# dmuley/sph-code

Measured on AMD Instinct MI355X. Metric: particle-steps/sec + achieved HBM GB/s, 10^6-particle 3D sphere, 1/2/4/8 GPUs, higher is better.
Workload: dtype f64

## Files before the change

### sph-code_amd/csrc/sphx_api.hip

```cpp
#include "sphx_internal.h"
#include <stdarg.h>
#include <stdlib.h>
#include <new>

int sphx_set_err(sphx_ctx* ctx, int code, const char* fmt, ...) {
    if (ctx) {
        va_list ap;
        va_start(ap, fmt);
        vsnprintf(ctx->err, sizeof(ctx->err), fmt, ap);
        va_end(ap);
    }
    return code;
}

void sphx_release(sphx_ctx* ctx, DevBuf& b) {
    for (size_t q = 0; q < ctx->allocs.size(); ++q)
        if (ctx->allocs[q] == b.p) { ctx->allocs[q] = ctx->allocs.back(); ctx->allocs.pop_back(); break; }
    if (b.p) (void)hipFree(b.p);
    b.p = nullptr;
    b.cap = 0;
}

int sphx_ensure(sphx_ctx* ctx, DevBuf& b, size_t bytes, hipStream_t in_use_on) {
    if (bytes == 0) bytes = 8;
// ... 275 lines not shown
    SPHX_TRY(upload(ctx, ctx->in_f, mu_array, nb));
    SPHX_TRY(upload(ctx, ctx->in_g, gamma_array, nb));
    SPHX_TRY(upload(ctx, ctx->in_h, particle_type, nb));
    if (neighbor) {
        SPHX_TRY(sphx_transpose_nbr(ctx, n, k, ctx->idx64.as<int64_t>()));
        ctx->nbr_api_valid = true; ctx->nbr_api_n = n; ctx->nbr_api_k = k;
    }
    PrepIn pin;
    pin.pos_aos(ctx->in_a.as<double>()); pin.vel_aos(ctx->in_b.as<double>());
    pin.m = ctx->in_c.as<double>(); pin.h = ctx->in_d.as<double>(); pin.T = ctx->in_e.as<double>();
    pin.mu = ctx->in_f.as<double>(); pin.gam = ctx->in_g.as<double>(); pin.ptype = ctx->in_h.as<double>();
    SPHX_TRY(sphx_prep(ctx, n, pin, visc_mode == 1, ctx->stream));
    SPHX_TRY(sphx_pass_density(ctx, n, k));
    if (visc_mode == 1) {
        SPHX_TRY(sphx_pass_visc_pw(ctx, n, k, ctx->in_c.as<double>()));
    } else {
        SPHX_TRY(sphx_pass_pi(ctx, n, k, ctx->in_d.as<double>(), ctx->in_h.as<double>()));
        SPHX_TRY(sphx_pass_visc(ctx, n, k, ctx->in_c.as<double>()));
    }
    if (f_un_nb) {
        SPHX_TRY(upload(ctx, ctx->in_i, f_un, (size_t)n * s * sizeof(double)));
        SPHX_TRY(sphx_ensure(ctx, ctx->F, (size_t)n * s * sizeof(double)));
        SPHX_TRY(sphx_pass_species(ctx, n, k, s, ctx->in_i.as<double>(), ctx->F.as<double>()));
        SPHX_TRY(download(ctx, f_un_nb, ctx->F.p, (size_t)n * s * sizeof(double)));
    }
    SPHX_TRY(download(ctx, hydro_accel, ctx->ha.p, 3 * nb));
    SPHX_TRY(download(ctx, visc_accel, ctx->va.p, 3 * nb));
    SPHX_TRY(download(ctx, visc_heat, ctx->vh.p, nb));
    SPHX_TRY(download(ctx, rho, ctx->rho.p, nb));
    SPHX_TRY(download(ctx, nden, ctx->nden.p, nb));
    SPHX_TRY(download(ctx, rho_dust, ctx->rhod.p, nb));
    HIPCHK(hipStreamSynchronize(ctx->stream));
    return SPHX_OK;
}

extern "C" int sphx_state_upload(sphx_ctx* ctx, int64_t n, int s, const double* pos, const double* vel,
                                 const double* mass, const double* ptype, const double* f_un,
                                 const double* T, const double* mu, const double* gamma,
                                 const double* E_internal, const double* accel_old) {
    if (!ctx) return SPHX_E_ARG;
    NEED(pos); NEED(vel); NEED(mass); NEED(ptype); NEED(T); NEED(mu); NEED(gamma); NEED(E_internal);
    if (n < 1 || n > 0x7FFFFFF0ll) return sphx_set_err(ctx, SPHX_E_ARG, "n=%lld out of range", (long long)n);
    if (f_un && (s < 1 || s > SPHX_MAX_SPECIES)) return sphx_set_err(ctx, SPHX_E_ARG, "s=%d out of range", s);
    HIPCHK(hipSetDevice(ctx->device));
    const size_t nb = (size_t)n * sizeof(double);
    StateArrays& st = ctx->st;
    DevBuf* scal[] = {&st.x, &st.y, &st.z, &st.vx, &st.vy, &st.vz, &st.ax, &st.ay, &st.az,
                      &st.m, &st.T, &st.mu, &st.gam, &st.E, &st.hprev, &st.ptype};
    for (DevBuf* b : scal) SPHX_TRY(sphx_ensure(ctx, *b, nb));
    SPHX_TRY(sphx_ensure(ctx, st.id, (size_t)n * sizeof(int)));
    SPHX_TRY(upload(ctx, ctx->in_a, pos, 3 * nb));
    SPHX_TRY(sphx_aos_to_soa3(ctx, n, ctx->in_a.as<double>(), st.x.as<double>(), st.y.as<double>(), st.z.as<double>()));
    SPHX_TRY(upload(ctx, ctx->in_b, vel, 3 * nb));
    SPHX_TRY(sphx_aos_to_soa3(ctx, n, ctx->in_b.as<double>(), st.vx.as<double>(), st.vy.as<double>(), st.vz.as<double>()));
    if (accel_old) {
        SPHX_TRY(upload(ctx, ctx->in_c, accel_old, 3 * nb));
        SPHX_TRY(sphx_aos_to_soa3(ctx, n, ctx->in_c.as<double>(), st.ax.as<double>(), st.ay.as<double>(), st.az.as<double>()));
    } else {
        HIPCHK(hipMemsetAsync(st.ax.p, 0, nb, ctx->stream));
        HIPCHK(hipMemsetAsync(st.ay.p, 0, nb, ctx->stream));
        HIPCHK(hipMemsetAsync(st.az.p, 0, nb, ctx->stream));
    }
    HIPCHK(hipMemcpyAsync(st.m.p, mass, nb, hipMemcpyHostToDevice, ctx->stream));
    HIPCHK(hipMemcpyAsync(st.T.p, T, nb, hipMemcpyHostToDevice, ctx->stream));
    HIPCHK(hipMemcpyAsync(st.mu.p, mu, nb, hipMemcpyHostToDevice, ctx->stream));
    HIPCHK(hipMemcpyAsync(st.gam.p, gamma, nb, hipMemcpyHostToDevice, ctx->stream));
    HIPCHK(hipMemcpyAsync(st.E.p, E_internal, nb, hipMemcpyHostToDevice, ctx->stream));
    HIPCHK(hipMemcpyAsync(st.ptype.p, ptype, nb, hipMemcpyHostToDevice, ctx->stream));
    HIPCHK(hipMemsetAsync(st.hprev.p, 0, nb, ctx->stream));
    SPHX_TRY(sphx_iota(ctx, n, st.id.as<int>()));
    ctx->s = 0;
    if (f_un) {
        const int sp = (s + 15) & ~15;
        SPHX_TRY(upload(ctx, ctx->in_d, f_un, (size_t)n * s * sizeof(double)));
        SPHX_TRY(sphx_ensure(ctx, ctx->fun_id, (size_t)n * sp * sizeof(double)));
        HIPCHK(hipMemsetAsync(ctx->fun_id.p, 0, (size_t)n * sp * sizeof(double), ctx->stream));
        HIPCHK(hipMemcpy2DAsync(ctx->fun_id.p, (size_t)sp * sizeof(double), ctx->in_d.p, (size_t)s * sizeof(double),
                                (size_t)s * sizeof(double), (size_t)n, hipMemcpyDeviceToDevice, ctx->stream));
        ctx->s = s;
        ctx->sp = sp;
    }
    HIPCHK(hipMemsetAsync(ctx->scal.p, 0, SC_NSLOTS * 8, ctx->stream));
    HIPCHK(hipMemsetAsync(ctx->badc.p, 0, (size_t)BADC_BUCKETS * BADC_STRIDE * sizeof(u64), ctx->stream));
    ctx->ct_primed = false;
    ctx->nbr_api_valid = false;
    HIPCHK(hipStreamSynchronize(ctx->stream));
    ctx->n = n;
    ctx->npad = sphx_pad64(n);
    ctx->has_state = true;
    ctx->drag = false;
    ctx->agb_on = false;
    ctx->gravity = 0;
    ctx->loop_forms = 0;
    ctx->list_valid = false;
    ctx->clip_valid = false;
    ctx->h_clip = 0.0;
    ctx->lag_bvalid[0] = ctx->lag_bvalid[1] = ctx->lag_hvalid[0] = ctx->lag_hvalid[1] = false;
    ctx->step_count = 0;
    ctx->tprev_valid = false;
    ctx->dt_last = 0.0;
    return SPHX_OK;
}

extern "C" int sphx_state_set_drag(sphx_ctx* ctx, const double* mean_grain_mass, const double* mean_cross) {
    if (!ctx) return SPHX_E_ARG;
    if (!ctx->has_state || ctx->step_count != 0)
        return sphx_set_err(ctx, SPHX_E_STATE, "sphx_state_set_drag must follow sphx_state_upload directly");
    HIPCHK(hipSetDevice(ctx->device));
    if (!mean_grain_mass || !mean_cross) { ctx->drag = false; return SPHX_OK; }
    const size_t nb = (size_t)ctx->n * sizeof(double);
    SPHX_TRY(sphx_ensure(ctx, ctx->st.mgm, nb));
    SPHX_TRY(sphx_ensure(ctx, ctx->st.mcs, nb));
    HIPCHK(hipMemcpyAsync(ctx->st.mgm.p, mean_grain_mass, nb, hipMemcpyHostToDevice, ctx->stream));
    HIPCHK(hipMemcpyAsync(ctx->st.mcs.p, mean_cross, nb, hipMemcpyHostToDevice, ctx->stream));
    HIPCHK(hipStreamSynchronize(ctx->stream));
    ctx->drag = true;
    return SPHX_OK;
}

extern "C" int sphx_state_set_loop_forms(sphx_ctx* ctx, int on, double d) {
    if (!ctx) return SPHX_E_ARG;
    if (!ctx->has_state) return sphx_set_err(ctx, SPHX_E_STATE, "sphx_state_set_loop_forms before sphx_state_upload");
    if (on && !(d > 0.0)) return sphx_set_err(ctx, SPHX_E_ARG, "the loop forms need the driver's global d > 0 (drv:68)");
    if (on && ctx->use_verlet) return sphx_set_err(ctx, SPHX_E_STATE, "loop-form steps are not combined with incremental search");
    if (on && ctx->visc_mode != 0)
        return sphx_set_err(ctx, SPHX_E_ARG, "loop-form steps have their own (pairwise) viscosity: visc_mode must be 0");
    ctx->loop_forms = on ? 1 : 0;
    ctx->loop_d = d;
    return SPHX_OK;
}

extern "C" int sphx_set_gravity_order(sphx_ctx* ctx, int order) {
    if (!ctx) return SPHX_E_ARG;
    if (order != 1 && order != 2) return sphx_set_err(ctx, SPHX_E_ARG, "gravity order %d not 1 (monopole) or 2 (quadrupole)", order);
    ctx->grav_order = order;
    return SPHX_OK;
}

extern "C" int sphx_set_clip_grad(sphx_ctx* ctx, int on) {
    if (!ctx) return SPHX_E_ARG;
    ctx->clip_grad = on ? 1 : 0;
    return SPHX_OK;
}

extern "C" int sphx_set_visc_mode(sphx_ctx* ctx, int mode) {
    if (!ctx) return SPHX_E_ARG;
    if (mode != 0 && mode != 1)
        return sphx_set_err(ctx, SPHX_E_ARG, "visc_mode %d unknown (0 = ref_axis0, 1 = pairwise)", mode);
    if (mode != 0 && ctx->loop_forms)
        return sphx_set_err(ctx, SPHX_E_ARG, "loop-form steps have their own (pairwise) viscosity: visc_mode must be 0");
    ctx->visc_mode = mode;
    return SPHX_OK;
}

extern "C" int sphx_state_set_gravity(sphx_ctx* ctx, int mode, double G) {
    if (!ctx) return SPHX_E_ARG;
    if (!ctx->has_state) return sphx_set_err(ctx, SPHX_E_STATE, "sphx_state_set_gravity before sphx_state_upload");
    if (mode < 0 || mode > 2) return sphx_set_err(ctx, SPHX_E_ARG, "gravity mode %d not in {0, 1, 2}", mode);
    if (mode == 2 && ctx->use_verlet)
        return sphx_set_err(ctx, SPHX_E_STATE, "tree gravity needs the cell grid of every step: not with incremental search");
    ctx->gravity = mode;
    ctx->grav_G = G;
    return SPHX_OK;
}

static PrepIn prep_in_of_state(const StateArrays& s) {
    PrepIn in;
    in.x = s.x.as<double>(); in.y = s.y.as<double>(); in.z = s.z.as<double>(); in.ps = 1;
    in.vx = s.vx.as<double>(); in.vy = s.vy.as<double>(); in.vz = s.vz.as<double>(); in.vs = 1;
    in.m = s.m.as<double>(); in.h = s.hprev.as<double>(); in.T = s.T.as<double>();
    in.mu = s.mu.as<double>(); in.gam = s.gam.as<double>(); in.ptype = s.ptype.as<double>();
    return in;
}

static int step_cell_hint(sphx_ctx* ctx, int64_t n, double* cell_hint) {
    *cell_hint = 0.0;
    if (ctx->step_count == 0) return SPHX_OK;
    const double* hs;
    if (ctx->lag_hvalid[ctx->lag_hslot]) {
        HIPCHK(hipEventSynchronize(ctx->lag_halias[ctx->lag_hslot] ? ctx->lag_halias[ctx->lag_hslot]
                                                                     : ctx->lag_hev[ctx->lag_hslot]));
        hs = (const double*)((char*)ctx->pinned + LAG_OFF + 512 * ctx->lag_hslot + 256);
        const u64* sv = (const u64*)hs;
        for (int q = 0; q < 10; ++q) ctx->knn_lag[q] = sv[(SC_NFAILQ - SC_HSUM) + q];
        ctx->knn_lag_valid = true;
    } else {
        HIPCHK(hipMemcpyAsync((char*)ctx->pinned + 256, ctx->scal.as<double>() + SC_HSUM, 4 * sizeof(double),
                              hipMemcpyDeviceToHost, ctx->stream));
        HIPCHK(hipStreamSynchronize(ctx->stream));
        hs = (const double*)((char*)ctx->pinned + 256);
    }
    const double hmean = hs[3] > 0.0 ? hs[0] / hs[3] : 0.0;
    if (hmean > 0.0 && isfinite(hmean)) {
        *cell_hint = ctx->cell_factor * sphx_cell_feedback(ctx, n) * hmean;
        ctx->h_clip = ctx->h_clip_factor * hmean;
    }
    return SPHX_OK;
}

static int step_search(sphx_ctx* ctx, int k, double dist, hipEvent_t* ev) {
    const int64_t n = ctx->n;
    if (ctx->use_verlet) SPHX_TRY(sphx_clamp(ctx, n, ctx->st));
    SPHX_TRY(sphx_ensure(ctx, ctx->nbr, (size_t)k * ctx->npad * sizeof(int)));
    if (ctx->use_verlet && ctx->list_valid && ctx->list_n == n && ctx->list_k == k) {
        StateArrays& r = ctx->st;
        HIPCHK(hipEventRecord(ev[1], ctx->stream));
        int64_t nfail = 0;
        SPHX_TRY(sphx_knn_refresh(ctx, n, k, r.x.as<double>(), r.y.as<double>(), r.z.as<double>(),
                                  ctx->nbr.as<int>(), r.hprev.as<double>(), &nfail));
        if (nfail == 0) {
            ctx->stats.refresh_steps++;
            return SPHX_OK;
        }
        ctx->list_valid = false;
    }
    double cell_hint = 0.0;
    SPHX_TRY(step_cell_hint(ctx, n, &cell_hint));
    {
        StateArrays& r = ctx->st;
        const bool blob = ctx->use_blob && !ctx->use_verlet;
        GridBuildOpts g;
        g.lagged = true;
        g.alias_ev = ev[1];
        g.sort_cells_later = blob;
        if (!ctx->use_verlet) { g.clamp_vel[0] = r.vx.as<double>(); g.clamp_vel[1] = r.vy.as<double>(); g.clamp_vel[2] = r.vz.as<double>(); }
        SPHX_TRY(sphx_build_grid(ctx, n, k, r.x.as<double>(), r.y.as<double>(), r.z.as<double>(), cell_hint, g));
        if (blob) SPHX_TRY(sphx_build_blob_order(ctx, n, true));
    }
    const bool split = ctx->side_stream && !ctx->use_verlet;
    SPHX_TRY(sphx_permute_state(ctx, n, split, ev[1]));
    StateArrays& r = ctx->st;
    KnnIn in;
    in.xs = r.x.as<double>(); in.ys = r.y.as<double>(); in.zs = r.z.as<double>();
    in.id = r.id.as<int>(); in.inv = ctx->inv.as<int>();
    in.rsearch = r.hprev.as<double>();
    in.hinted = ctx->step_count > 0 && !ctx->use_verlet;
    in.lag_external = true;
    in.rscale = ctx->rscale;
    in.rbound = dist;
    KnnOut o;
    o.nbr = ctx->nbr.as<int>();
    o.h_sorted = r.hprev.as<double>();
    o.idx64 = nullptr; o.dist = nullptr; o.nontriv = nullptr; o.h_by_id = nullptr;
    if (ctx->use_verlet) {
        SPHX_TRY(sphx_ensure(ctx, ctx->list64, (size_t)n * 64 * sizeof(int)));
        SPHX_TRY(sphx_ensure(ctx, ctx->dref, (size_t)n * sizeof(double)));
        o.list64 = ctx->list64.as<int>();
        o.dref = ctx->dref.as<double>();
        in.rscale = ctx->rscale_build;
    }
    SPHX_TRY(sphx_knn(ctx, n, k, in, o));
    if (split) HIPCHK(hipStreamWaitEvent(ctx->stream, ctx->ev_perm, 0));
    if (ctx->use_verlet) {
        SPHX_TRY(sphx_save_list_positions(ctx, n, r.x.as<double>(), r.y.as<double>(), r.z.as<double>()));
        ctx->list_valid = true;
        ctx->list_n = n;
        ctx->list_k = k;
    }
    ctx->stats.rebuild_steps++;
    return SPHX_OK;
}

static int step_h_sums_out(sphx_ctx* ctx, int64_t n, const double* h, hipStream_t stream) {
    SPHX_TRY(sphx_hsum(ctx, n, h, stream));
    const int hsl = ctx->lag_hslot ^ 1;
    HIPCHK(hipMemcpyAsync((char*)ctx->pinned + LAG_OFF + 512 * hsl + 256, ctx->scal.as<double>() + SC_HSUM,
                          (SC_KGDBG + 2 - SC_HSUM + 1) * sizeof(double), hipMemcpyDeviceToHost, stream));
    HIPCHK(hipEventRecord(ctx->lag_hev[hsl], stream));
    ctx->lag_halias[hsl] = nullptr;
    ctx->lag_hvalid[hsl] = true;
    ctx->lag_hslot = hsl;
    return SPHX_OK;
}

static int step_sums(sphx_ctx* ctx, int k, hipEvent_t* ev, hipEvent_t search_end, bool detail) {
    const int64_t n = ctx->n;
    StateArrays& s = ctx->st;
    const bool pairwise = ctx->visc_mode == 1 && !ctx->loop_forms;
    const bool fork = ctx->qorder && ctx->use_lds && !ctx->loop_forms && ctx->side_stream;
    if (fork) HIPCHK(hipStreamWaitEvent(ctx->side_stream, search_end, 0));
    else SPHX_TRY(step_h_sums_out(ctx, n, s.hprev.as<double>(), ctx->stream));
    if (ctx->qorder && ctx->use_lds) SPHX_TRY(sphx_blob_translate(ctx, n, k));
    const bool species = ctx->s > 0 && ctx->fun_id.p;
    if (ctx->loop_forms) {
        if (ctx->drag || species)
            SPHX_TRY(sphx_prep(ctx, n, prep_in_of_state(s), pairwise, ctx->stream));
        if (detail) HIPCHK(hipEventRecord(ev[3], ctx->stream));
        SPHX_TRY(sphx_loop_step_sums(ctx, n, k, ctx->loop_d));
        if (detail) HIPCHK(hipEventRecord(ev[9], ctx->stream));
        if (species) SPHX_TRY(sphx_step_species(ctx, n, k));
        if (detail) HIPCHK(hipEventRecord(ev[4], ctx->stream));
        if (detail) HIPCHK(hipEventRecord(ev[5], ctx->stream));
    } else {
        SPHX_TRY(sphx_prep(ctx, n, prep_in_of_state(s), pairwise, fork ? ctx->side_stream : ctx->stream));
        if (fork) {
            HIPCHK(hipEventRecord(ctx->ev_join, ctx->side_stream));
            HIPCHK(hipStreamWaitEvent(ctx->stream, ctx->ev_join, 0));
            SPHX_TRY(step_h_sums_out(ctx, n, s.hprev.as<double>(), ctx->side_stream));
        }
        if (detail) HIPCHK(hipEventRecord(ev[3], ctx->stream));
        const bool sp_fused = species && ctx->species_fused && ctx->species_lds && ctx->use_lds && ctx->qorder && ctx->blob_lists &&
                              !ctx->map_perm && ctx->sp == 16 && ctx->s <= 16 && k <= SPHX_MAX_K;
        if (sp_fused) {
            const int S = ctx->s;
            SPHX_TRY(sphx_ensure(ctx, ctx->rho, (size_t)n * sizeof(double)));
            SPHX_TRY(sphx_ensure(ctx, ctx->rhod, (size_t)n * sizeof(double)));
            SPHX_TRY(sphx_ensure(ctx, ctx->nden, (size_t)n * sizeof(double)));
            SPHX_TRY(sphx_ensure(ctx, ctx->G, (size_t)n * 3 * sizeof(double)));
            SPHX_TRY(sphx_ensure(ctx, ctx->ha, (size_t)n * 3 * sizeof(double)));
            SPHX_TRY(sphx_ensure(ctx, ctx->F, (size_t)n * S * sizeof(double)));
            if (ctx->agb_on) {
                SPHX_TRY(sphx_ensure(ctx, ctx->Zmet, (size_t)n * sizeof(double)));
                SPHX_TRY(sphx_ensure(ctx, ctx->agb_dust, (size_t)n * S * sizeof(double)));
            }
            SPHX_TRY(sphx_blob_density_species(ctx, n, k, true, S, ctx->fun_id.as<double>(), s.id.as<int>(),
                                               s.m.as<double>(), ctx->F.as<double>(), ctx->Zmet.as<double>(),
                                               ctx->agb_dust.as<double>(), (ctx->agb_on && ctx->Zmet.p && ctx->agb_dust.p) ? 1 : 0));
        } else {
            SPHX_TRY(sphx_pass_density(ctx, n, k, true));
        }
        if (detail) HIPCHK(hipEventRecord(ev[9], ctx->stream));
        if (species && !sp_fused) SPHX_TRY(sphx_step_species(ctx, n, k));
        if (detail) HIPCHK(hipEventRecord(ev[4], ctx->stream));
        if (ctx->visc_mode == 1) {
            SPHX_TRY(sphx_pass_visc_pw(ctx, n, k, s.m.as<double>()));
        } else {
            SPHX_TRY(sphx_pass_pi(ctx, n, k, s.hprev.as<double>(), s.ptype.as<double>()));
            if (detail) HIPCHK(hipEventRecord(ev[5], ctx->stream));
            SPHX_TRY(sphx_pass_visc(ctx, n, k, s.m.as<double>()));
        }
    }
    if (ctx->drag)
        SPHX_TRY(sphx_pass_drag(ctx, n, k, s.m.as<double>(), s.ptype.as<double>(), s.mgm.as<double>(), s.mcs.as<double>()));
    return SPHX_OK;
}

static int one_step(sphx_ctx* ctx, int k, double dist, int first, double fixed_dt, bool call_first, bool call_last) {
    const int64_t n = ctx->n;
    const int ring = (int)(ctx->step_count % 3);
    hipEvent_t* ev = ctx->evring[ring];
    const bool detail = ctx->timing_detail;
    ctx->ev_detail[ring] = detail;
    const bool rec0 = detail || call_first, rec7 = detail || call_last;
    ctx->ev_has07[ring] = (rec0 ? 1 : 0) | (rec7 ? 2 : 0) | (ctx->visc_mode == 1 && !ctx->loop_forms ? 4 : 0);
    ctx->map_perm = nullptr;
    ctx->qorder = nullptr;
    ctx->blob_lists = false;
    ctx->blob_split_valid = false;
    ctx->pass_part = 0;
    ctx->nbr_api_valid = false;
    if (rec0) HIPCHK(hipEventRecord(ev[0], ctx->stream));
    SPHX_TRY(step_search(ctx, k, dist, ev));
    HIPCHK(hipEventRecord(ev[2], ctx->stream));
    SPHX_TRY(step_sums(ctx, k, ev, ev[2], detail));
    if (detail) HIPCHK(hipEventRecord(ev[6], ctx->stream));
    StateArrays& s = ctx->st;
    if (ctx->gravity) {
        SPHX_TRY(sphx_ensure(ctx, ctx->grav, (size_t)n * 3 * sizeof(double)));
        double* eps = ctx->scal.as<double>() + SC_GRAV_EPS;
        SPHX_TRY(sphx_median(ctx, n, s.hprev.as<double>(), eps));
        if (ctx->gravity == 1)
            SPHX_TRY(sphx_gravity_launch(ctx, n, s.x.as<double>(), s.y.as<double>(), s.z.as<double>(), 1,
                                         s.m.as<double>(), eps, 0.0, ctx->grav_G, nullptr, ctx->grav.as<double>()));
        else
            SPHX_TRY(sphx_gravity_tree_launch(ctx, n, s.x.as<double>(), s.y.as<double>(), s.z.as<double>(),
                                              s.m.as<double>(), ctx->grav_ws, eps, 0.0, ctx->grav_G, nullptr,
                                              ctx->grav.as<double>()));
    }
    if (detail) HIPCHK(hipEventRecord(ev[8], ctx->stream));
    SPHX_TRY(sphx_integrate(ctx, n, 1, first, fixed_dt));
    if (rec7) HIPCHK(hipEventRecord(ev[7], ctx->stream));
    ctx->step_count++;
    return SPHX_OK;
}

static int collect_stats(sphx_ctx* ctx, int ring) {
    if (!(ctx->ev_pending & (1u << ring))) return SPHX_OK;
    ctx->ev_pending &= ~(1u << ring);
    hipEvent_t* ev = ctx->evring[ring];
    const int has = ctx->ev_has07[ring];
    HIPCHK(hipEventSynchronize((has & 2) ? ev[7] : ev[2]));
    sphx_stats& st = ctx->stats;
    float ms[7] = {0.f, 0.f, 0.f, 0.f, 0.f, 0.f, 0.f};
    HIPCHK(hipEventElapsedTime(&ms[1], ev[1], ev[2]));
    st.ms_search += ms[1];
    st.steps += 1;
    st.search_steps += 1;
    st.n = ctx->n;
    if (!ctx->ev_detail[ring]) return SPHX_OK;
    float tot;
    HIPCHK(hipEventElapsedTime(&tot, ev[0], ev[7]));
    HIPCHK(hipEventElapsedTime(&ms[0], ev[0], ev[1]));
    st.ms_grid += ms[0]; st.ms_total += tot;
    for (int i = 2; i < 6; ++i) {
        if ((has & 4) && i >= 4) break;
        HIPCHK(hipEventElapsedTime(&ms[i], ev[i], ev[i + 1]));
    }
    if (has & 4) HIPCHK(hipEventElapsedTime(&ms[5], ev[4], ev[6]));
    st.ms_prep += ms[2];
    float mg = 0.f, mi = 0.f;
    HIPCHK(hipEventElapsedTime(&mg, ev[6], ev[8]));
    HIPCHK(hipEventElapsedTime(&mi, ev[8], ev[7]));
    ms[6] = mi;
    st.ms_gravity += mg;
    {
        float md = 0.f, msp = 0.f;
        HIPCHK(hipEventElapsedTime(&md, ev[3], ev[9]));
        HIPCHK(hipEventElapsedTime(&msp, ev[9], ev[4]));
        ms[3] = md;
        st.ms_species += msp;
    }
    st.ms_density += ms[3]; st.ms_pi += ms[4]; st.ms_visc += ms[5]; st.ms_integrate += ms[6];
    st.detail_steps += 1;
    return SPHX_OK;
}

extern "C" int sphx_step(sphx_ctx* ctx, int nsteps, int k, double dist, int first, double fixed_dt) {
    if (!ctx) return SPHX_E_ARG;
    if (!ctx->has_state) return sphx_set_err(ctx, SPHX_E_STATE, "sphx_step before sphx_state_upload");
    if (k < 1 || k > SPHX_MAX_K) return sphx_set_err(ctx, SPHX_E_ARG, "N_NEIGH=%d not in 1..%d", k, SPHX_MAX_K);
    if (nsteps < 1) return sphx_set_err(ctx, SPHX_E_ARG, "nsteps=%d < 1", nsteps);
    HIPCHK(hipSetDevice(ctx->device));
    if (!(dist > 0.0) || !isfinite(dist)) dist = 0.0;
    ctx->k = k;
    const bool per_call = !ctx->timing_detail;
    if (per_call) HIPCHK(hipEventRecord(ctx->ev[8], ctx->stream));
    for (int it = 0; it < nsteps; ++it) {
        const int ring = (int)(ctx->step_count % 3);
        SPHX_TRY(collect_stats(ctx, ring));
        SPHX_TRY(one_step(ctx, k, dist, first && it == 0, fixed_dt, false, false));
        ctx->ev_pending |= 1u << ring;
        SPHX_TRY(collect_stats(ctx, (ring + 1) % 3));
    }
    if (per_call) HIPCHK(hipEventRecord(ctx->ev[9], ctx->stream));
    HIPCHK(hipMemcpyAsync(ctx->pinned, ctx->scal.p, SC_NSLOTS * 8, hipMemcpyDeviceToHost, ctx->stream));
    HIPCHK(hipStreamSynchronize(ctx->stream));
    for (int r = 0; r < 3; ++r) SPHX_TRY(collect_stats(ctx, (int)((ctx->step_count + r) % 3)));
    if (per_call) {
        float tot = 0.f;
        HIPCHK(hipEventElapsedTime(&tot, ctx->ev[8], ctx->ev[9]));
        ctx->stats.ms_total += tot;
    }
    const u64* sc = (const u64*)ctx->pinned;
    ctx->dt_last = ((const double*)ctx->pinned)[SC_DT];
    ctx->stats.candidates = (int64_t)sc[SC_CAND];
    ctx->stats.retries = (int64_t)sc[SC_RETRY];
    ctx->stats.fallback_queries = (int64_t)(u32)sc[SC_NFAILQ];
    ctx->stats.short_rows = (int64_t)sc[SC_SHORT];
    SPHX_TRY(sphx_badc_read(ctx));
    return SPHX_OK;
}

extern "C" int sphx_state_download(sphx_ctx* ctx, double* pos, double* vel, double* accel,
                                   double* E_internal, double* T, double* sizes, double* rho,
                                   double* nden, double* visc_heat, double* dt_last) {
    if (!ctx) return SPHX_E_ARG;
    if (!ctx->has_state) return sphx_set_err(ctx, SPHX_E_STATE, "no state uploaded");
    HIPCHK(hipSetDevice(ctx->device));
    const int64_t n = ctx->n;
    const size_t nb = (size_t)n * sizeof(double);
    StateArrays& s = ctx->st;
    const int* id = s.id.as<int>();
    SPHX_TRY(sphx_ensure(ctx, ctx->out_a, 3 * nb));
    double* stage = ctx->out_a.as<double>();
    struct V3 { double* host; DevBuf *a, *b, *c; };
    V3 v3[] = {{pos, &s.x, &s.y, &s.z}, {vel, &s.vx, &s.vy, &s.vz}, {accel, &s.ax, &s.ay, &s.az}};
    for (V3& v : v3) {
        if (!v.host) continue;
        SPHX_TRY(sphx_soa3_to_aos_by_id(ctx, n, id, v.a->as<double>(), v.b->as<double>(), v.c->as<double>(), stage));
        SPHX_TRY(download(ctx, v.host, stage, 3 * nb));
        HIPCHK(hipStreamSynchronize(ctx->stream));
    }
    struct V1 { double* host; const double* dev; };
    const bool stepped = ctx->step_count > 0;
    V1 v1[] = {{E_internal, s.E.as<double>()}, {T, s.T.as<double>()}, {sizes, s.hprev.as<double>()},
               {rho, stepped ? ctx->rho.as<double>() : nullptr},
               {nden, stepped ? ctx->nden.as<double>() : nullptr},
               {visc_heat, stepped ? ctx->vh.as<double>() : nullptr}};
    for (V1& v : v1) {
        if (!v.host) continue;
        if (!v.dev) { memset(v.host, 0, nb); continue; }
        SPHX_TRY(sphx_scatter_rows_by_id(ctx, n, 1, id, v.dev, stage));
        SPHX_TRY(download(ctx, v.host, stage, nb));
        HIPCHK(hipStreamSynchronize(ctx->stream));
    }
    if (dt_last) *dt_last = ctx->dt_last;
    return SPHX_OK;
}

int sphx_agb_table_set(sphx_ctx* ctx, int S, int nspl, const int32_t* ntx, const int32_t* nty, const double* tx, const double* ty,
                       const double* coeffs, const int32_t* mapto, double divisor, const double* mu_specie, double solar_mass) {
    ctx->agb_on = false;
    if (nspl == 0) return SPHX_OK;
    if (S < 7 || S > AGB_MAX_SPEC) return sphx_set_err(ctx, SPHX_E_ARG, "AGB table: %d species (7..%d)", S, AGB_MAX_SPEC);
    if (!ntx || !nty || !tx || !ty || !coeffs || !mapto || !mu_specie)
        return sphx_set_err(ctx, SPHX_E_ARG, "AGB table: NULL argument");
    if (nspl < 1 || nspl > AGB_MAX_SPL) return sphx_set_err(ctx, SPHX_E_ARG, "AGB table: %d splines", nspl);
    if (!(divisor != 0.0)) return sphx_set_err(ctx, SPHX_E_ARG, "AGB table: divisor is 0");
    HIPCHK(hipSetDevice(ctx->device));
    AgbTable& t = ctx->agb;
    t.nspl = nspl; t.nspec = S;
    size_t ntx_tot = 0, nty_tot = 0, nc_tot = 0;
    for (int o = 0; o < nspl; ++o) {
        if (ntx[o] < 4 || nty[o] < 4) return sphx_set_err(ctx, SPHX_E_ARG, "AGB table: spline %d has fewer than 4 knots", o);
        if (mapto[o] < 0 || mapto[o] >= S) return sphx_set_err(ctx, SPHX_E_ARG, "AGB table: mapto[%d]=%d out of range", o, mapto[o]);
        ntx_tot += ntx[o]; nty_tot += nty[o]; nc_tot += (size_t)(ntx[o] - 2) * (nty[o] - 2);
    }
    size_t ox = 0, oy = ntx_tot, oc = ntx_tot + nty_tot;
    for (int o = 0; o < nspl; ++o) {
        t.tx_off[o] = (int)ox; t.ty_off[o] = (int)oy; t.c_off[o] = (int)oc;
        t.ntx[o] = ntx[o]; t.nty[o] = nty[o]; t.mapto[o] = mapto[o];
        ox += ntx[o]; oy += nty[o]; oc += (size_t)(ntx[o] - 2) * (nty[o] - 2);
    }
// ... 122 lines not shown
```

### sph-code_amd/csrc/sphx_dev.hip

```cpp
#include "sphx_internal.h"
#pragma clang fp contract(off)
#include <float.h>
#include "sphx_leapfrog.h"

extern "C" int sphx_set_stream(sphx_ctx* ctx, void* stream) {
    if (!ctx) return SPHX_E_ARG;
    HIPCHK(hipSetDevice(ctx->device));
    HIPCHK(hipStreamSynchronize(ctx->stream));
    ctx->stream = (hipStream_t)stream;
    return SPHX_OK;
}

extern "C" int sphx_reset_stream(sphx_ctx* ctx) {
    if (!ctx) return SPHX_E_ARG;
    HIPCHK(hipSetDevice(ctx->device));
    HIPCHK(hipStreamSynchronize(ctx->stream));
    ctx->stream = ctx->own_stream;
    return SPHX_OK;
}

__global__ __launch_bounds__(256) void gather3_aos_kernel(int n, const int* perm, const double* aos,
                                                          double* xs, double* ys, double* zs, int* inv) {
    int t = blockIdx.x * blockDim.x + threadIdx.x;
    if (t >= n) return;
// ... 81 lines not shown

extern "C" int sphx_dev_get_order(sphx_ctx* ctx, int64_t n_total, int32_t* out) {
    if (!ctx) return SPHX_E_ARG;
    NEED(out);
    if (!ctx->map_perm || ctx->n != n_total)
        return sphx_set_err(ctx, SPHX_E_STATE, "sphx_dev_get_order: no search over %lld particles", (long long)n_total);
    HIPCHK(hipSetDevice(ctx->device));
    HIPCHK(hipMemcpyAsync(out, ctx->map_perm, (size_t)n_total * sizeof(int), hipMemcpyDeviceToDevice, ctx->stream));
    return SPHX_OK;
}

extern "C" int sphx_dev_select_blobs(sphx_ctx* ctx, int part) {
    if (!ctx) return SPHX_E_ARG;
    if (part < 0 || part > 2) return sphx_set_err(ctx, SPHX_E_ARG, "sphx_dev_select_blobs: part %d not in 0..2", part);
    ctx->pass_part = 0;
    if (part == 0) return 0;
    if (!(ctx->map_perm && ctx->qorder && ctx->blob_lists && ctx->blob_split_valid)) return 0;
    ctx->pass_part = part;
    return 1;
}

extern "C" int sphx_dev_blob_split_counts(sphx_ctx* ctx, int32_t counts[3]) {
    if (!ctx) return SPHX_E_ARG;
    NEED(counts);
    if (!ctx->blob_split_valid) return sphx_set_err(ctx, SPHX_E_STATE, "sphx_dev_blob_split_counts: no split (LDS passes off, or no search yet)");
    HIPCHK(hipSetDevice(ctx->device));
    HIPCHK(hipMemcpyAsync(counts, ctx->blob_split.as<int>() + (size_t)ctx->blob_split_nblk, 3 * sizeof(int),
                          hipMemcpyDeviceToHost, ctx->stream));
    HIPCHK(hipStreamSynchronize(ctx->stream));
    return SPHX_OK;
}

extern "C" int sphx_dev_set_mean_h(sphx_ctx* ctx, double mean_h) {
    if (!ctx) return SPHX_E_ARG;
    ctx->dev_hmean = mean_h;
    return SPHX_OK;
}

extern "C" int sphx_dev_prep(sphx_ctx* ctx, const double* pos, const double* vel, const double* mass,
                             const double* h, const double* T, const double* mu, const double* gamma,
                             const double* ptype) {
    if (!ctx) return SPHX_E_ARG;
    NEED(pos); NEED(vel); NEED(mass); NEED(h); NEED(T); NEED(mu); NEED(gamma); NEED(ptype);
    if (!ctx->map_perm) return sphx_set_err(ctx, SPHX_E_STATE, "sphx_dev_prep before sphx_dev_search");
    HIPCHK(hipSetDevice(ctx->device));
    PrepIn in;
    in.pos_aos(pos); in.vel_aos(vel);
    in.m = mass; in.h = h; in.T = T; in.mu = mu; in.gam = gamma; in.ptype = ptype;
    return sphx_prep(ctx, ctx->n, in, ctx->visc_mode == 1, ctx->stream);
}

struct Borrow {
    DevBuf& b;
    DevBuf saved;
    Borrow(DevBuf& buf, void* p, size_t bytes) : b(buf), saved(buf) {
        if (p) { b.p = p; b.cap = bytes; }
    }
    ~Borrow() { b = saved; }
    Borrow(const Borrow&) = delete;
    Borrow& operator=(const Borrow&) = delete;
};

extern "C" int sphx_dev_density(sphx_ctx* ctx, double* rho, double* rho_dust, double* nden,
                                double* hydro_accel) {
    if (!ctx) return SPHX_E_ARG;
    if (!ctx->map_perm) return sphx_set_err(ctx, SPHX_E_STATE, "sphx_dev_density before sphx_dev_search");
    HIPCHK(hipSetDevice(ctx->device));
    const size_t nb = (size_t)ctx->n * sizeof(double);
    Borrow b1(ctx->rho, rho, nb), b2(ctx->rhod, rho_dust, nb), b3(ctx->nden, nden, nb), b4(ctx->ha, hydro_accel, 3 * nb);
    SPHX_TRY(sphx_pass_density(ctx, ctx->n, ctx->k));
    return SPHX_OK;
}

extern "C" int sphx_dev_pi(sphx_ctx* ctx, const double* rho_complete, double* Pi, double* Bw, double* ct_out) {
    if (!ctx) return SPHX_E_ARG;
    NEED(rho_complete);
    if (!ctx->map_perm) return sphx_set_err(ctx, SPHX_E_STATE, "sphx_dev_pi before sphx_dev_search");
    HIPCHK(hipSetDevice(ctx->device));
    const int64_t n = ctx->n;
    if (ctx->pass_part != 1)
        hipLaunchKernelGGL(inject_field_kernel, dim3((unsigned)((n + 255) / 256)), dim3(256), 0, ctx->stream, (int)n,
                           ctx->map_perm, rho_complete, ctx->rho_s.as<double>(), 1);
    HIPCHK(hipGetLastError());
    if (ctx->pass_part == 2) ctx->ct_primed = true;
    {
        Borrow b1(ctx->Pi, Pi, (size_t)n * sizeof(double)), b2(ctx->Bw, Bw, (size_t)n * sizeof(double));
        SPHX_TRY(sphx_pass_pi(ctx, n, ctx->k, nullptr, nullptr));
    }
    if (ct_out)
        HIPCHK(hipMemcpyAsync(ct_out, ctx->scal.as<u64>() + SC_CT_BITS, 8, hipMemcpyDeviceToDevice, ctx->stream));
    return SPHX_OK;
}

extern "C" int sphx_dev_visc(sphx_ctx* ctx, const double* Bw_complete, const double* mass,
                             double* visc_accel, double* visc_heat) {
    if (!ctx) return SPHX_E_ARG;
    NEED(Bw_complete); NEED(mass);
    if (!ctx->map_perm) return sphx_set_err(ctx, SPHX_E_STATE, "sphx_dev_visc before sphx_dev_search");
    HIPCHK(hipSetDevice(ctx->device));
    const int64_t n = ctx->n;
    if (ctx->pass_part != 1)
        hipLaunchKernelGGL(inject_field_kernel, dim3((unsigned)((n + 255) / 256)), dim3(256), 0, ctx->stream, (int)n,
                           ctx->map_perm, Bw_complete, ctx->bc_s.as<double>(), 2);
    HIPCHK(hipGetLastError());
    Borrow b1(ctx->va, visc_accel, 3 * (size_t)n * sizeof(double)), b2(ctx->vh, visc_heat, (size_t)n * sizeof(double));
    SPHX_TRY(sphx_pass_visc(ctx, n, ctx->k, mass));
    return SPHX_OK;
}

extern "C" int sphx_dev_visc_pairwise(sphx_ctx* ctx, const double* rho_complete, const double* mass,
                                      double* visc_accel, double* visc_heat, double* ct_out) {
    if (!ctx) return SPHX_E_ARG;
    NEED(rho_complete); NEED(mass);
    if (!ctx->map_perm) return sphx_set_err(ctx, SPHX_E_STATE, "sphx_dev_visc_pairwise before sphx_dev_search");
    if (ctx->visc_mode != 1) return sphx_set_err(ctx, SPHX_E_STATE, "sphx_dev_visc_pairwise needs sphx_set_visc_mode(ctx, 1)");
    if (!ctx->recs_pw)
        return sphx_set_err(ctx, SPHX_E_STATE, "sphx_dev_visc_pairwise: the records were not built in pairwise mode "
                                               "(sphx_set_visc_mode(ctx, 1) before sphx_dev_prep)");
    HIPCHK(hipSetDevice(ctx->device));
    const int64_t n = ctx->n;
    if (ctx->pass_part != 1)
        hipLaunchKernelGGL(inject_field_kernel, dim3((unsigned)((n + 255) / 256)), dim3(256), 0, ctx->stream, (int)n,
                           ctx->map_perm, rho_complete, ctx->rho_s.as<double>(), 1);
    HIPCHK(hipGetLastError());
    if (ctx->pass_part == 2) ctx->ct_primed = true;
    {
        Borrow b1(ctx->va, visc_accel, 3 * (size_t)n * sizeof(double)), b2(ctx->vh, visc_heat, (size_t)n * sizeof(double));
        SPHX_TRY(sphx_pass_visc_pw(ctx, n, ctx->k, mass));
    }
    if (ct_out)
        HIPCHK(hipMemcpyAsync(ct_out, ctx->scal.as<u64>() + SC_CT_BITS, 8, hipMemcpyDeviceToDevice, ctx->stream));
    return SPHX_OK;
}

#define nan_to_num_v sphx_nan_to_num
struct DevIntegArgs {
    int n;
    double *pos, *vel, *acc, *E, *T;
    const double *m, *mu, *gam, *ptype, *ha, *va, *vh;
    const double *G, *rho;
    const double *drag_on, *drag_re, *drho, *drhod;
    double dt, m_h, kB, lim;
    const double* red2;
    double* dt_out;
    int first;
    double fixed_dt, dt_0, max_age;
    u64* counters;
};
__global__ __launch_bounds__(256) void dev_integrate_kernel(DevIntegArgs a) {
    int i = blockIdx.x * blockDim.x + threadIdx.x;
    if (i >= a.n) return;
    double dt = a.dt;
    if (a.red2) {
        if (a.red2[0] > 0.5) {
            if (i == 0) *a.dt_out = 0.0;
            return;
        }
        const double ct_min = -a.red2[1];
        const double ctv = sphx_ct_value(ct_min > DBL_MAX, ct_min, a.dt_0);
        dt = (a.fixed_dt > 0.0) ? a.fixed_dt : sphx_dt_rule(ctv, a.first, a.dt_0, a.max_age);
        if (i == 0) *a.dt_out = dt;
    }
    const double g = (a.ptype[i] == 0.0) ? 1.0 : 0.0;
    double v[3], pa[3], vis[3];
    bool bad_acc = false;
#pragma unroll
    for (int c = 0; c < 3; ++c) {
        v[c] = a.vel[3 * (size_t)i + c];
        if (a.G) {
            const double praw = a.G[3 * (size_t)i + c] / a.rho[i] * g;
            pa[c] = nan_to_num_v(praw);
            vis[c] = a.va[3 * (size_t)i + c];
            bad_acc = bad_acc || !sphx_finite(praw) || !sphx_finite(vis[c]);
        } else {
            const double praw = -a.ha[3 * (size_t)i + c] * g, vraw = -a.va[3 * (size_t)i + c] * g;
            pa[c] = nan_to_num_v(praw);
            vis[c] = nan_to_num_v(vraw);
            bad_acc = bad_acc || !sphx_finite(praw) || !sphx_finite(vraw);
        }
        if (a.drag_on) {
            const double draw = a.drag_on[3 * (size_t)i + c] * a.drhod[i] / a.drho[i] * g, rraw = a.drag_re[3 * (size_t)i + c];
            const double dg = nan_to_num_v(draw);
            vis[c] = dg + nan_to_num_v(rraw) + vis[c];
            bad_acc = bad_acc || !sphx_finite(draw) || !sphx_finite(rraw);
        }
    }
    double x[3], old[3], tot[3];
#pragma unroll
    for (int c = 0; c < 3; ++c) { x[c] = a.pos[3 * (size_t)i + c]; old[c] = a.acc[3 * (size_t)i + c]; }
    sphx_leapfrog_update(dt, x, v, vis, pa, nullptr, old, tot);
#pragma unroll
    for (int c = 0; c < 3; ++c) {
        a.pos[3 * (size_t)i + c] = x[c];
        a.vel[3 * (size_t)i + c] = v[c];
        a.acc[3 * (size_t)i + c] = tot[c];
    }
    double E = a.E[i], T;
    const double heat = a.vh[i];
    const bool bad_en = !sphx_finite(E) || !sphx_finite(heat * dt);
    sphx_energy_update(dt, heat, a.mu[i], a.gam[i], a.m[i], a.m_h, a.kB, E, T);
    a.E[i] = E;
    a.T[i] = T;
    if (a.counters) {
        bool bad_st = false;
#pragma unroll
        for (int c = 0; c < 3; ++c) bad_st = bad_st || !sphx_finite(x[c]) || !sphx_finite(v[c]);
        sphx_count_bad(a.counters, BAD_ACCEL, bad_acc);
        sphx_count_bad(a.counters, BAD_ENERGY, bad_en);
        sphx_count_bad(a.counters, BAD_STATE, bad_st);
    }
}
static DevIntegArgs dev_integ_args(sphx_ctx* ctx, int64_t n_owned, double* pos, double* vel, double* accel_old, double* E_internal,
                                   double* T, const double* mass, const double* mu, const double* gamma, const double* ptype,
                                   const double* ha, const double* va, const double* vh, double dt) {
// ... 595 lines not shown
```

### sph-code_amd/csrc/sphx_grid.hip

```cpp
#include "sphx_internal.h"
#include <rocprim/rocprim.hpp>
#include <float.h>

#define RED_BLOCK 256
#define RED_MAXBLOCKS 1024
#define FUSED_MAXBLOCKS 4096

__device__ __forceinline__ double wave_min(double v) {
#pragma unroll
    for (int o = 32; o > 0; o >>= 1) v = fmin(v, __shfl_xor(v, o, 64));
    return v;
}
__device__ __forceinline__ double wave_max(double v) {
#pragma unroll
    for (int o = 32; o > 0; o >>= 1) v = fmax(v, __shfl_xor(v, o, 64));
    return v;
}

__device__ __forceinline__ double wave_sum(double v) {
#pragma unroll
    for (int o = 32; o > 0; o >>= 1) v += __shfl_xor(v, o, 64);
    return v;
}

#define BB_W 13
#define BB_PIVOT 16
#define BB_OUT 19
struct ClipBox { double lo[3], hi[3]; int on; double pivot[3]; int pivot_dev; };
static void clip_set_pivot(ClipBox& clip, const double* fallback) {
    clip.pivot_dev = 0;
    for (int c = 0; c < 3; ++c) clip.pivot[c] = clip.on ? 0.5 * (clip.lo[c] + clip.hi[c]) : (fallback ? fallback[c] : 0.0);
    if (!clip.on && !fallback) clip.pivot_dev = 1;
    for (int c = 0; c < 3; ++c) if (!isfinite(clip.pivot[c])) clip.pivot[c] = 0.0;
}
__device__ __forceinline__ void clip_pivot(const ClipBox& clip, int n, const double* x, const double* y, const double* z,
                                           double p[3]) {
    p[0] = clip.pivot[0]; p[1] = clip.pivot[1]; p[2] = clip.pivot[2];
    if (clip.pivot_dev && n > 0) {
        const double f[3] = {x[0], y[0], z[0]};
        for (int c = 0; c < 3; ++c) p[c] = isfinite(f[c]) ? f[c] : 0.0;
    }
}
__global__ __launch_bounds__(RED_BLOCK) void bbox_partial(int n, const double* x, const double* y,
                                                          const double* z, ClipBox clip, double* partial) {
    __shared__ double sm[RED_BLOCK / 64][BB_W];
    double mn[3] = {INFINITY, INFINITY, INFINITY}, mx[3] = {-INFINITY, -INFINITY, -INFINITY};
    double su[3] = {0.0, 0.0, 0.0}, sq[3] = {0.0, 0.0, 0.0}, cnt = 0.0;
    double piv[3];
    clip_pivot(clip, n, x, y, z, piv);
    for (int i = blockIdx.x * blockDim.x + threadIdx.x; i < n; i += gridDim.x * blockDim.x) {
        double v[3] = {x[i], y[i], z[i]};
        if (isfinite(v[0]) && isfinite(v[1]) && isfinite(v[2])) {
            bool in = true;
#pragma unroll
            for (int c = 0; c < 3; ++c) {
                mn[c] = fmin(mn[c], v[c]); mx[c] = fmax(mx[c], v[c]);
                if (clip.on && (v[c] < clip.lo[c] || v[c] > clip.hi[c])) in = false;
            }
            if (in) {
                cnt += 1.0;
#pragma unroll
                for (int c = 0; c < 3; ++c) { const double r = v[c] - piv[c]; su[c] += r; sq[c] += r * r; }
            }
        }
    }
    int lane = threadIdx.x & 63, wave = threadIdx.x >> 6;
#pragma unroll
    for (int c = 0; c < 3; ++c) {
        mn[c] = wave_min(mn[c]); mx[c] = wave_max(mx[c]); su[c] = wave_sum(su[c]); sq[c] = wave_sum(sq[c]);
    }
    cnt = wave_sum(cnt);
    if (lane == 0) {
        for (int c = 0; c < 3; ++c) {
            sm[wave][c] = mn[c]; sm[wave][3 + c] = mx[c]; sm[wave][6 + c] = su[c]; sm[wave][9 + c] = sq[c];
        }
        sm[wave][12] = cnt;
    }
    __syncthreads();
    if (threadIdx.x < BB_W) {
        const int c = threadIdx.x;
        double v = sm[0][c];
        for (int w = 1; w < RED_BLOCK / 64; ++w)
            v = c < 3 ? fmin(v, sm[w][c]) : (c < 6 ? fmax(v, sm[w][c]) : v + sm[w][c]);
        partial[blockIdx.x * BB_W + c] = v;
    }
// ... 19 lines not shown
    if ((threadIdx.x & 63) == 0) sw[threadIdx.x >> 6] = v;
    __syncthreads();
    if (threadIdx.x == 0) {
        const double a0 = sw[0], a1 = sw[1], a2 = sw[2], a3 = sw[3];
        out[c] = c < 3 ? fmin(fmin(a0, a1), fmin(a2, a3)) : (c < 6 ? fmax(fmax(a0, a1), fmax(a2, a3)) : (a0 + a1) + (a2 + a3));
    }
}

static int bbox_launch(sphx_ctx* ctx, int64_t n, const double* x, const double* y, const double* z, bool use_clip,
                       void* host_dst) {
    ClipBox clip;
    clip.on = (use_clip && ctx->clip_valid) ? 1 : 0;
    for (int c = 0; c < 3; ++c) { clip.lo[c] = ctx->clip_lo[c]; clip.hi[c] = ctx->clip_hi[c]; }
    clip_set_pivot(clip, nullptr);
    int blocks = (int)((n + RED_BLOCK - 1) / RED_BLOCK);
    if (blocks > RED_MAXBLOCKS) blocks = RED_MAXBLOCKS;
    SPHX_TRY(sphx_ensure(ctx, ctx->bbox_tmp, (size_t)(RED_MAXBLOCKS + 2 + FUSED_MAXBLOCKS) * BB_W * sizeof(double)));
    double* part = ctx->bbox_tmp.as<double>();
    double* fin = part + (size_t)RED_MAXBLOCKS * BB_W;
    hipLaunchKernelGGL(bbox_partial, dim3(blocks), dim3(RED_BLOCK), 0, ctx->stream, (int)n, x, y, z, clip, part);
    hipLaunchKernelGGL(bbox_final, dim3(BB_W + 3), dim3(256), 0, ctx->stream, blocks, part, fin, (int)n, x, y, z, clip);
    HIPCHK(hipGetLastError());
    HIPCHK(hipMemcpyAsync(host_dst, fin, BB_OUT * sizeof(double), hipMemcpyDeviceToHost, ctx->stream));
    return SPHX_OK;
}
static void bbox_finish(const void* host_src, double out_minmax[13], double rel[9] = nullptr) {
    memcpy(out_minmax, host_src, BB_W * sizeof(double));
    double piv[3];
    memcpy(piv, (const double*)host_src + BB_PIVOT, sizeof(piv));
    const double cnt = out_minmax[12] > 0.0 ? out_minmax[12] : 1.0;
    for (int c = 0; c < 3; ++c) {
        const double mean = out_minmax[6 + c] / cnt;
        double var = out_minmax[9 + c] / cnt - mean * mean;
        if (rel) { rel[c] = out_minmax[c] - piv[c]; rel[3 + c] = out_minmax[3 + c] - piv[c]; rel[6 + c] = mean; }
        out_minmax[6 + c] = piv[c] + mean;
        out_minmax[9 + c] = var > 0.0 ? sqrt(var) : 0.0;
    }
}
static int bbox_sync(sphx_ctx* ctx, int64_t n, const double* x, const double* y, const double* z,
                     double out_minmax[13], bool use_clip, double rel[9]) {
    SPHX_TRY(bbox_launch(ctx, n, x, y, z, use_clip, ctx->pinned));
    HIPCHK(hipStreamSynchronize(ctx->stream));
    bbox_finish(ctx->pinned, out_minmax, rel);
    return SPHX_OK;
}
int sphx_bbox(sphx_ctx* ctx, int64_t n, const double* x, const double* y, const double* z,
              double out_minmax[13], bool use_clip) {
    return bbox_sync(ctx, n, x, y, z, out_minmax, use_clip, nullptr);
}

__device__ __forceinline__ int cell_coord_g(double v, double vmin, double inv_cell, int nmax1) {
    double t = (v - vmin) * inv_cell;
    t = fmin(fmax(t, 0.0), (double)nmax1);
    return (int)t;
}

__global__ __launch_bounds__(256) void cell_count(int n, const double* x, const double* y,
                                                  const double* z, GridParams g, int* cell_of,
                                                  int* hist) {
    int i = blockIdx.x * blockDim.x + threadIdx.x;
    if (i >= n) return;
    int cx = cell_coord_g(x[i], g.xmin, g.inv_cell, g.nx - 1);
    int cy = cell_coord_g(y[i], g.ymin, g.inv_cell, g.ny - 1);
    int cz = cell_coord_g(z[i], g.zmin, g.inv_cell, g.nz - 1);
    int c = (cz * g.ny + cy) * g.nx + cx;
    cell_of[i] = c;
    atomicAdd(&hist[c], 1);
}

struct FusedCountArgs {
    int n;
    double *x, *y, *z, *vx, *vy, *vz;
    double lim;
    ClipBox clip;
    GridParams g;
    int* cell_of;
    int* hist;
    double* partial;
    unsigned* ticket;
    double* fin;
    u64* ct_reset;
    int* zero_int;
    int* rank;
};
__global__ __launch_bounds__(RED_BLOCK) void grid_count_fused(FusedCountArgs a) {
    __shared__ double sm[RED_BLOCK / 64][BB_W];
    double mn[3] = {INFINITY, INFINITY, INFINITY}, mx[3] = {-INFINITY, -INFINITY, -INFINITY};
    double su[3] = {0.0, 0.0, 0.0}, sq[3] = {0.0, 0.0, 0.0}, cnt = 0.0;
    const GridParams g = a.g;
    const double piv[3] = {a.clip.pivot[0], a.clip.pivot[1], a.clip.pivot[2]};
    if (a.ct_reset && blockIdx.x == 0 && threadIdx.x == 0) *a.ct_reset = SPHX_CT_NONE;
    if (a.zero_int && blockIdx.x == 0 && threadIdx.x == 0) { a.zero_int[0] = 0; a.zero_int[1] = 0; }
    for (int i = blockIdx.x * blockDim.x + threadIdx.x; i < a.n; i += gridDim.x * blockDim.x) {
        double v[3] = {a.x[i], a.y[i], a.z[i]};
        if (a.vx) {
            const double o0 = v[0], o1 = v[1], o2 = v[2];
#pragma unroll
            for (int c = 0; c < 3; ++c) {
                double q = v[c];
                q = (q > a.lim) ? a.lim : q;
                q = (q < -a.lim) ? -a.lim : q;
                v[c] = sphx_nan_to_num(q);
            }
            if (__double_as_longlong(v[0]) != __double_as_longlong(o0)) a.x[i] = v[0];
            if (__double_as_longlong(v[1]) != __double_as_longlong(o1)) a.y[i] = v[1];
            if (__double_as_longlong(v[2]) != __double_as_longlong(o2)) a.z[i] = v[2];
            const double w0 = a.vx[i], w1 = a.vy[i], w2 = a.vz[i];
            const double u0 = sphx_nan_to_num(w0), u1 = sphx_nan_to_num(w1), u2 = sphx_nan_to_num(w2);
            if (__double_as_longlong(u0) != __double_as_longlong(w0)) a.vx[i] = u0;
            if (__double_as_longlong(u1) != __double_as_longlong(w1)) a.vy[i] = u1;
            if (__double_as_longlong(u2) != __double_as_longlong(w2)) a.vz[i] = u2;
        }
        if (isfinite(v[0]) && isfinite(v[1]) && isfinite(v[2])) {
            bool in = true;
#pragma unroll
            for (int c = 0; c < 3; ++c) {
                mn[c] = fmin(mn[c], v[c]); mx[c] = fmax(mx[c], v[c]);
                if (a.clip.on && (v[c] < a.clip.lo[c] || v[c] > a.clip.hi[c])) in = false;
            }
            if (in) {
                cnt += 1.0;
#pragma unroll
                for (int c = 0; c < 3; ++c) { const double r = v[c] - piv[c]; su[c] += r; sq[c] += r * r; }
            }
        }
        const int cx = cell_coord_g(v[0], g.xmin, g.inv_cell, g.nx - 1);
        const int cy = cell_coord_g(v[1], g.ymin, g.inv_cell, g.ny - 1);
        const int cz = cell_coord_g(v[2], g.zmin, g.inv_cell, g.nz - 1);
        const int c = (cz * g.ny + cy) * g.nx + cx;
        a.cell_of[i] = c;
        if (a.rank) a.rank[i] = atomicAdd(&a.hist[c], 1);
        else atomicAdd(&a.hist[c], 1);
    }
    const int lane = threadIdx.x & 63, wave = threadIdx.x >> 6;
#pragma unroll
    for (int c = 0; c < 3; ++c) {
        mn[c] = wave_min(mn[c]); mx[c] = wave_max(mx[c]); su[c] = wave_sum(su[c]); sq[c] = wave_sum(sq[c]);
    }
    cnt = wave_sum(cnt);
    if (lane == 0) {
        for (int c = 0; c < 3; ++c) {
            sm[wave][c] = mn[c]; sm[wave][3 + c] = mx[c]; sm[wave][6 + c] = su[c]; sm[wave][9 + c] = sq[c];
        }
        sm[wave][12] = cnt;
    }
    __syncthreads();
    if (threadIdx.x < BB_W) {
        const int c = threadIdx.x;
        double v = sm[0][c];
        for (int w = 1; w < RED_BLOCK / 64; ++w)
            v = c < 3 ? fmin(v, sm[w][c]) : (c < 6 ? fmax(v, sm[w][c]) : v + sm[w][c]);
        a.partial[blockIdx.x * BB_W + c] = v;
    }
}


#define SCAN_ITEMS 8
#define SCAN_BLOCK 256
#define SCAN_TILE (SCAN_ITEMS * SCAN_BLOCK)

__device__ __forceinline__ int block_exclusive_scan(int v, int* total_out) {
    __shared__ int wsum[SCAN_BLOCK / 64];
    int lane = threadIdx.x & 63, wave = threadIdx.x >> 6;
    int incl = v;
#pragma unroll
    for (int o = 1; o < 64; o <<= 1) {
        int up = __shfl_up(incl, o, 64);
        if (lane >= o) incl += up;
    }
    if (lane == 63) wsum[wave] = incl;
    __syncthreads();
    int woff = 0, tot = 0;
#pragma unroll
    for (int w = 0; w < SCAN_BLOCK / 64; ++w) {
        int s = wsum[w];
        if (w < wave) woff += s;
        tot += s;
    }
    __syncthreads();
    *total_out = tot;
    return woff + incl - v;
}

#define LBS_ITEMS 32
#define LBS_TILE (LBS_ITEMS * 256)
#define LBS_MAXTILES 512
template <int ZERO>
__global__ __launch_bounds__(256) void lookback_scan_kernel(int n_items, int* __restrict__ in, int* __restrict__ out,
                                                            u64* state, int* ctr, unsigned epoch, int ntiles) {
    __shared__ int s_prefix;
// ... 177 lines not shown
    }
    if (bb_part && (int)blockIdx.x < BB_W && (int)gridDim.x >= BB_W) {
        const int c = blockIdx.x;
        double v = c < 3 ? INFINITY : (c < 6 ? -INFINITY : 0.0);
        for (int b = threadIdx.x; b < bb_nblocks; b += 256) {
            const double p = bb_part[b * BB_W + c];
            v = c < 3 ? fmin(v, p) : (c < 6 ? fmax(v, p) : v + p);
        }
        v = c < 3 ? wave_min(v) : (c < 6 ? wave_max(v) : wave_sum(v));
        if ((threadIdx.x & 63) == 0) sw[threadIdx.x >> 6] = v;
        __syncthreads();
        if (threadIdx.x == 0) {
            const double a0 = sw[0], a1 = sw[1], a2 = sw[2], a3 = sw[3];
            const double r_ = c < 3 ? fmin(fmin(a0, a1), fmin(a2, a3)) : (c < 6 ? fmax(fmax(a0, a1), fmax(a2, a3)) : (a0 + a1) + (a2 + a3));
            bb_out[c] = r_;
            if (bb_host) bb_host[c] = r_;
        }
    }
}

#define CELL_SORT_SERIAL 16
#define CELL_SORT_WAVE 512
#define DENSE_CELL 48
#define CROWDED_LIST_MIN 2048
template <int U>
__device__ __forceinline__ void sort_crowded_cell(int* perm, int bs, int m, int lane) {
    int v[U], rank[U];
#pragma unroll
    for (int u = 0; u < U; ++u) {
        const int q = lane + 64 * u;
        v[u] = q < m ? perm[bs + q] : 0x7FFFFFFF;
        rank[u] = 0;
    }
#pragma unroll
    for (int c2 = 0; c2 < U; ++c2) {
        const int lc = m - 64 * c2 < 64 ? m - 64 * c2 : 64;
        for (int tt = 0; tt < lc; ++tt) {
            const int kt = __builtin_amdgcn_readlane(v[c2], tt);
#pragma unroll
            for (int u = 0; u < U; ++u) rank[u] += kt < v[u] ? 1 : 0;
        }
    }
#pragma unroll
    for (int u = 0; u < U; ++u)
        if (lane + 64 * u < m) perm[bs + rank[u]] = v[u];
}
__device__ __forceinline__ void sort_crowded_cell_any(int* perm, int bs, int m, int lane) {
    if (m <= 64) sort_crowded_cell<1>(perm, bs, m, lane);
    else if (m <= 128) sort_crowded_cell<2>(perm, bs, m, lane);
    else if (m <= 256) sort_crowded_cell<4>(perm, bs, m, lane);
    else sort_crowded_cell<8>(perm, bs, m, lane);
}
__device__ __forceinline__ void sort_cell_members(int* perm, int s, int cnt, bool on) {
    if (on && cnt > 1 && cnt <= CELL_SORT_SERIAL) {
        for (int i = s + 1; i < s + cnt; ++i) {
            const int v = perm[i];
            int j = i - 1;
            while (j >= s && perm[j] > v) { perm[j + 1] = perm[j]; --j; }
            perm[j + 1] = v;
        }
    }
    u64 big = __builtin_amdgcn_ballot_w64(on && cnt > CELL_SORT_SERIAL && cnt <= CELL_SORT_WAVE);
    const int lane = threadIdx.x & 63;
    while (big) {
        const int t = __builtin_ctzll(big);
        big &= big - 1;
        const int bs = __builtin_amdgcn_readlane(s, t), m = __builtin_amdgcn_readlane(cnt, t);
        sort_crowded_cell_any(perm, bs, m, lane);
    }
}
__global__ __launch_bounds__(256) void cell_sort_members(int ncells, const int* cell_start, int* perm) {
    int c = blockIdx.x * blockDim.x + threadIdx.x;
    int s = 0, cnt = 0;
    if (c < ncells) { s = cell_start[c]; cnt = cell_start[c + 1] - s; }
    sort_cell_members(perm, s, cnt, true);
}

#define SPHX_MAX_CELLS (SCAN_TILE * 4096)

int sphx_build_grid(sphx_ctx* ctx, int64_t n, int k, const double* x, const double* y, const double* z, double cell_hint,
                    const GridBuildOpts& opts) {
    double bb[13], rel[9];
    bool clamp_pending = opts.clamp_vel[0] != nullptr;
    auto clamp_now = [&]() -> int {
        if (!clamp_pending) return SPHX_OK;
        clamp_pending = false;
        return sphx_clamp(ctx, n, ctx->st);
    };
    ClipBox clip0;
    clip0.on = ctx->clip_valid ? 1 : 0;
    for (int c = 0; c < 3; ++c) { clip0.lo[c] = ctx->clip_lo[c]; clip0.hi[c] = ctx->clip_hi[c]; }
    bool fused = false;
    int lag_cur = 0;
    if (opts.lagged) {
        const int prev = ctx->lag_bslot, cur = prev ^ 1;
        char* slot = (char*)ctx->pinned + LAG_OFF;
        const int64_t pn = ctx->lag_bn[prev];
        const int use = (ctx->lag_bvalid[prev] && pn > 0 && (n > pn ? n - pn : pn - n) * 4 <= n) ? prev : cur;
        lag_cur = cur;
        fused = use == prev;
        if (!fused) {
            SPHX_TRY(clamp_now());
            SPHX_TRY(bbox_launch(ctx, n, x, y, z, true, slot + 512 * cur));
            HIPCHK(hipEventRecord(ctx->lag_bev[cur], ctx->stream));
            ctx->lag_balias[cur] = nullptr;
        }
        HIPCHK(hipEventSynchronize(ctx->lag_balias[use] ? ctx->lag_balias[use] : ctx->lag_bev[use]));
        bbox_finish(slot + 512 * use, bb, rel);
        ctx->lag_bvalid[cur] = true;
        ctx->lag_bn[cur] = n;
        ctx->lag_bslot = cur;
    } else {
        SPHX_TRY(clamp_now());
        SPHX_TRY(bbox_sync(ctx, n, x, y, z, bb, true, rel));
    }
    if (ctx->clip_valid && bb[12] < 0.5 * (double)n) {
        SPHX_TRY(clamp_now());
        SPHX_TRY(bbox_sync(ctx, n, x, y, z, bb, false, rel));
    }
    double tmin[3], tmax[3], L[3];
    for (int c = 0; c < 3; ++c) {
        if (!(bb[3 + c] >= bb[c])) { bb[c] = 0.0; bb[3 + c] = 0.0; rel[c] = rel[3 + c] = 0.0; }
        tmin[c] = bb[c]; tmax[c] = bb[3 + c];
        const double piv = bb[6 + c] - rel[6 + c];
        double lo_r = rel[c], hi_r = rel[3 + c];
        const double lo = rel[6 + c] - ctx->box_sigmas * bb[9 + c], hi = rel[6 + c] + ctx->box_sigmas * bb[9 + c];
        if (bb[9 + c] > 0.0 && hi > lo) {
            if (lo_r < lo) { lo_r = lo; bb[c] = piv + lo; }
            if (hi_r > hi) { hi_r = hi; bb[3 + c] = piv + hi; }
        }
        L[c] = hi_r - lo_r;
        if (!(L[c] >= 0.0) || !isfinite(L[c])) L[c] = bb[3 + c] - bb[c];
    }
    double Lmax = 0.0;
    for (int c = 0; c < 3; ++c) if (L[c] > Lmax) Lmax = L[c];
    for (int c = 0; c < 3; ++c) {
        const double mid = 0.5 * (bb[c] + bb[3 + c]), half = (L[c] > 0.0 ? L[c] : Lmax);
        ctx->clip_lo[c] = mid - half;
        ctx->clip_hi[c] = mid + half;
    }
    ctx->clip_valid = (Lmax > 0.0);
    if (!(Lmax > 0.0)) Lmax = 1.0;
    double cell = cell_hint;
    if (!(cell > 0.0) || !isfinite(cell)) {
        double V = 1.0;
        for (int c = 0; c < 3; ++c) V *= (L[c] > 1e-6 * Lmax ? L[c] : 1e-6 * Lmax);
        cell = ctx->cell_factor * cbrt(V * (double)k / ((double)n * 4.1887902047863905));
    }
    if (cell < Lmax * 1e-4) cell = Lmax * 1e-4;
    int64_t cap = 32 * n + 1024;
    if (cap > SPHX_MAX_CELLS) cap = SPHX_MAX_CELLS;
    if (ctx->max_cells > 0 && cap > ctx->max_cells) cap = ctx->max_cells;
    int nx, ny, nz;
    for (;;) {
        nx = (int)fmin(floor(L[0] / cell) + 1.0, 2047.0);
        ny = (int)fmin(floor(L[1] / cell) + 1.0, 2047.0);
        nz = (int)fmin(floor(L[2] / cell) + 1.0, 2047.0);
        int64_t tot = (int64_t)nx * ny * nz;
        if (tot <= cap) break;
        cell *= 1.02 * cbrt((double)tot / (double)cap);
    }
    GridParams& g = ctx->grid;
    for (int c = 0; c < 3; ++c) { ctx->tbox_h[c] = tmin[c]; ctx->tbox_h[3 + c] = tmax[c]; }
    ctx->olev.L = 0;
    ctx->tbox = ctx->bbox_tmp.as<double>() + (size_t)RED_MAXBLOCKS * BB_W;
    g.xmin = bb[0]; g.ymin = bb[1]; g.zmin = bb[2];
    g.cell = cell; g.inv_cell = 1.0 / cell;
    g.nx = nx; g.ny = ny; g.nz = nz;
    g.ncells = nx * ny * nz;
    g.fnx1 = (float)(nx - 1); g.fny1 = (float)(ny - 1); g.fnz1 = (float)(nz - 1);
    ctx->stats.cells = g.ncells;
    ctx->stats.cell_size = cell;

    const int nc = g.ncells;
    SPHX_TRY(sphx_ensure(ctx, ctx->cell_of, (size_t)n * sizeof(int)));
    SPHX_TRY(sphx_ensure(ctx, ctx->perm, (size_t)n * sizeof(int)));
    SPHX_TRY(sphx_ensure(ctx, ctx->cell_start, ((size_t)nc + 2) * sizeof(int)));
    const size_t fill_cap0 = ctx->cell_fill.cap;
    SPHX_TRY(sphx_ensure(ctx, ctx->cell_fill, ((size_t)nc + 2) * sizeof(int)));
    if (ctx->cell_fill.cap != fill_cap0) ctx->cell_fill_zeroed = nullptr;
    int nblk = (nc + SCAN_TILE - 1) / SCAN_TILE;
    SPHX_TRY(sphx_ensure(ctx, ctx->scan_tmp, ((size_t)nblk + 2) * sizeof(int)));
    int* fill = ctx->cell_fill.as<int>();
    int* start = ctx->cell_start.as<int>();
    int* bsum = ctx->scan_tmp.as<int>();
    if (ctx->cell_fill_zeroed != ctx->cell_fill.p) {
        HIPCHK(hipMemsetAsync(fill, 0, ctx->cell_fill.cap, ctx->stream));
        ctx->cell_fill_zeroed = ctx->cell_fill.p;
    }
    int pb = (int)((n + 255) / 256);
    (void)bsum;
    int bb_fold_blocks = 0;
    const int* rank_dev = nullptr;
    const double* bb_fold_part = nullptr;
    double* bb_fold_out = nullptr;
    if (fused) {
        const bool fresh = ctx->bbox_tmp.p == nullptr;
        SPHX_TRY(sphx_ensure(ctx, ctx->bbox_tmp, (size_t)(RED_MAXBLOCKS + 2 + FUSED_MAXBLOCKS) * BB_W * sizeof(double)));
        double* fin = ctx->bbox_tmp.as<double>() + (size_t)RED_MAXBLOCKS * BB_W;
        unsigned* ticket = reinterpret_cast<unsigned*>(fin + BB_W);
        double* part = fin + 2 * BB_W;
        if (fresh || !ctx->bbox_ticket_zeroed) {
            HIPCHK(hipMemsetAsync(ticket, 0, sizeof(double), ctx->stream));
            ctx->bbox_ticket_zeroed = true;
        }
        FusedCountArgs fa;
        fa.n = (int)n;
        fa.x = const_cast<double*>(x); fa.y = const_cast<double*>(y); fa.z = const_cast<double*>(z);
        fa.vx = fa.vy = fa.vz = nullptr;
        if (clamp_pending) { fa.vx = opts.clamp_vel[0]; fa.vy = opts.clamp_vel[1]; fa.vz = opts.clamp_vel[2]; }
        clamp_pending = false;
        fa.lim = ctx->cst.pos_clamp;
        fa.clip = clip0;
        clip_set_pivot(fa.clip, ctx->tbox_h);
        memcpy((char*)ctx->pinned + LAG_OFF + 512 * lag_cur + BB_PIVOT * sizeof(double), fa.clip.pivot, 3 * sizeof(double));
        fa.g = g;
        fa.cell_of = ctx->cell_of.as<int>();
        fa.hist = fill;
        fa.partial = part; fa.ticket = ticket; fa.fin = fin;
        fa.ct_reset = ctx->scal.as<u64>() + SC_CT_BITS;
        fa.zero_int = nullptr;
        SPHX_TRY(sphx_ensure(ctx, ctx->cell_rank, (size_t)n * sizeof(int)));
        fa.rank = ctx->cell_rank.as<int>();
        rank_dev = fa.rank;
        if (ctx->fail_list.p && ctx->fail_list.cap >= ((size_t)sphx_pad64(n) + 64) * sizeof(int)) {
            fa.zero_int = ctx->fail_list.as<int>() + sphx_pad64(n);
            ctx->fcount_zeroed = ctx->fail_list.p;
            ctx->fcount_zeroed_n = n;
        }
        ctx->ct_primed = true;
        int fb = pb < FUSED_MAXBLOCKS ? pb : FUSED_MAXBLOCKS;
        hipLaunchKernelGGL(grid_count_fused, dim3(fb), dim3(RED_BLOCK), 0, ctx->stream, fa);
        HIPCHK(hipGetLastError());
        if (pb >= BB_W) {
            bb_fold_blocks = fb; bb_fold_part = part; bb_fold_out = fin;
        } else {
            hipLaunchKernelGGL(bbox_final, dim3(BB_W), dim3(256), 0, ctx->stream, fb, part, fin, 0,
                               (const double*)nullptr, (const double*)nullptr, (const double*)nullptr, fa.clip);
            bb_fold_out = fin;
        }
    } else {
        hipLaunchKernelGGL(cell_count, dim3(pb), dim3(256), 0, ctx->stream, (int)n, x, y, z, g,
                           ctx->cell_of.as<int>(), fill);
    }
    bool hist_zeroed = false;
    SPHX_TRY(excl_scan_plus_total(ctx, fill, start, nc, rank_dev != nullptr, &hist_zeroed));
    const bool to_host = bb_fold_part != nullptr && bb_fold_out && pb >= BB_W;
    double* bb_host = to_host ? reinterpret_cast<double*>((char*)ctx->pinned + LAG_OFF + 512 * lag_cur) : nullptr;
    hipLaunchKernelGGL(cell_scatter, dim3(pb), dim3(256), 0, ctx->stream, (int)n,
                       ctx->cell_of.as<int>(), start, fill, ctx->perm.as<int>(), bb_fold_blocks, bb_fold_part, bb_fold_out, bb_host, rank_dev);
    if (rank_dev && !hist_zeroed) HIPCHK(hipMemsetAsync(fill, 0, ((size_t)nc + 1) * sizeof(int), ctx->stream));
    if (bb_fold_out) {
        char* slot = (char*)ctx->pinned + LAG_OFF;
        if (!to_host)
            HIPCHK(hipMemcpyAsync(slot + 512 * lag_cur, bb_fold_out, BB_W * sizeof(double), hipMemcpyDeviceToHost, ctx->stream));
        if (opts.alias_ev) {
            ctx->lag_balias[lag_cur] = opts.alias_ev;
        } else {
            HIPCHK(hipEventRecord(ctx->lag_bev[lag_cur], ctx->stream));
            ctx->lag_balias[lag_cur] = nullptr;
        }
    }
    ctx->cells_unsorted = opts.sort_cells_later;
    if (!opts.sort_cells_later) {
        hipLaunchKernelGGL(cell_sort_members, dim3((unsigned)((nc + 255) / 256)), dim3(256), 0, ctx->stream, nc, start,
                           ctx->perm.as<int>());
    }
    HIPCHK(hipGetLastError());
    return SPHX_OK;
}

__device__ __forceinline__ int olev_key_of(const OutLevels& o, double x, double y, double z) {
    const double ax = fabs(x - o.cx), ay = fabs(y - o.cy), az = fabs(z - o.cz);
    const double m = fmax(fmax(ax, ay), az) / o.hmax;
    int e = 0;
    (void)frexp(m, &e);
    int lev = (m == m && m <= 1.7e308) ? e : o.L;
    lev = lev < 1 ? 1 : (lev > o.L ? o.L : lev);
    const double W = ldexp(o.hmax, lev);
    const double ic = (double)OLEV_N / (2.0 * W);
    const double nm1 = (double)(OLEV_N - 1);
    const int cx = (int)fmin(fmax((x - (o.cx - W)) * ic, 0.0), nm1);
    const int cy = (int)fmin(fmax((y - (o.cy - W)) * ic, 0.0), nm1);
    const int cz = (int)fmin(fmax((z - (o.cz - W)) * ic, 0.0), nm1);
    return ((lev - 1) * OLEV_N + cz) * OLEV_N * OLEV_N + cy * OLEV_N + cx;
}
__global__ __launch_bounds__(256) void olev_count(int n, const double* x, const double* y, const double* z, GridParams g,
                                                  OutLevels o, int* key, int* hist) {
    const int i = blockIdx.x * blockDim.x + threadIdx.x;
    if (i >= n) return;
    const double xi = x[i], yi = y[i], zi = z[i];
    int kx = -1;
    if (sphx_outside_box(g, xi, yi, zi)) {
        kx = olev_key_of(o, xi, yi, zi);
        atomicAdd(&hist[kx], 1);
    }
    key[i] = kx;
}
__global__ __launch_bounds__(256) void olev_scatter(int n, const int* key, const int* start, int* hist, int* list) {
    const int i = blockIdx.x * blockDim.x + threadIdx.x;
    if (i >= n) return;
    const int kx = key[i];
    if (kx < 0) return;
    list[start[kx] + atomicSub(&hist[kx], 1) - 1] = i;
}

int sphx_build_outlier_levels(sphx_ctx* ctx, int64_t n, const double* xs, const double* ys, const double* zs) {
    const GridParams& g = ctx->grid;
    OutLevels& o = ctx->olev;
    o.L = 0;
    const double ex = 0.5 * g.nx * g.cell, ey = 0.5 * g.ny * g.cell, ez = 0.5 * g.nz * g.cell;
    o.cx = g.xmin + ex; o.cy = g.ymin + ey; o.cz = g.zmin + ez;
    o.hmax = fmax(fmax(ex, ey), ez);
    if (!(o.hmax > 0.0) || !isfinite(o.hmax)) return SPHX_OK;
    double ext = 0.0;
// ... 146 lines not shown
```

### sph-code_amd/csrc/sphx_integrate.hip

```cpp
#include "sphx_internal.h"
#pragma clang fp contract(off)
#include <float.h>

#include "sphx_leapfrog.h"
#define nan_to_num sphx_nan_to_num

__global__ __launch_bounds__(256) void clamp_kernel(int n, double lim, double* x, double* y, double* z,
                                                    double* vx, double* vy, double* vz) {
    int i = blockIdx.x * blockDim.x + threadIdx.x;
    if (i >= n) return;
    double* p[3] = {x, y, z};
    double* v[3] = {vx, vy, vz};
#pragma unroll
    for (int c = 0; c < 3; ++c) {
        p[c][i] = sphx_clamp_pos(p[c][i], lim);
        v[c][i] = nan_to_num(v[c][i]);
    }
}

int sphx_clamp(sphx_ctx* ctx, int64_t n, StateArrays& s) {
    hipLaunchKernelGGL(clamp_kernel, dim3((unsigned)((n + 255) / 256)), dim3(256), 0, ctx->stream, (int)n,
                       ctx->cst.pos_clamp, s.x.as<double>(), s.y.as<double>(), s.z.as<double>(),
                       s.vx.as<double>(), s.vy.as<double>(), s.vz.as<double>());
    HIPCHK(hipGetLastError());
    return SPHX_OK;
}

struct GatherArgs {
    int n, narr, s;
    const int* perm;
    const double* src[18];
    double* dst[18];
    const int* id_src; int* id_dst; int* inv;
    const double* fun_src; double* fun_dst;
    GridParams bs_g; BlobBits bs_b;
    const int *bs_cell_of, *bs_cell_start, *bs_mstart;
    int* bs_porder;
    int* bs_mcount;
};
__global__ __launch_bounds__(256) void gather_kernel(GatherArgs a) {
    int t = blockIdx.x * blockDim.x + threadIdx.x;
    if (t >= a.n) return;
    const int p = a.perm[t];
    if (a.bs_porder) {
        const int c = a.bs_cell_of[p];
        const int cx = c % a.bs_g.nx, cy = (c / a.bs_g.nx) % a.bs_g.ny, cz = c / (a.bs_g.nx * a.bs_g.ny);
        const unsigned rk = blob_rank(cx, cy, cz, a.bs_b);
        a.bs_porder[a.bs_mstart[rk] + (t - a.bs_cell_start[c])] = t;
        if (t == a.bs_cell_start[c]) a.bs_mcount[rk] = 0;
    }
    for (int q = 0; q < a.narr; ++q) a.dst[q][t] = a.src[q][p];
    if (a.id_src) {
        const int id = a.id_src[p];
        a.id_dst[t] = id;
        if (a.inv) a.inv[id] = t;
    }
    if (a.fun_src) {
        const double2* src = reinterpret_cast<const double2*>(a.fun_src + (size_t)p * a.s);
        double2* dst = reinterpret_cast<double2*>(a.fun_dst + (size_t)t * a.s);
        for (int q = 0; q < a.s / 2; ++q) dst[q] = src[q];
    }
}

int sphx_permute_state(sphx_ctx* ctx, int64_t n, bool split, hipEvent_t after_first) {
    StateArrays& a = ctx->st;
    StateArrays& b = ctx->alt;
    DevBuf* src[] = {&a.x, &a.y, &a.z, &a.hprev, &a.vx, &a.vy, &a.vz, &a.ax, &a.ay, &a.az,
                     &a.m, &a.T, &a.mu, &a.gam, &a.E, &a.ptype};
    DevBuf* dst[] = {&b.x, &b.y, &b.z, &b.hprev, &b.vx, &b.vy, &b.vz, &b.ax, &b.ay, &b.az,
                     &b.m, &b.T, &b.mu, &b.gam, &b.E, &b.ptype};
    GatherArgs g;
    g.bs_porder = nullptr;
    if (ctx->blob_scatter_pending) {
        g.bs_g = ctx->grid; g.bs_b = ctx->blob_scatter_bits;
        g.bs_cell_of = ctx->cell_of.as<int>(); g.bs_cell_start = ctx->cell_start.as<int>();
        g.bs_mstart = ctx->blob_scatter_mstart; g.bs_porder = ctx->porder.as<int>();
        g.bs_mcount = ctx->mcount.as<int>();
        ctx->blob_scatter_pending = false;
    }
    g.n = (int)n; g.narr = 16; g.s = ctx->sp;
    g.perm = ctx->perm.as<int>();
    for (int q = 0; q < 16; ++q) {
        SPHX_TRY(sphx_ensure(ctx, *dst[q], (size_t)n * sizeof(double)));
        g.src[q] = src[q]->as<double>();
        g.dst[q] = dst[q]->as<double>();
    }
    if (ctx->drag) {
// ... 34 lines not shown
    __shared__ bool last;
    double s = 0.0, c = 0.0;
    unsigned nbad = 0;
    for (int i = blockIdx.x * blockDim.x + threadIdx.x; i < n; i += gridDim.x * blockDim.x) {
        const double v = h[i];
        if (v > 0.0 && (clip <= 0.0 || v <= clip)) { s += v; c += 1.0; }
        nbad += (v > 0.0 && v <= DBL_MAX) ? 0u : 1u;
    }
    if (__ballot(nbad != 0u)) {
#pragma unroll
        for (int o = 32; o > 0; o >>= 1) nbad += __shfl_xor(nbad, o, 64);
        if ((threadIdx.x & 63) == 0)
            atomicAdd(&counters[(((blockIdx.x << 2) | (threadIdx.x >> 6)) & (BADC_BUCKETS - 1)) * BADC_STRIDE + BAD_H], (u64)nbad);
    }
#pragma unroll
    for (int o = 32; o > 0; o >>= 1) { s += __shfl_xor(s, o, 64); c += __shfl_xor(c, o, 64); }
    if ((threadIdx.x & 63) == 0) { sm[threadIdx.x >> 6] = s; sc[threadIdx.x >> 6] = c; }
    __syncthreads();
    if (threadIdx.x == 0) {
        partial[2 * blockIdx.x] = sm[0] + sm[1] + sm[2] + sm[3];
        partial[2 * blockIdx.x + 1] = sc[0] + sc[1] + sc[2] + sc[3];
        __threadfence();
        last = atomicInc(ticket, gridDim.x - 1) == gridDim.x - 1;
    }
    __syncthreads();
    if (last) {
        __threadfence();
        double ts = 0.0, tc = 0.0;
        for (unsigned b = threadIdx.x; b < gridDim.x; b += blockDim.x) {
            ts += __builtin_nontemporal_load(&partial[2 * b]);
            tc += __builtin_nontemporal_load(&partial[2 * b + 1]);
        }
#pragma unroll
        for (int o = 32; o > 0; o >>= 1) { ts += __shfl_xor(ts, o, 64); tc += __shfl_xor(tc, o, 64); }
        __syncthreads();
        if ((threadIdx.x & 63) == 0) { sm[threadIdx.x >> 6] = ts; sc[threadIdx.x >> 6] = tc; }
        __syncthreads();
        if (threadIdx.x == 0) {
            *out_sum = (sm[0] + sm[1]) + (sm[2] + sm[3]);
            *out_cnt = (sc[0] + sc[1]) + (sc[2] + sc[3]);
        }
    }
}
#define HSUM_BLOCKS 512
int sphx_hsum(sphx_ctx* ctx, int64_t n, const double* h, hipStream_t stream) {
    double* out = ctx->scal.as<double>() + SC_HSUM;
    double* cnt = ctx->scal.as<double>() + SC_HCNT;
    const bool fresh = ctx->hsum_tmp.p == nullptr;
    SPHX_TRY(sphx_ensure(ctx, ctx->hsum_tmp, (size_t)(2 * HSUM_BLOCKS + 2) * sizeof(double), stream));
    double* partial = ctx->hsum_tmp.as<double>();
    unsigned* ticket = reinterpret_cast<unsigned*>(partial + 2 * HSUM_BLOCKS);
    if (fresh) HIPCHK(hipMemsetAsync(ticket, 0, sizeof(double), stream));
    int blocks = (int)((n + 255) / 256);
    if (blocks > HSUM_BLOCKS) blocks = HSUM_BLOCKS;
    hipLaunchKernelGGL(hsum_kernel, dim3(blocks), dim3(256), 0, stream, (int)n, h, ctx->h_clip, partial, ticket,
                       out, cnt, ctx->badc.as<u64>());
    HIPCHK(hipGetLastError());
    return SPHX_OK;
}

__global__ void prime_ct_kernel(u64* ct_bits) { *ct_bits = SPHX_CT_NONE; }
int sphx_prime_ct(sphx_ctx* ctx, u64* ct_bits) {
    hipLaunchKernelGGL(prime_ct_kernel, dim3(1), dim3(1), 0, ctx->stream, ct_bits);
    HIPCHK(hipGetLastError());
    return SPHX_OK;
}

__global__ void dt_kernel(u64* ct_bits, double* dt_out, int first, double fixed_dt, double dt_0,
                          double max_age) {
    if (threadIdx.x != 0 || blockIdx.x != 0) return;
    double dt;
    const u64 b = *ct_bits;
    *ct_bits = SPHX_CT_NONE;
    if (fixed_dt > 0.0) {
        dt = fixed_dt;
    } else {
        const double ct = sphx_ct_value(b == SPHX_CT_NONE, __longlong_as_double((long long)b), dt_0);
        dt = sphx_dt_rule(ct, first, dt_0, max_age);
    }
    *dt_out = dt;
}

int sphx_compute_dt(sphx_ctx* ctx, int first, double fixed_dt) {
    hipLaunchKernelGGL(dt_kernel, dim3(1), dim3(64), 0, ctx->stream, ctx->scal.as<u64>() + SC_CT_BITS,
                       ctx->scal.as<double>() + SC_DT, first, fixed_dt, ctx->cst.dt_0, ctx->cst.max_age);
    HIPCHK(hipGetLastError());
    ctx->ct_primed = true;
    return SPHX_OK;
}

struct IntegArgs {
    int n;
    double *x, *y, *z, *vx, *vy, *vz, *ax, *ay, *az;
    double *E, *T;
    const double *m, *mu, *gam, *ptype;
    const double *ha, *va, *vh;
    const double *rho, *rhod, *drag_on, *drag_re;
    const double* grav;
    const double* G;
    const double* dt;
    double m_h, kB;
    int no_old;
    const u64* ct_bits;
    double* dt_out;
    int first;
    double fixed_dt, dt_0, max_age;
    u64* counters;
};
__global__ __launch_bounds__(256) void integrate_kernel(IntegArgs a) {
    int i = blockIdx.x * blockDim.x + threadIdx.x;
    if (i >= a.n) return;
    double dt;
    if (a.ct_bits) {
        if (a.fixed_dt > 0.0) {
            dt = a.fixed_dt;
        } else {
            const u64 b = *a.ct_bits;
            const double ct = sphx_ct_value(b == SPHX_CT_NONE, __longlong_as_double((long long)b), a.dt_0);
            dt = sphx_dt_rule(ct, a.first, a.dt_0, a.max_age);
        }
        if (i == 0) *a.dt_out = dt;
    } else {
        dt = *a.dt;
    }
    const double g = (a.ptype[i] == 0.0) ? 1.0 : 0.0;
    const double v[3] = {a.vx[i], a.vy[i], a.vz[i]};
    double pa[3], vis[3];
    bool bad_acc = false;
#pragma unroll
    for (int c = 0; c < 3; ++c) {
        if (a.G) {
            const double praw = a.G[3 * (size_t)i + c] / a.rho[i] * g;
            pa[c] = nan_to_num(praw);
            vis[c] = a.va[3 * (size_t)i + c];
            bad_acc = bad_acc || !sphx_finite(praw) || !sphx_finite(vis[c]);
        } else {
            const double praw = -a.ha[3 * (size_t)i + c] * g, vraw = -a.va[3 * (size_t)i + c] * g;
            pa[c] = nan_to_num(praw);
            vis[c] = nan_to_num(vraw);
            bad_acc = bad_acc || !sphx_finite(praw) || !sphx_finite(vraw);
        }
        if (a.drag_on) {
            const double draw = a.drag_on[3 * (size_t)i + c] * a.rhod[i] / a.rho[i] * g, rraw = a.drag_re[3 * (size_t)i + c];
            const double dg = nan_to_num(draw);
            vis[c] = dg + nan_to_num(rraw) + vis[c];
            bad_acc = bad_acc || !sphx_finite(draw) || !sphx_finite(rraw);
        }
    }
    double x[3] = {a.x[i], a.y[i], a.z[i]};
    double vv[3] = {v[0], v[1], v[2]};
    double gr[3], old[3], tot[3];
#pragma unroll
    for (int c = 0; c < 3; ++c) gr[c] = a.grav ? a.grav[3 * (size_t)i + c] : 0.0;
    old[0] = a.ax[i]; old[1] = a.ay[i]; old[2] = a.az[i];
    sphx_leapfrog_update(dt, x, vv, vis, pa, a.grav ? gr : nullptr, a.no_old ? nullptr : old, tot);
    a.x[i] = x[0]; a.y[i] = x[1]; a.z[i] = x[2];
    a.vx[i] = vv[0]; a.vy[i] = vv[1]; a.vz[i] = vv[2];
    a.ax[i] = tot[0]; a.ay[i] = tot[1]; a.az[i] = tot[2];
    double E = a.E[i], T;
    const double heat = a.vh[i];
    const bool bad_en = !sphx_finite(E) || !sphx_finite(heat * dt);
    sphx_energy_update(dt, heat, a.mu[i], a.gam[i], a.m[i], a.m_h, a.kB, E, T);
    a.E[i] = E;
    a.T[i] = T;
    if (a.counters) {
        bool bad_st = false;
#pragma unroll
        for (int c = 0; c < 3; ++c) bad_st = bad_st || !sphx_finite(x[c]) || !sphx_finite(vv[c]);
        sphx_count_bad(a.counters, BAD_ACCEL, bad_acc);
        sphx_count_bad(a.counters, BAD_ENERGY, bad_en);
        sphx_count_bad(a.counters, BAD_STATE, bad_st);
    }
}

int sphx_integrate(sphx_ctx* ctx, int64_t n, int fold_dt, int first, double fixed_dt) {
    StateArrays& s = ctx->st;
    IntegArgs a;
    a.ct_bits = fold_dt ? ctx->scal.as<u64>() + SC_CT_BITS : nullptr;
    a.dt_out = ctx->scal.as<double>() + SC_DT;
    a.first = first; a.fixed_dt = fixed_dt; a.dt_0 = ctx->cst.dt_0; a.max_age = ctx->cst.max_age;
    a.n = (int)n;
    a.x = s.x.as<double>(); a.y = s.y.as<double>(); a.z = s.z.as<double>();
    a.vx = s.vx.as<double>(); a.vy = s.vy.as<double>(); a.vz = s.vz.as<double>();
    a.ax = s.ax.as<double>(); a.ay = s.ay.as<double>(); a.az = s.az.as<double>();
    SPHX_TRY(sphx_ensure(ctx, ctx->alt.T, (size_t)n * sizeof(double)));
    a.E = s.E.as<double>(); a.T = ctx->alt.T.as<double>();
    a.m = s.m.as<double>(); a.mu = s.mu.as<double>(); a.gam = s.gam.as<double>();
    a.ptype = s.ptype.as<double>();
    a.ha = ctx->ha.as<double>(); a.va = ctx->va.as<double>(); a.vh = ctx->vh.as<double>();
    a.rho = ctx->rho.as<double>(); a.rhod = ctx->rhod.as<double>();
    a.drag_on = ctx->drag ? ctx->drag_on.as<double>() : nullptr;
    a.drag_re = ctx->drag ? ctx->drag_re.as<double>() : nullptr;
    a.grav = ctx->gravity ? ctx->grav.as<double>() : nullptr;
    a.G = ctx->loop_forms ? ctx->G.as<double>() : nullptr;
    a.dt = ctx->scal.as<double>() + SC_DT;
    a.m_h = ctx->cst.m_h; a.kB = ctx->cst.k_B;
    a.no_old = 0;
    a.counters = ctx->badc.as<u64>();
    hipLaunchKernelGGL(integrate_kernel, dim3((unsigned)((n + 255) / 256)), dim3(256), 0, ctx->stream, a);
    HIPCHK(hipGetLastError());
    { DevBuf t = s.T; s.T = ctx->alt.T; ctx->alt.T = t; }
    ctx->tprev_valid = true;
    return SPHX_OK;
}

__global__ __launch_bounds__(256) void pressure_by_id(int n, const int* id, const double* nden, const double* T, double kB,
                                                      double* out) {
    const int t = blockIdx.x * blockDim.x + threadIdx.x;
    if (t < n) out[id[t]] = nden[t] * kB * T[t];
}
extern "C" int sphx_state_download_pressure(sphx_ctx* ctx, double* pressure) {
    if (!ctx || !pressure) return SPHX_E_ARG;
    if (!ctx->has_state) return sphx_set_err(ctx, SPHX_E_STATE, "no state uploaded");
    HIPCHK(hipSetDevice(ctx->device));
    const int64_t n = ctx->n;
    if (ctx->step_count < 1 || !ctx->tprev_valid || !ctx->alt.T.p) { memset(pressure, 0, (size_t)n * sizeof(double)); return SPHX_OK; }
    SPHX_TRY(sphx_ensure(ctx, ctx->out_a, (size_t)n * sizeof(double)));
    hipLaunchKernelGGL(pressure_by_id, dim3((unsigned)((n + 255) / 256)), dim3(256), 0, ctx->stream, (int)n,
                       ctx->st.id.as<int>(), ctx->nden.as<double>(), ctx->alt.T.as<double>(), ctx->cst.k_B, ctx->out_a.as<double>());
    HIPCHK(hipGetLastError());
    HIPCHK(hipMemcpyAsync(pressure, ctx->out_a.p, (size_t)n * sizeof(double), hipMemcpyDeviceToHost, ctx->stream));
    HIPCHK(hipStreamSynchronize(ctx->stream));
    return SPHX_OK;
}

__global__ __launch_bounds__(256) void dt_rule_kernel(int n, const double* ct, const int* first, double dt_0,
                                                      double max_age, double* out) {
    int i = blockIdx.x * blockDim.x + threadIdx.x;
    if (i < n) out[i] = sphx_dt_rule(ct[i], first[i], dt_0, max_age);
}
static int up_(sphx_ctx* ctx, DevBuf& b, const void* host, size_t bytes) {
    SPHX_TRY(sphx_ensure(ctx, b, bytes));
    HIPCHK(hipMemcpyAsync(b.p, host, bytes, hipMemcpyHostToDevice, ctx->stream));
    return SPHX_OK;
}

extern "C" int sphx_dt_rule(sphx_ctx* ctx, int64_t n, const double* ct, const int32_t* first, double* dt) {
    if (!ctx) return SPHX_E_ARG;
    NEED(ct); NEED(first); NEED(dt);
    if (n < 1) return SPHX_OK;
    HIPCHK(hipSetDevice(ctx->device));
    SPHX_TRY(up_(ctx, ctx->in_a, ct, (size_t)n * 8));
    SPHX_TRY(up_(ctx, ctx->in_b, first, (size_t)n * 4));
    SPHX_TRY(sphx_ensure(ctx, ctx->out_a, (size_t)n * 8));
    hipLaunchKernelGGL(dt_rule_kernel, dim3((unsigned)((n + 255) / 256)), dim3(256), 0, ctx->stream, (int)n,
                       ctx->in_a.as<double>(), ctx->in_b.as<int>(), ctx->cst.dt_0, ctx->cst.max_age, ctx->out_a.as<double>());
    HIPCHK(hipGetLastError());
    HIPCHK(hipMemcpyAsync(dt, ctx->out_a.p, (size_t)n * 8, hipMemcpyDeviceToHost, ctx->stream));
    HIPCHK(hipStreamSynchronize(ctx->stream));
    return SPHX_OK;
}

__global__ __launch_bounds__(256) void clamp_aos_kernel(int n3, double lim, double* pos, double* vel) {
    int e = blockIdx.x * blockDim.x + threadIdx.x;
    if (e >= n3) return;
    pos[e] = sphx_clamp_pos(pos[e], lim);
    vel[e] = nan_to_num(vel[e]);
}
extern "C" int sphx_clamp_arrays(sphx_ctx* ctx, int64_t n, double* points, double* velocities) {
    if (!ctx) return SPHX_E_ARG;
    NEED(points); NEED(velocities);
    if (n < 1) return SPHX_OK;
    HIPCHK(hipSetDevice(ctx->device));
    const size_t nb3 = (size_t)n * 24;
    SPHX_TRY(up_(ctx, ctx->in_a, points, nb3));
    SPHX_TRY(up_(ctx, ctx->in_b, velocities, nb3));
    hipLaunchKernelGGL(clamp_aos_kernel, dim3((unsigned)((3 * n + 255) / 256)), dim3(256), 0, ctx->stream, (int)(3 * n),
                       ctx->cst.pos_clamp, ctx->in_a.as<double>(), ctx->in_b.as<double>());
    HIPCHK(hipGetLastError());
    HIPCHK(hipMemcpyAsync(points, ctx->in_a.p, nb3, hipMemcpyDeviceToHost, ctx->stream));
    HIPCHK(hipMemcpyAsync(velocities, ctx->in_b.p, nb3, hipMemcpyDeviceToHost, ctx->stream));
    HIPCHK(hipStreamSynchronize(ctx->stream));
    return SPHX_OK;
}

extern "C" int sphx_leapfrog(sphx_ctx* ctx, int64_t n, double* points, double* velocities, double* total_accel,
                             const double* old_accel, double* E_internal, double* T, const double* mass,
                             const double* mu, const double* gamma, const double* ptype, const double* grav_accel,
                             const double* delp, const double* densities, const double* dust_densities,
                             const double* drag_on_gas, const double* drag_reaction, const double* av_accel,
                             const double* av_heat, double dt) {
    if (!ctx) return SPHX_E_ARG;
    NEED(points); NEED(velocities); NEED(total_accel); NEED(E_internal); NEED(T); NEED(mass); NEED(mu);
    NEED(gamma); NEED(ptype); NEED(delp); NEED(densities); NEED(av_accel); NEED(av_heat);
    if ((drag_on_gas != nullptr) != (drag_reaction != nullptr) || (drag_on_gas && !dust_densities))
// ... 120 lines not shown
```

### sph-code_amd/csrc/sphx_internal.h

```cpp
#pragma once
#include <hip/hip_runtime.h>
#include <stdint.h>
#include <stdio.h>
#include <string.h>
#include <math.h>
#include <float.h>
#include <vector>
#include "../../include/sphx.h"
#include "sphx_agb.h"

#define SPHX_WAVE 64
#define SPHX_W6_C 1.5666814710608448

typedef unsigned long long u64;
typedef unsigned int u32;

struct DevBuf {
    void* p = nullptr;
    size_t cap = 0;
    template <class T> T* as() const { return (T*)p; }
};

struct __attribute__((aligned(64))) RecA {
    double x, y, z;
// ... 62 lines not shown
    unsigned out = 0;
    for (int q = 0; q < b; ++q) {
        out |= ((X[2] >> q) & 1u) << (3 * q);
        out |= ((X[1] >> q) & 1u) << (3 * q + 1);
        out |= ((X[0] >> q) & 1u) << (3 * q + 2);
    }
    return out;
}
__device__ __forceinline__ unsigned blob_rank(int cx, int cy, int cz, BlobBits b) {
    if (b.hilbert) return hilbert_rank((unsigned)cx, (unsigned)cy, (unsigned)cz, b.hilbert);
    unsigned out = 0;
    int pos = 0;
    for (int q = 0; q < 11; ++q) {
        if (q < b.bx) out |= (unsigned)((cx >> q) & 1) << pos++;
        if (q < b.by) out |= (unsigned)((cy >> q) & 1) << pos++;
        if (q < b.bz) out |= (unsigned)((cz >> q) & 1) << pos++;
    }
    return out;
}

struct StateArrays {
    DevBuf x, y, z, vx, vy, vz, ax, ay, az;
    DevBuf m, T, mu, gam, E, hprev;
    DevBuf ptype;
    DevBuf id;
    DevBuf fun;
    DevBuf mgm, mcs;
};

#define SPHX_LDS_KERNELS 16

struct sphx_ctx {
    int device = 0;
    hipStream_t stream = nullptr;
    hipStream_t own_stream = nullptr;
    hipStream_t side_stream = nullptr;
    sphx_constants cst;
    char tunables[1024] = {0};
    double rscale = 1.08, cell_factor = 0.55;
    double rscale_build = 1.3;
    bool use_verlet = false;
    bool use_blob = true;
    int blob_curve = 0;
    bool use_group = true;
    bool use_lds = true;
    bool drag_lds = true;
    bool blob_split_on = true;
    bool species_lds = true;
    bool species_fused = true;
    int blob_grid = 0;
    int blob_slots = 1 << 20;
    int olev_mode = 2;
    int distrust_mode = 0;
    bool cell_feedback = true;
    double cell_fb_hi = 0.30, cell_fb_lo = 0.10;
    int64_t max_cells = 0;
    double box_sigmas = 3.0;
    double h_clip_factor = 8.0;
    double reach_cap = 0.0;
    bool timing_detail = false;
    int clip_grad = 0;
    int visc_mode = 0;
    bool drag = false;
    int loop_forms = 0;
    double loop_d = 0.0;
    int gravity = 0;
    double grav_G = 0.0;
    int grav_order = 2;
    bool grav_per_thread = false;
    int grav_ws = 1;
    bool agb_on = false;
    AgbTable agb;
    double dev_hmean = 0.0;

    char err[512] = {0};
    sphx_stats stats;
    int64_t n = 0, npad = 0;
    int k = 0, s = 0;
    int sp = 0;
    bool has_state = false;
    int64_t step_count = 0;
    double dt_last = 0.0;
    bool tprev_valid = false;
    bool ct_primed = false;
    bool recs_pw = false;
    bool nbr_api_valid = false;
    int64_t nbr_api_n = 0;
    int nbr_api_k = 0;
    bool list_valid = false;
    int64_t list_n = 0;
    int list_k = 0;
    const int* map_perm = nullptr;
    int map_nactive = 0;
    const int* qorder = nullptr;
    bool blob_lists = false;
    bool blob_split_valid = false;
    int blob_split_nblk = 0;
    int pass_part = 0;
    bool loop2_interior_done = false;
    bool dev_ev_pending = false;
    const double *dev_drag_on = nullptr, *dev_drag_re = nullptr, *dev_drag_rho = nullptr, *dev_drag_rhod = nullptr;
    GridParams grid;
    const double* tbox = nullptr;
    double tbox_h[6] = {0, 0, 0, 0, 0, 0};
    double clip_lo[3] = {0, 0, 0}, clip_hi[3] = {0, 0, 0};
    bool clip_valid = false;
    double h_clip = 0.0;
    double cell_scale = 1.0;
    bool cells_unsorted = false;
    bool blob_scatter_pending = false;
    BlobBits blob_scatter_bits;
    const int* blob_scatter_mstart = nullptr;
    bool bbox_ticket_zeroed = false;
    const void* cell_fill_zeroed = nullptr;
    const void* mcount_zeroed = nullptr;
    int mcount_zeroed_M = 0;
    const void* fcount_zeroed = nullptr;
    int64_t fcount_zeroed_n = 0;
    const void* ds_cnt_zeroed = nullptr;
    const void* olev_fill_zeroed = nullptr;
    unsigned lbs_epoch[2] = {0u, 0u};
    const void* lds_raised[SPHX_LDS_KERNELS] = {nullptr};
    int n_lds_raised = 0;
    OutLevels olev;
    bool olev_ev_valid = false;
    u64 farq_seen = 0;
    int64_t farq_last = 0;
    int64_t list_len_last = 0;
    bool knn_lag_valid = false;
    u64 knn_lag[10] = {0, 0, 0, 0, 0, 0, 0, 0, 0, 0};
    u64 densep_seen = 0;
    int64_t densep_last = 0;
    u64 crowded_seen = 0;
    int64_t crowded_last = 0;
    bool distrust = false;
    u64 badhint_seen = 0;
    bool ev_detail[3] = {false, false, false};
    int ev_has07[3] = {0, 0, 0};
    unsigned ev_pending = 0;
    hipEvent_t lag_balias[2] = {nullptr, nullptr}, lag_halias[2] = {nullptr, nullptr};
    bool lag_bvalid[2] = {false, false}, lag_hvalid[2] = {false, false};
    int64_t lag_bn[2] = {0, 0};
    int lag_bslot = 0, lag_hslot = 0;

    std::vector<void*> allocs;
    DevBuf rec1, recv;
    DevBuf rho_s, bc_s, self_s;
    DevBuf drag_on, drag_re;
    DevBuf need_pyr;
    DevBuf fun_id;
    DevBuf crowded;
    DevBuf loop_side;
    DevBuf ds_cnt, ds_start, ds_ent;
    DevBuf lrec_a, lrec_v;
    DevBuf grav, grav_sort, grav_tmp;
    DevBuf grav_pyr, grav_cell;
    DevBuf grav_quad;
    DevBuf list64, dref, pos0, pos4;
    DevBuf nbr;
    DevBuf porder, mcount, mstart;
    DevBuf agb_knots, Zmet, agb_dust;
    DevBuf fail_list;
    DevBuf olev_start, olev_fill, olev_list, olev_key;
    DevBuf lbs_state[2];
    DevBuf cell_rank;
    DevBuf tie_list;
    DevBuf slot16, uniq;
// ... 5 lines not shown
    DevBuf idx64, dist_out, nontriv, h_api;
    DevBuf arb_rec, arb_wrec, arb_flag, arb_cmax, arb_q, arb_key, arb_tmp, arb_acc, arb_out, arb_red;
    DevBuf arb_pos, arb_cs, arb_perm;
    int64_t arb_ball_id = 0, arb_ball_n = 0, arb_ball_m = 0;
    GridParams arb_g;
    double arb_tb[6] = {0, 0, 0, 0, 0, 0};
    double arb_ms[4] = {0, 0, 0, 0};
    hipEvent_t arb_ev[5] = {nullptr, nullptr, nullptr, nullptr, nullptr};
    StateArrays st, alt;
    DevBuf badc;
    DevBuf scal_tmp;
    DevBuf hsum_tmp;
    hipEvent_t ev_join = nullptr;
    hipEvent_t ev_perm = nullptr;
    hipEvent_t olev_ev = nullptr;
    hipEvent_t ev[10] = {nullptr};
    hipEvent_t evring[3][10] = {{nullptr}};
    hipEvent_t lag_bev[2] = {nullptr, nullptr}, lag_hev[2] = {nullptr, nullptr};
    void* pinned = nullptr;
};

int sphx_set_err(sphx_ctx* ctx, int code, const char* fmt, ...);
int sphx_ensure(sphx_ctx* ctx, DevBuf& b, size_t bytes, hipStream_t in_use_on);
static inline int sphx_ensure(sphx_ctx* ctx, DevBuf& b, size_t bytes) { return sphx_ensure(ctx, b, bytes, ctx->stream); }
void sphx_release(sphx_ctx* ctx, DevBuf& b);

#define HIPCHK(expr)                                                                         \
    do {                                                                                     \
        hipError_t e_ = (expr);                                                              \
        if (e_ != hipSuccess)                                                                \
            return sphx_set_err(ctx, SPHX_E_HIP, "%s:%d %s -> %s", __FILE__, __LINE__,       \
                                #expr, hipGetErrorString(e_));                               \
    } while (0)
#define NEED(p)                                                                              \
    do {                                                                                     \
        if (!(p)) return sphx_set_err(ctx, SPHX_E_ARG, "%s: argument %s is NULL", __func__, #p); \
    } while (0)
#define SPHX_TRY(expr)                                                                       \
    do {                                                                                     \
        int r_ = (expr);                                                                     \
        if (r_ != SPHX_OK) return r_;                                                        \
    } while (0)

static inline int64_t sphx_pad64(int64_t n) { return (n + 63) & ~int64_t(63); }

__device__ __forceinline__ int xcd_block(int b, int nb) {
    const int q = nb >> 3, r = nb & 7, x = b & 7, s = b >> 3;
    return x * q + (x < r ? x : r) + s;
}

#ifndef SPHX_SUM_PARTS
#define SPHX_SUM_PARTS 4
#endif

#define LAG_OFF 1024

__device__ __forceinline__ double sphx_nan_to_num(double v) {
    if (v != v) return 0.0;
    if (v > DBL_MAX) return DBL_MAX;
    if (v < -DBL_MAX) return -DBL_MAX;
    return v;
}

#define SPHX_CT_NONE 0x7FF0000000000000ull
int sphx_prime_ct(sphx_ctx* ctx, u64* ct_bits);

enum {
    SC_CT_BITS = 0,
    SC_DT = 1,
    SC_CAND = 2,
    SC_RETRY = 3,
    SC_HSUM = 4,
    SC_DISP2 = 5,
    SC_NFAIL = 6,
    SC_HCNT = 7,
    SC_GRAV_EPS = 8,
    SC_NFAILQ = 9,
    SC_SHORT = 10,
    SC_FARQ = 11,
    SC_BADHINT = 12,
    SC_CROWDED = 13,
    SC_DENSEP = 14,
    SC_KGDBG = 16,
    SC_NSLOTS = 24
};

enum {
    BAD_ACCEL = 0,
    BAD_ENERGY = 1,
    BAD_STATE = 2,
    BAD_H = 3,
    BADC_BUCKETS = 64, BADC_STRIDE = 16
};
int sphx_badc_read(sphx_ctx* ctx);

int sphx_bbox(sphx_ctx* ctx, int64_t n, const double* x, const double* y, const double* z,
              double out_minmax[13], bool use_clip);
int sphx_median(sphx_ctx* ctx, int64_t n, const double* v, double* out_dev);
int sphx_gravity_launch(sphx_ctx* ctx, int64_t n, const double* x, const double* y, const double* z, int ps,
                        const double* m, const double* eps_dev, double eps, double G, const int* omap,
                        double* acc);
int sphx_gravity_tree_launch(sphx_ctx* ctx, int64_t n, const double* x, const double* y, const double* z,
                             const double* m, int ws, const double* eps_dev, double eps, double G, const int* omap,
                             double* acc);
int sphx_dev_collect(sphx_ctx* ctx);
int sphx_loop_step_sums(sphx_ctx* ctx, int64_t n, int k, double d);
int sphx_build_blob_order(sphx_ctx* ctx, int64_t n, bool defer_scatter = false);
static inline double sphx_cell_feedback(sphx_ctx* ctx, int64_t n) {
    if (ctx->cell_feedback && n > 0) {
        const double dense = (double)ctx->densep_last / (double)n;
        if (dense > ctx->cell_fb_hi) ctx->cell_scale = ctx->cell_scale * 0.97 > 0.35 ? ctx->cell_scale * 0.97 : 0.35;
        else if (dense < ctx->cell_fb_lo) ctx->cell_scale = ctx->cell_scale * 1.01 < 1.0 ? ctx->cell_scale * 1.01 : 1.0;
    }
    return ctx->cell_scale;
}
int sphx_blob_translate(sphx_ctx* ctx, int64_t n, int k);
int sphx_blob_density_species(sphx_ctx* ctx, int64_t n, int k, bool lean, int S, const double* fun, const int* row_of,
                              const double* m_sorted, double* F, double* Z, double* agb, int agb_on);
int sphx_blob_density(sphx_ctx* ctx, int64_t n, int k, bool lean);
int sphx_blob_pi(sphx_ctx* ctx, int64_t n, int k, u64* ct_bits);
int sphx_blob_visc(sphx_ctx* ctx, int64_t n, int k, const double* m);
int sphx_blob_visc_pw(sphx_ctx* ctx, int64_t n, int k, const double* m, u64* ct_bits);
int sphx_blob_species(sphx_ctx* ctx, int64_t n, int k, int S, const double* fun, const int* row_of, const double* m_sorted, double* F,
                      double* Z, double* agb, int agb_on);
struct GridBuildOpts {
    bool lagged = false;
    hipEvent_t alias_ev = nullptr;
    bool sort_cells_later = false;
    double* clamp_vel[3] = {nullptr, nullptr, nullptr};
};
int sphx_build_grid(sphx_ctx* ctx, int64_t n, int k, const double* x, const double* y, const double* z, double cell_hint,
                    const GridBuildOpts& opts = GridBuildOpts());
int sphx_excl_scan_int(sphx_ctx* ctx, const int* in, int* out, int n);
struct alignas(32) DragEntry { u64 key; double x, y, z; };
struct DragScatter { int* cnt; const int* start; DragEntry* ent; };
__device__ __forceinline__ void sphx_drag_put(const DragScatter& sc, int slot, u64 key, double x, double y, double z) {
    double2* q = reinterpret_cast<double2*>(sc.ent + slot);
    q[0] = make_double2(__longlong_as_double((long long)key), x);
    q[1] = make_double2(y, z);
}
int sphx_drag_scatter_plan(sphx_ctx* ctx, int64_t n, int k, const int* nbr, const double* ptype, const int* qorder, DragScatter* out,
                           bool blob = false);
int sphx_drag_scatter_reduce(sphx_ctx* ctx, int64_t n, const DragScatter& d, double* react);
int sphx_blob_drag(sphx_ctx* ctx, int64_t n, int k, bool count_only, const double* m, const double* ptype, const double* mgm,
                   const double* mcs, const int* id, double* onto, const DragScatter& sc);
int sphx_build_outlier_levels(sphx_ctx* ctx, int64_t n, const double* xs, const double* ys, const double* zs);
struct KnnIn {
    const double *xs, *ys, *zs;
    const int32_t* id;
    const int32_t* inv = nullptr;
    const double* rsearch = nullptr;
    double rscale = 1.0, rbound = 0.0;
    bool hinted = false;
    bool hint_by_id = false;
    bool lag_external = false;
};
struct KnnOut {
    int32_t* nbr;
    int32_t* list64 = nullptr;
    double* dref = nullptr;
    double* h_sorted;
    int64_t* idx64;
    double* dist;
    int64_t* nontriv;
    double* h_by_id;
};
int sphx_knn(sphx_ctx* ctx, int64_t n, int k, const KnnIn& in, const KnnOut& out);
struct PrepIn {
    const double *x, *y, *z; int ps;
    const double *vx, *vy, *vz; int vs;
    const double *m, *h, *T, *mu, *gam, *ptype;
    void pos_aos(const double* p) { x = p; y = p + 1; z = p + 2; ps = 3; }
    void vel_aos(const double* v) { vx = v; vy = v + 1; vz = v + 2; vs = 3; }
};
int sphx_prep(sphx_ctx* ctx, int64_t n, const PrepIn& in, bool pairwise, hipStream_t stream);
int sphx_pass_density(sphx_ctx* ctx, int64_t n, int k, bool lean = false);
int sphx_pass_pi(sphx_ctx* ctx, int64_t n, int k, const double* h, const double* ptype);
int sphx_pass_visc(sphx_ctx* ctx, int64_t n, int k, const double* m);
int sphx_pass_visc_pw(sphx_ctx* ctx, int64_t n, int k, const double* m);
int sphx_pass_species(sphx_ctx* ctx, int64_t n, int k, int s, const double* fun, double* F);
int sphx_step_species(sphx_ctx* ctx, int64_t n, int k);
int sphx_species_on(sphx_ctx* ctx, int64_t n, int k, int S, int SP, const double* fun, const int* row_of, const double* m_sorted,
                    double* F, double* Z, double* agb);
int sphx_agb_table_set(sphx_ctx* ctx, int S, int nspl, const int32_t* ntx, const int32_t* nty, const double* tx, const double* ty,
                       const double* coeffs, const int32_t* mapto, double divisor, const double* mu_specie, double solar_mass);
int sphx_transpose_nbr(sphx_ctx* ctx, int64_t n, int k, const int64_t* nb_rowmajor);

int sphx_clamp(sphx_ctx* ctx, int64_t n, StateArrays& s);
int sphx_permute_state(sphx_ctx* ctx, int64_t n, bool split, hipEvent_t after_first);
int sphx_hsum(sphx_ctx* ctx, int64_t n, const double* h, hipStream_t stream);
int sphx_compute_dt(sphx_ctx* ctx, int first, double fixed_dt);
int sphx_integrate(sphx_ctx* ctx, int64_t n, int fold_dt = 0, int first = 0, double fixed_dt = 0.0);
int sphx_pass_drag(sphx_ctx* ctx, int64_t n, int k, const double* m, const double* ptype, const double* mgm,
                   const double* mcs);
int sphx_aos_to_soa3(sphx_ctx* ctx, int64_t n, const double* aos, double* x, double* y, double* z);
int sphx_soa3_to_aos_by_id(sphx_ctx* ctx, int64_t n, const int* id, const double* x, const double* y,
                           const double* z, double* aos);
int sphx_scatter_rows_by_id(sphx_ctx* ctx, int64_t n, int w, const int* id, const double* in, double* out);
int sphx_gather3(sphx_ctx* ctx, int64_t n, const int* perm, const double* x, const double* y,
                 const double* z, double* xs, double* ys, double* zs);
int sphx_iota(sphx_ctx* ctx, int64_t n, int* out);
int sphx_knn_refresh(sphx_ctx* ctx, int64_t n, int k, const double* x, const double* y, const double* z,
                     int32_t* nbr, double* h_sorted, int64_t* nfail_out);
int sphx_save_list_positions(sphx_ctx* ctx, int64_t n, const double* x, const double* y, const double* z);
```

### sph-code_amd/csrc/sphx_loopforms.hip

```cpp
#include "sphx_internal.h"
#include "sphx_pair.h"
#pragma clang fp contract(off)
#include <float.h>

#define PI64 201.06192982974676

__device__ __forceinline__ double pow9(double d) {
    double d2 = d * d, d4 = d2 * d2;
    return d4 * d4 * d;
}
__device__ __forceinline__ double weigh2(double r2, double m, double d, double m0, double d9) {
    const double a = m0 / m;
    const double q = pow(m / m0, 2.0 / 3.0) * (d * d) - r2;
    return m * 315.0 * (a * a * a) * (q * q * q) / (PI64 * d9);
}
__device__ __forceinline__ double weigh2_dust(double r2, double m, double ds) {
    const double q = ds * ds - r2;
    return m * 315.0 * (q * q * q) / (PI64 * pow9(ds));
}
__device__ __forceinline__ double grad_coef(double r2, double m, double d, double m0, double d9, double tk) {
    const double a = m0 / m;
    const double q = pow(m / m0, 2.0 / 3.0) * (d * d) - r2;
    double c = -315.0 * 6.0 * (a * a * a) / (PI64 * d9) * (q * q) * ((tk == 0.0) ? 1.0 : 0.0);
    return (q > 0.0) ? c : 0.0;
// ... 189 lines not shown
    a.out1 = ctx->out_a.as<double>();
    LAUNCH1(loop_density_kernel<0>);
    return down(ctx, out, a.out1, (size_t)n * sizeof(double));
}

extern "C" int sphx_dust_density(sphx_ctx* ctx, int64_t n, int k, const double* points, const double* mass,
                                 const int64_t* neighbor, const double* particle_type,
                                 const double* sizes, double* out) {
    if (!ctx) return SPHX_E_ARG;
    NEED(points); NEED(mass); NEED(particle_type); NEED(sizes); NEED(out);
    LoopArgs a;
    SPHX_TRY(loop_begin(ctx, n, k, neighbor, &a));
    UPF(in_a, points, 3 * n, pos); UPF(in_c, mass, n, m); UPF(in_h, particle_type, n, pt);
    UPF(in_d, sizes, n, h);
    a.d = 1.0;
    SPHX_TRY(sphx_ensure(ctx, ctx->out_a, (size_t)n * sizeof(double)));
    a.out1 = ctx->out_a.as<double>();
    LAUNCH1(loop_density_kernel<1>);
    return down(ctx, out, a.out1, (size_t)n * sizeof(double));
}

extern "C" int sphx_num_dens(sphx_ctx* ctx, int64_t n, int k, const double* mass, const double* points,
                             const double* mu_array, const int64_t* neighbor, double d, double* out) {
    if (!ctx) return SPHX_E_ARG;
    NEED(points); NEED(mass); NEED(mu_array); NEED(out);
    LoopArgs a;
    SPHX_TRY(loop_begin(ctx, n, k, neighbor, &a));
    UPF(in_a, points, 3 * n, pos); UPF(in_c, mass, n, m); UPF(in_f, mu_array, n, mu);
    a.d = d;
    SPHX_TRY(sphx_ensure(ctx, ctx->out_a, (size_t)n * sizeof(double)));
    a.out1 = ctx->out_a.as<double>();
    LAUNCH1(loop_density_kernel<2>);
    return down(ctx, out, a.out1, (size_t)n * sizeof(double));
}

extern "C" int sphx_del_pressure(sphx_ctx* ctx, int64_t n, int k, const double* points, const double* mass,
                                 const double* particle_type, const int64_t* neighbor,
                                 const double* E_internal, const double* gamma_array, double d, double* out) {
    if (!ctx) return SPHX_E_ARG;
    NEED(points); NEED(mass); NEED(particle_type); NEED(E_internal); NEED(gamma_array); NEED(out);
    LoopArgs a;
    SPHX_TRY(loop_begin(ctx, n, k, neighbor, &a));
    UPF(in_a, points, 3 * n, pos); UPF(in_c, mass, n, m); UPF(in_h, particle_type, n, pt);
    UPF(in_e, E_internal, n, E); UPF(in_g, gamma_array, n, gam);
    a.d = d;
    SPHX_TRY(sphx_ensure(ctx, ctx->out_b, (size_t)n * 3 * sizeof(double)));
    a.out3 = ctx->out_b.as<double>();
    LAUNCH1(loop_del_pressure_kernel);
    return down(ctx, out, a.out3, (size_t)n * 3 * sizeof(double));
}

extern "C" int sphx_artificial_viscosity(sphx_ctx* ctx, int64_t n, int k, const int64_t* neighbor,
                                         const double* points, const double* particle_type,
                                         const double* sizes, const double* mass, const double* densities,
                                         const double* velocities, const double* T,
                                         const double* gamma_array, const double* mu_array, double d,
                                         double* visc_accel, double* visc_heat) {
    if (!ctx) return SPHX_E_ARG;
    (void)sizes;
    NEED(points); NEED(mass); NEED(particle_type); NEED(densities); NEED(velocities);
    NEED(T); NEED(gamma_array); NEED(mu_array); NEED(visc_accel); NEED(visc_heat);
    LoopArgs a;
    SPHX_TRY(loop_begin(ctx, n, k, neighbor, &a));
    UPF(in_a, points, 3 * n, pos); UPF(in_b, velocities, 3 * n, vel); UPF(in_c, mass, n, m);
    UPF(in_h, particle_type, n, pt); UPF(in_d, densities, n, rho); UPF(in_e, T, n, T);
    UPF(in_g, gamma_array, n, gam); UPF(in_f, mu_array, n, mu);
    a.d = d;
    SPHX_TRY(sphx_ensure(ctx, ctx->out_a, (size_t)n * sizeof(double)));
    SPHX_TRY(sphx_ensure(ctx, ctx->out_b, (size_t)n * 3 * sizeof(double)));
    a.out1 = ctx->out_a.as<double>(); a.out3 = ctx->out_b.as<double>();
    LAUNCH1(loop_av_kernel);
    SPHX_TRY(down(ctx, visc_accel, a.out3, (size_t)n * 3 * sizeof(double)));
    return down(ctx, visc_heat, a.out1, (size_t)n * sizeof(double));
}

extern "C" int sphx_crossing_time(sphx_ctx* ctx, int64_t n, int k, const int64_t* neighbor,
                                  const double* velocities, const double* sizes,
                                  const double* particle_type, double* out) {
    if (!ctx) return SPHX_E_ARG;
    NEED(velocities); NEED(sizes); NEED(particle_type); NEED(out);
    LoopArgs a;
    SPHX_TRY(loop_begin(ctx, n, k, neighbor, &a));
    UPF(in_b, velocities, 3 * n, vel); UPF(in_d, sizes, n, h); UPF(in_h, particle_type, n, pt);
    a.ct_bits = ctx->scal.as<u64>() + SC_CT_BITS;
    SPHX_TRY(sphx_prime_ct(ctx, a.ct_bits));
    ctx->ct_primed = false;
    LAUNCH1(loop_ct_kernel);
    u64 bits = 0;
    SPHX_TRY(down(ctx, &bits, a.ct_bits, sizeof(u64)));
    if (bits == SPHX_CT_NONE) {
        *out = ctx->cst.dt_0 / 10.0;
    } else {
        double v;
        memcpy(&v, &bits, 8);
        *out = v + 0.0001;
    }
    return SPHX_OK;
}

extern "C" int sphx_net_impulse(sphx_ctx* ctx, int64_t n, int k, const double* points, const double* mass,
                                const double* sizes, const double* velocities, const double* particle_type,
                                const int64_t* neighbor, const double* mean_grain_mass,
                                const double* mean_cross, double* accel_onto, double* accel_reaction) {
    if (!ctx) return SPHX_E_ARG;
    NEED(points); NEED(mass); NEED(sizes); NEED(velocities); NEED(particle_type);
    NEED(mean_grain_mass); NEED(mean_cross); NEED(accel_onto); NEED(accel_reaction);
    LoopArgs a;
    SPHX_TRY(loop_begin(ctx, n, k, neighbor, &a));
    UPF(in_a, points, 3 * n, pos); UPF(in_b, velocities, 3 * n, vel); UPF(in_c, mass, n, m);
    UPF(in_h, particle_type, n, pt); UPF(in_d, sizes, n, h); UPF(in_e, mean_grain_mass, n, mgm);
    UPF(in_f, mean_cross, n, mcs);
    SPHX_TRY(sphx_ensure(ctx, ctx->out_b, (size_t)n * 3 * sizeof(double)));
    SPHX_TRY(sphx_ensure(ctx, ctx->out_c, (size_t)n * 3 * sizeof(double)));
    a.out3 = ctx->out_b.as<double>(); a.out3b = ctx->out_c.as<double>();
    DragScatter sc;
    SPHX_TRY(sphx_drag_scatter_plan(ctx, n, k, a.nbr, a.pt, nullptr, &sc));
    hipLaunchKernelGGL(loop_impulse_kernel, dim3((unsigned)((n + 255) / 256)), dim3(256), 0, ctx->stream, a, sc);
    HIPCHK(hipGetLastError());
    SPHX_TRY(sphx_drag_scatter_reduce(ctx, n, sc, a.out3b));
    SPHX_TRY(down(ctx, accel_onto, a.out3, (size_t)n * 3 * sizeof(double)));
    return down(ctx, accel_reaction, a.out3b, (size_t)n * 3 * sizeof(double));
}

#include "sphx_blob.h"
struct RecP1 { double x, y, z, hq, w1, g1, muns, E; };
struct RecP2 { double x, y, z, css, vx, vy, vz, rho; };

struct LoopPrepArgs {
    int n;
    const double *x, *y, *z, *vx, *vy, *vz, *m, *pt, *mu, *gam, *E, *T;
    double d, m0, m_h, kB, amu;
    RecP1* p1; RecP2* p2;
};
__global__ __launch_bounds__(256) void loop_prep_kernel(LoopPrepArgs a) {
    const int i = blockIdx.x * blockDim.x + threadIdx.x;
    if (i >= a.n) return;
    const double m = a.m[i], d9 = pow9(a.d);
    const double aa = a.m0 / m;
    const bool gas = (a.pt[i] == 0.0);
    RecP1 r;
    r.x = a.x[i]; r.y = a.y[i]; r.z = a.z[i];
    r.hq = pow(m / a.m0, 2.0 / 3.0) * (a.d * a.d);
    r.w1 = m * 315.0 * (aa * aa * aa);
    r.g1 = -315.0 * 6.0 * (aa * aa * aa) / (PI64 * d9);
    const double mun = a.mu[i] * a.m_h;
    r.muns = gas ? mun : -mun;
    r.E = a.E[i];
    a.p1[i] = r;
    RecP2 v;
    v.x = r.x; v.y = r.y; v.z = r.z;
    const double cs = sphx_nan_to_num(sqrt(a.gam[i] * a.kB * a.T[i] / (a.mu[i] * a.amu)));
    v.css = gas ? cs : -(cs + 1.0);
    v.vx = a.vx[i]; v.vy = a.vy[i]; v.vz = a.vz[i];
    v.rho = 0.0;
    a.p2[i] = v;
}

struct L1Acc { double rho, rd, n, gx, gy, gz; };
__device__ __forceinline__ void loop1_term(L1Acc& a, const Q4& q0, const Q4& q1, double gam_j, double dm, double dh,
                                           double xi, double yi, double zi, double Ei, bool gas_i, double d9) {
    const double dx = q0.a - xi, dy = q0.b - yi, dz = q0.c - zi;
    const double r2 = dx * dx + dy * dy + dz * dz;
    const double q = q0.d - r2;
    const double w = q1.a * (q * q * q) / (PI64 * d9);
    const bool gas_j = q1.c > 0.0;
    const double vr = w * (gas_j ? 1.0 : 0.0);
    if (vr > 0.0) a.rho += vr;
    const double vn = w / fabs(q1.c);
    if (vn > 0.0) a.n += vn;
// ... 268 lines not shown
        }
        __syncthreads();
    }
    block_min_vote<PASS_T>(mine, ct_bits);
}

static int loop_prep_launch(sphx_ctx* ctx, int64_t n, double d, StateArrays& st) {
    const size_t nb = (size_t)n * sizeof(double);
    DevBuf* outs[] = {&ctx->rho, &ctx->rhod, &ctx->nden, &ctx->vh};
    for (DevBuf* b : outs) SPHX_TRY(sphx_ensure(ctx, *b, nb));
    SPHX_TRY(sphx_ensure(ctx, ctx->G, 3 * nb));
    SPHX_TRY(sphx_ensure(ctx, ctx->va, 3 * nb));
    SPHX_TRY(sphx_ensure(ctx, ctx->lrec_a, (size_t)n * sizeof(RecP1)));
    SPHX_TRY(sphx_ensure(ctx, ctx->lrec_v, (size_t)n * sizeof(RecP2)));
    LoopPrepArgs p;
    p.n = (int)n;
    p.x = st.x.as<double>(); p.y = st.y.as<double>(); p.z = st.z.as<double>();
    p.vx = st.vx.as<double>(); p.vy = st.vy.as<double>(); p.vz = st.vz.as<double>();
    p.m = st.m.as<double>(); p.pt = st.ptype.as<double>();
    p.mu = st.mu.as<double>(); p.gam = st.gam.as<double>(); p.E = st.E.as<double>(); p.T = st.T.as<double>();
    p.d = d; p.m0 = ctx->cst.m_0; p.m_h = ctx->cst.m_h; p.kB = ctx->cst.k_B; p.amu = ctx->cst.amu;
    p.p1 = ctx->lrec_a.as<RecP1>(); p.p2 = ctx->lrec_v.as<RecP2>();
    hipLaunchKernelGGL(loop_prep_kernel, dim3((unsigned)((n + 255) / 256)), dim3(256), 0, ctx->stream, p);
    HIPCHK(hipGetLastError());
    return SPHX_OK;
}
__global__ __launch_bounds__(256) void loop_dust_side_kernel(int n, const double* __restrict__ pt, const double* __restrict__ m,
                                                             const double* __restrict__ h, const double* __restrict__ gam,
                                                             RecP1* p1, double* side) {
    const int i = blockIdx.x * blockDim.x + threadIdx.x;
    if (i >= n) return;
    const double t = pt[i];
    if (t == 0.0) { side[i] = gam[i]; return; }
    if (t == 2.0) { side[i] = m[i]; p1[i].g1 = h[i]; }
    else side[i] = -1.0;
}
static int loop_pass1_launch(sphx_ctx* ctx, int64_t n, int k, double d, StateArrays& st, const double* h) {
    const double d2 = d * d, d4 = d2 * d2, d9 = d4 * d4 * d;
    const int npad = (int)sphx_pad64(n);
    RecP1* p1 = ctx->lrec_a.as<RecP1>(); RecP2* p2 = ctx->lrec_v.as<RecP2>();
    if (ctx->qorder && ctx->blob_lists) {
        SPHX_TRY(sphx_lds_opt_in(ctx, reinterpret_cast<const void*>(blob_loop1_kernel), IMG_BYTES(72, SPHX_MAX_K)));
        const int nblk = (npad + BLOB_P - 1) / BLOB_P;
        const int g = sphx_blob_grid(ctx, nblk);
        SPHX_TRY(sphx_ensure(ctx, ctx->loop_side, (size_t)n * sizeof(double)));
        hipLaunchKernelGGL(loop_dust_side_kernel, dim3((unsigned)((n + 255) / 256)), dim3(256), 0, ctx->stream, (int)n,
                           st.ptype.as<double>(), st.m.as<double>(), h, st.gam.as<double>(), p1, ctx->loop_side.as<double>());
        hipLaunchKernelGGL(blob_loop1_kernel, dim3(g), dim3(PASS_T), IMG_BYTES(72, k), ctx->stream, (int)n, npad, k, nblk,
                           d9, ctx->nbr.as<int>(), ctx->slot16.as<u16>(), ctx->uniq.as<int>(), ctx->qorder, p1,
                           ctx->loop_side.as<double>(),
                           ctx->rho.as<double>(), ctx->rhod.as<double>(), ctx->nden.as<double>(), ctx->G.as<double>(), p2,
                           sphx_blob_sel(ctx, 0));
    } else {
        hipLaunchKernelGGL(loop_pass1_kernel, dim3((unsigned)((n + 255) / 256)), dim3(256), 0, ctx->stream, (int)n, npad, k, d9,
                           ctx->nbr.as<int>(), p1, st.gam.as<double>(), st.ptype.as<double>(), st.m.as<double>(),
                           h, ctx->qorder, ctx->rho.as<double>(), ctx->rhod.as<double>(),
                           ctx->nden.as<double>(), ctx->G.as<double>(), p2);
    }
    HIPCHK(hipGetLastError());
    return SPHX_OK;
}
static int loop_pass2_launch(sphx_ctx* ctx, int64_t n, int k, StateArrays& st, const double* h, u64* ct, int part = 0) {
    const int npad = (int)sphx_pad64(n);
    RecP1* p1 = ctx->lrec_a.as<RecP1>(); RecP2* p2 = ctx->lrec_v.as<RecP2>();
    if (ctx->qorder && ctx->blob_lists) {
        SPHX_TRY(sphx_lds_opt_in(ctx, reinterpret_cast<const void*>(blob_loop2_kernel), IMG_BYTES(72, SPHX_MAX_K)));
        const int nblk = (npad + BLOB_P - 1) / BLOB_P;
        const int g = sphx_blob_grid(ctx, nblk);
        hipLaunchKernelGGL(blob_loop2_kernel, dim3(g), dim3(PASS_T), IMG_BYTES(72, k), ctx->stream, (int)n, npad, k, nblk,
                           ctx->nbr.as<int>(), ctx->slot16.as<u16>(), ctx->uniq.as<int>(), ctx->qorder, p1, p2,
                           st.m.as<double>(), h, ctx->va.as<double>(), ctx->vh.as<double>(), ct, sphx_blob_sel(ctx, part));
    } else {
        hipLaunchKernelGGL(loop_pass2_kernel, dim3((unsigned)((n + 255) / 256)), dim3(256), 0, ctx->stream, (int)n, npad, k,
                           ctx->nbr.as<int>(), p1, p2, st.m.as<double>(), h, ctx->qorder, ctx->va.as<double>(),
                           ctx->vh.as<double>(), ct);
    }
    HIPCHK(hipGetLastError());
    return SPHX_OK;
}

int sphx_loop_step_sums(sphx_ctx* ctx, int64_t n, int k, double d) {
    StateArrays& st = ctx->st;
    SPHX_TRY(loop_prep_launch(ctx, n, d, st));
    u64* ct = ctx->scal.as<u64>() + SC_CT_BITS;
    if (!ctx->ct_primed) SPHX_TRY(sphx_prime_ct(ctx, ct));
    ctx->ct_primed = false;
    SPHX_TRY(loop_pass1_launch(ctx, n, k, d, st, st.hprev.as<double>()));
    SPHX_TRY(loop_pass2_launch(ctx, n, k, st, st.hprev.as<double>(), ct));
    return SPHX_OK;
}

struct DevGatherArgs {
    int n;
    const int* perm;
    const double *pos, *vel, *m, *T, *mu, *gam, *pt, *E;
    double *x, *y, *z, *vx, *vy, *vz, *sm, *sT, *smu, *sgam, *spt, *sE;
};
__global__ __launch_bounds__(256) void dev_gather_state_kernel(DevGatherArgs a) {
    const int s = blockIdx.x * blockDim.x + threadIdx.x;
    if (s >= a.n) return;
    const size_t c = (size_t)a.perm[s];
    a.x[s] = a.pos[3 * c]; a.y[s] = a.pos[3 * c + 1]; a.z[s] = a.pos[3 * c + 2];
    a.vx[s] = a.vel[3 * c]; a.vy[s] = a.vel[3 * c + 1]; a.vz[s] = a.vel[3 * c + 2];
    a.sm[s] = a.m[c]; a.sT[s] = a.T[c]; a.smu[s] = a.mu[c]; a.sgam[s] = a.gam[c]; a.spt[s] = a.pt[c]; a.sE[s] = a.E[c];
}
__global__ __launch_bounds__(256) void dev_to_sorted_kernel(int n, const int* perm, int n_active, int owned_only,
                                                            const double* src, double* dst) {
    const int s = blockIdx.x * blockDim.x + threadIdx.x;
    if (s >= n) return;
    const int c = perm[s];
    dst[s] = (owned_only && c >= n_active) ? 0.0 : src[c];
}
__global__ __launch_bounds__(256) void dev_rho_to_records_kernel(int n, const int* perm, const double* rho, RecP2* p2) {
    const int s = blockIdx.x * blockDim.x + threadIdx.x;
    if (s < n) p2[s].rho = rho[perm[s]];
}
__global__ __launch_bounds__(256) void dev_to_caller_kernel(int n, const int* perm, int n_active, int w,
                                                            const double* src, double* dst) {
    const int s = blockIdx.x * blockDim.x + threadIdx.x;
    if (s >= n) return;
    const int c = perm[s];
    if (c >= n_active) return;
    for (int q = 0; q < w; ++q) dst[(size_t)c * w + q] = src[(size_t)s * w + q];
}

extern "C" int sphx_dev_loop_prep(sphx_ctx* ctx, const double* pos, const double* vel, const double* mass,
                                  const double* T, const double* mu, const double* gamma, const double* ptype,
                                  const double* E_internal, double d) {
    if (!ctx) return SPHX_E_ARG;
    NEED(pos); NEED(vel); NEED(mass); NEED(T); NEED(mu); NEED(gamma); NEED(ptype); NEED(E_internal);
    if (!ctx->map_perm) return sphx_set_err(ctx, SPHX_E_STATE, "sphx_dev_loop_prep before sphx_dev_search");
    if (!(d > 0.0)) return sphx_set_err(ctx, SPHX_E_ARG, "sphx_dev_loop_prep: d must be positive");
    HIPCHK(hipSetDevice(ctx->device));
    const int64_t n = ctx->n;
    StateArrays& st = ctx->alt;
    DevBuf* bufs[] = {&st.x, &st.y, &st.z, &st.vx, &st.vy, &st.vz, &st.m, &st.T, &st.mu, &st.gam, &st.ptype, &st.E,
                      &st.hprev, &st.ax};
    for (DevBuf* b : bufs) SPHX_TRY(sphx_ensure(ctx, *b, (size_t)n * sizeof(double)));
    DevGatherArgs g;
    g.n = (int)n; g.perm = ctx->map_perm;
    g.pos = pos; g.vel = vel; g.m = mass; g.T = T; g.mu = mu; g.gam = gamma; g.pt = ptype; g.E = E_internal;
    g.x = st.x.as<double>(); g.y = st.y.as<double>(); g.z = st.z.as<double>();
    g.vx = st.vx.as<double>(); g.vy = st.vy.as<double>(); g.vz = st.vz.as<double>();
    g.sm = st.m.as<double>(); g.sT = st.T.as<double>(); g.smu = st.mu.as<double>(); g.sgam = st.gam.as<double>();
    g.spt = st.ptype.as<double>(); g.sE = st.E.as<double>();
    hipLaunchKernelGGL(dev_gather_state_kernel, dim3((unsigned)((n + 255) / 256)), dim3(256), 0, ctx->stream, g);
    HIPCHK(hipGetLastError());
    ctx->loop_d = d;
    return loop_prep_launch(ctx, n, d, st);
}

extern "C" int sphx_dev_loop_pass1(sphx_ctx* ctx, const double* h_complete, double* rho, double* rho_dust, double* nden,
                                   double* delp) {
    if (!ctx) return SPHX_E_ARG;
    NEED(h_complete);
    if (!ctx->map_perm || !(ctx->loop_d > 0.0)) return sphx_set_err(ctx, SPHX_E_STATE, "sphx_dev_loop_pass1 before sphx_dev_loop_prep");
    HIPCHK(hipSetDevice(ctx->device));
    const int64_t n = ctx->n;
    const unsigned grid = (unsigned)((n + 255) / 256);
    StateArrays& st = ctx->alt;
    hipLaunchKernelGGL(dev_to_sorted_kernel, dim3(grid), dim3(256), 0, ctx->stream, (int)n, ctx->map_perm, ctx->map_nactive, 0,
                       h_complete, st.hprev.as<double>());
    hipLaunchKernelGGL(dev_to_sorted_kernel, dim3(grid), dim3(256), 0, ctx->stream, (int)n, ctx->map_perm, ctx->map_nactive, 1,
                       h_complete, st.ax.as<double>());
    SPHX_TRY(loop_pass1_launch(ctx, n, ctx->k, ctx->loop_d, st, st.hprev.as<double>()));
    struct O { double* dst; const double* src; int w; } outs[] = {{rho, ctx->rho.as<double>(), 1}, {rho_dust, ctx->rhod.as<double>(), 1},
                                                                   {nden, ctx->nden.as<double>(), 1}, {delp, ctx->G.as<double>(), 3}};
    for (O& o : outs)
        if (o.dst)
            hipLaunchKernelGGL(dev_to_caller_kernel, dim3(grid), dim3(256), 0, ctx->stream, (int)n, ctx->map_perm,
                               ctx->map_nactive, o.w, o.src, o.dst);
    HIPCHK(hipGetLastError());
    return SPHX_OK;
}

extern "C" int sphx_dev_loop_pass2_interior(sphx_ctx* ctx) {
    if (!ctx) return SPHX_E_ARG;
    if (!ctx->map_perm || !(ctx->loop_d > 0.0))
        return sphx_set_err(ctx, SPHX_E_STATE, "sphx_dev_loop_pass2_interior before sphx_dev_loop_pass1");
    ctx->loop2_interior_done = false;
    if (!(ctx->qorder && ctx->blob_lists && ctx->blob_split_valid)) return 0;
    HIPCHK(hipSetDevice(ctx->device));
    u64* ct = ctx->scal.as<u64>() + SC_CT_BITS;
    SPHX_TRY(sphx_prime_ct(ctx, ct));
    ctx->ct_primed = false;
    SPHX_TRY(loop_pass2_launch(ctx, ctx->n, ctx->k, ctx->alt, ctx->alt.ax.as<double>(), ct, 1));
    ctx->loop2_interior_done = true;
    return 1;
}

extern "C" int sphx_dev_loop_pass2(sphx_ctx* ctx, const double* rho_complete, double* visc_accel, double* visc_heat,
                                   double* ct_out) {
    if (!ctx) return SPHX_E_ARG;
    NEED(rho_complete);
    if (!ctx->map_perm || !(ctx->loop_d > 0.0)) return sphx_set_err(ctx, SPHX_E_STATE, "sphx_dev_loop_pass2 before sphx_dev_loop_prep");
    HIPCHK(hipSetDevice(ctx->device));
    const int64_t n = ctx->n;
    const unsigned grid = (unsigned)((n + 255) / 256);
    StateArrays& st = ctx->alt;
    hipLaunchKernelGGL(dev_rho_to_records_kernel, dim3(grid), dim3(256), 0, ctx->stream, (int)n, ctx->map_perm, rho_complete,
                       ctx->lrec_v.as<RecP2>());
    u64* ct = ctx->scal.as<u64>() + SC_CT_BITS;
    const bool rest_only = ctx->loop2_interior_done;
    ctx->loop2_interior_done = false;
    if (!rest_only) SPHX_TRY(sphx_prime_ct(ctx, ct));
    ctx->ct_primed = false;
    SPHX_TRY(loop_pass2_launch(ctx, n, ctx->k, st, st.ax.as<double>(), ct, rest_only ? 2 : 0));
    if (visc_accel)
        hipLaunchKernelGGL(dev_to_caller_kernel, dim3(grid), dim3(256), 0, ctx->stream, (int)n, ctx->map_perm, ctx->map_nactive,
                           3, ctx->va.as<double>(), visc_accel);
    if (visc_heat)
        hipLaunchKernelGGL(dev_to_caller_kernel, dim3(grid), dim3(256), 0, ctx->stream, (int)n, ctx->map_perm, ctx->map_nactive,
                           1, ctx->vh.as<double>(), visc_heat);
    HIPCHK(hipGetLastError());
    if (ct_out)
        HIPCHK(hipMemcpyAsync(ct_out, ct, 8, hipMemcpyDeviceToDevice, ctx->stream));
    return SPHX_OK;
}
```

### sph-code_amd/csrc/sphx_sums.hip

```cpp
#include "sphx_internal.h"
#include "sphx_wave.h"
#include "sphx_pair.h"
#pragma clang fp contract(off)
#include <float.h>
#include <stdlib.h>

struct PrepArgs {
    int n;
    const double *x, *y, *z; int ps;
    const double *vx, *vy, *vz; int vs;
    const double *m, *h, *T, *mu, *gam, *ptype;
    double kB, amu;
    RecA* ra; RecB* rb; RecBC* bc; RecSelf* self;
    const int* perm;
    int which, n_active;
    int pairwise;
};

__global__ __launch_bounds__(256) void prep_kernel(PrepArgs a) {
    const int t = blockIdx.x * blockDim.x + threadIdx.x;
    if (t >= a.n) return;
    const int i = a.perm ? a.perm[t] : t;
    if (a.which && ((i < a.n_active) != (a.which == 1))) return;
    const double m = a.m[i], h = a.h[i], T = a.T[i], mu = a.mu[i], gam = a.gam[i], pt = a.ptype[i];
// ... 106 lines not shown
        if (jb[u] < 0) continue;
        density_term<SqrtLib>(acc[u & (SPHX_SUM_PARTS - 1)], q0b[u], q1b[u], xr, yr, zr, hi2, ci, Ai, clip != 0);
      }
    }
    const double s_rho = parts_total(acc, &DensAcc::rho), s_rd = parts_total(acc, &DensAcc::rd), s_n = parts_total(acc, &DensAcc::n);
    const double gx = parts_total(acc, &DensAcc::gx), gy = parts_total(acc, &DensAcc::gy), gz = parts_total(acc, &DensAcc::gz);
    rho[o] = s_rho; rhod[o] = s_rd; nden[o] = s_n;
    rho_s[i] = s_rho;
    if (G) { G[3 * (size_t)o + 0] = -gx; G[3 * (size_t)o + 1] = -gy; G[3 * (size_t)o + 2] = -gz; }
    ha[3 * (size_t)o + 0] = -gx / s_rho;
    ha[3 * (size_t)o + 1] = -gy / s_rho;
    ha[3 * (size_t)o + 2] = -gz / s_rho;
}

int sphx_pass_density(sphx_ctx* ctx, int64_t n, int k, bool lean) {
    SPHX_TRY(sphx_ensure(ctx, ctx->rho, (size_t)n * sizeof(double)));
    SPHX_TRY(sphx_ensure(ctx, ctx->rhod, (size_t)n * sizeof(double)));
    SPHX_TRY(sphx_ensure(ctx, ctx->nden, (size_t)n * sizeof(double)));
    SPHX_TRY(sphx_ensure(ctx, ctx->G, (size_t)n * 3 * sizeof(double)));
    SPHX_TRY(sphx_ensure(ctx, ctx->ha, (size_t)n * 3 * sizeof(double)));
    if (ctx->qorder && ctx->blob_lists) return sphx_blob_density(ctx, n, k, lean);
    hipLaunchKernelGGL(pass_density_kernel, dim3((unsigned)((n + 255) / 256)), dim3(256), 0, ctx->stream,
                       (int)n, (int)sphx_pad64(n), k, ctx->clip_grad, ctx->nbr.as<int>(), ctx->rec1.as<RecA>(),
                       ctx->rho_s.as<double>(), ctx->qorder, OutMap{ctx->map_perm, ctx->map_perm ? ctx->map_nactive : (int)n},
                       ctx->rho.as<double>(), ctx->rhod.as<double>(), ctx->nden.as<double>(),
                       lean ? nullptr : ctx->G.as<double>(), ctx->ha.as<double>());
    HIPCHK(hipGetLastError());
    return SPHX_OK;
}

__global__ __launch_bounds__(256) void pass_pi_kernel(int n, int npad, int k, const int* __restrict__ nbr,
                                                      const RecB* __restrict__ recb,
                                                      const double* __restrict__ rho_s,
                                                      const RecSelf* __restrict__ selfr, RecBC* bc,
                                                      const int* __restrict__ qorder, OutMap om, double* Pi, double* BwOut,
                                                      u64* ct_bits) {
    const int p = xcd_block(blockIdx.x, gridDim.x) * blockDim.x + threadIdx.x;
    u64 my_ct = SPHX_CT_NONE;
    const int i = (p < n) ? (qorder ? qorder[p] : p) : n;
    const int o = (i < n) ? out_index(om, i) : 0x7FFFFFFF;
    if (i < n && o < om.n_active) {
        int j0 = nbr[p];
        if (j0 < 0) j0 = i;
        const double* rq = reinterpret_cast<const double*>(&recb[j0]);
        const Q4 r0 = gload4(rq), rv = gload4(rq + 4);
        const RecSelf sf = selfr[i];
        const double rho_i = rho_s[i], cs_i = sf.csi, ms_i = sf.mg, h_i = sf.h;
        double a_pi[SPHX_SUM_PARTS] = {}, maxrel = 0.0;
        for (int kk0 = 0; kk0 < k; kk0 += NBATCH) {
          int jb[NBATCH];
          Q4 q0b[NBATCH], qvb[NBATCH];
          double rhob[NBATCH];
#pragma unroll
          for (int u = 0; u < NBATCH; ++u) jb[u] = (kk0 + u < k) ? nbr[(size_t)(kk0 + u) * npad + p] : -1;
#pragma unroll
          for (int u = 0; u < NBATCH; ++u) {
              const int jj = jb[u] < 0 ? i : jb[u];
              const double* qb = reinterpret_cast<const double*>(&recb[jj]);
              q0b[u] = gload4(qb); qvb[u] = gload4(qb + 4);
              rhob[u] = rho_s[jj];
          }
#pragma unroll
          for (int u = 0; u < NBATCH; ++u) {
            if (jb[u] < 0) continue;
            const PiPair t = pi_term<SqrtLib>(q0b[u], qvb[u], rhob[u], r0, rv, rho_i, cs_i);
            a_pi[u & (SPHX_SUM_PARTS - 1)] += t.pi;
            maxrel = fmax(maxrel, t.rel);
          }
        }
        const double s_pi = parts_total(a_pi);
        Pi[o] = s_pi;
        const double bw = fmax(ms_i, 0.0) * s_pi;
        bc[i].Bw = bw;
        if (BwOut) BwOut[o] = bw;
        if (ms_i > 0.0) my_ct = ct_vote_bits(h_i, maxrel);
    }
    block_min_vote<256>(my_ct, ct_bits);
}

int sphx_pass_pi(sphx_ctx* ctx, int64_t n, int k, const double* h, const double* ptype) {
    (void)ptype; (void)h;
    SPHX_TRY(sphx_ensure(ctx, ctx->Pi, (size_t)n * sizeof(double)));
    SPHX_TRY(sphx_ensure(ctx, ctx->Bw, (size_t)n * sizeof(double)));
    u64* ct = ctx->scal.as<u64>() + SC_CT_BITS;
    if (!ctx->ct_primed) SPHX_TRY(sphx_prime_ct(ctx, ct));
    ctx->ct_primed = false;
    if (ctx->qorder && ctx->blob_lists) return sphx_blob_pi(ctx, n, k, ct);
    hipLaunchKernelGGL(pass_pi_kernel, dim3((unsigned)((n + 255) / 256)), dim3(256), 0, ctx->stream,
                       (int)n, (int)sphx_pad64(n), k, ctx->nbr.as<int>(), ctx->recv.as<RecB>(),
                       ctx->rho_s.as<double>(), ctx->self_s.as<RecSelf>(), ctx->bc_s.as<RecBC>(), ctx->qorder,
                       OutMap{ctx->map_perm, ctx->map_perm ? ctx->map_nactive : (int)n},
                       ctx->Pi.as<double>(), ctx->map_perm ? ctx->Bw.as<double>() : nullptr, ct);
    HIPCHK(hipGetLastError());
    return SPHX_OK;
}

__global__ __launch_bounds__(256) void pass_visc_kernel(int n, int npad, int k, int clip,
                                                        const int* __restrict__ nbr,
                                                        const RecB* __restrict__ recb,
                                                        const RecBC* __restrict__ bc,
                                                        const int* __restrict__ qorder, OutMap om,
                                                        const double* __restrict__ m, double* va,
                                                        double* vh) {
    const int p = xcd_block(blockIdx.x, gridDim.x) * blockDim.x + threadIdx.x;
    if (p >= n) return;
    const int i = qorder ? qorder[p] : p;
    const int o = out_index(om, i);
    if (o >= om.n_active) return;
    int j0 = nbr[p];
    if (j0 < 0) j0 = i;
    const double* rq = reinterpret_cast<const double*>(&recb[j0]);
    const Q4 r0 = gload4(rq), rv = gload4(rq + 4);
    const double2 bci = *reinterpret_cast<const double2*>(&bc[i]);
    const double hi2 = recb[i].h2, ci = -6.0 * bci.y, Bi = bci.x;
    ViscAcc acc[SPHX_SUM_PARTS] = {};
    for (int kk0 = 0; kk0 < k; kk0 += NBATCH) {
      int jb[NBATCH];
      Q4 q0b[NBATCH], qvb[NBATCH];
      double2 bcb[NBATCH];
#pragma unroll
      for (int u = 0; u < NBATCH; ++u) jb[u] = (kk0 + u < k) ? nbr[(size_t)(kk0 + u) * npad + p] : -1;
#pragma unroll
      for (int u = 0; u < NBATCH; ++u) {
          const int jj = jb[u] < 0 ? i : jb[u];
          const double* qb = reinterpret_cast<const double*>(&recb[jj]);
          q0b[u] = gload4(qb); qvb[u] = gload4(qb + 4);
          bcb[u] = *reinterpret_cast<const double2*>(&bc[jj]);
      }
#pragma unroll
      for (int u = 0; u < NBATCH; ++u) {
        if (jb[u] < 0) continue;
        visc_term<SqrtLib>(acc[u & (SPHX_SUM_PARTS - 1)], q0b[u], qvb[u], bcb[u].x, bcb[u].y, r0, rv, hi2, ci, Bi, clip != 0);
      }
    }
    const double ax = parts_total(acc, &ViscAcc::x), ay = parts_total(acc, &ViscAcc::y), az = parts_total(acc, &ViscAcc::z);
    const double heat = parts_total(acc, &ViscAcc::h);
    va[3 * (size_t)o + 0] = -ax; va[3 * (size_t)o + 1] = -ay; va[3 * (size_t)o + 2] = -az;
    vh[o] = heat * m[o] / 2.0;
}

int sphx_pass_visc(sphx_ctx* ctx, int64_t n, int k, const double* m) {
    SPHX_TRY(sphx_ensure(ctx, ctx->va, (size_t)n * 3 * sizeof(double)));
    SPHX_TRY(sphx_ensure(ctx, ctx->vh, (size_t)n * sizeof(double)));
    if (ctx->qorder && ctx->blob_lists) return sphx_blob_visc(ctx, n, k, m);
    hipLaunchKernelGGL(pass_visc_kernel, dim3((unsigned)((n + 255) / 256)), dim3(256), 0, ctx->stream,
                       (int)n, (int)sphx_pad64(n), k, ctx->clip_grad, ctx->nbr.as<int>(), ctx->recv.as<RecB>(),
                       ctx->bc_s.as<RecBC>(), ctx->qorder,
                       OutMap{ctx->map_perm, ctx->map_perm ? ctx->map_nactive : (int)n}, m,
                       ctx->va.as<double>(), ctx->vh.as<double>());
    HIPCHK(hipGetLastError());
    return SPHX_OK;
}

__global__ __launch_bounds__(256) void pass_visc_pw_kernel(int n, int npad, int k, int clip,
                                                           const int* __restrict__ nbr,
                                                           const RecB* __restrict__ recb,
                                                           const double* __restrict__ rho_s,
                                                           const RecBC* __restrict__ bc,
                                                           const RecSelf* __restrict__ selfr,
                                                           const int* __restrict__ qorder, OutMap om,
                                                           const double* __restrict__ m, double* va, double* vh,
                                                           u64* ct_bits) {
    const int p = xcd_block(blockIdx.x, gridDim.x) * blockDim.x + threadIdx.x;
    u64 my_ct = SPHX_CT_NONE;
    const int i = (p < n) ? (qorder ? qorder[p] : p) : n;
    const int o = (i < n) ? out_index(om, i) : 0x7FFFFFFF;
    if (i < n && o < om.n_active) {
        int j0 = nbr[p];
        if (j0 < 0) j0 = i;
        const double* rq = reinterpret_cast<const double*>(&recb[j0]);
        const Q4 r0 = gload4(rq), rv = gload4(rq + 4);
        const RecSelf sf = selfr[i];
        const double rho_i = rho_s[i], cs_i = sf.csi, h_i = sf.h;
        const double hi2 = recb[i].h2, ci = -6.0 * bc[i].Bw;
        ViscAcc acc[SPHX_SUM_PARTS] = {};
        double maxrel = 0.0;
        for (int kk0 = 0; kk0 < k; kk0 += NBATCH) {
          int jb[NBATCH];
          Q4 q0b[NBATCH], qvb[NBATCH];
          double rhob[NBATCH], mcb[NBATCH];
#pragma unroll
          for (int u = 0; u < NBATCH; ++u) jb[u] = (kk0 + u < k) ? nbr[(size_t)(kk0 + u) * npad + p] : -1;
#pragma unroll
          for (int u = 0; u < NBATCH; ++u) {
              const int jj = jb[u] < 0 ? i : jb[u];
              const double* qb = reinterpret_cast<const double*>(&recb[jj]);
              q0b[u] = gload4(qb); qvb[u] = gload4(qb + 4);
              rhob[u] = rho_s[jj];
              mcb[u] = bc[jj].Bw;
          }
#pragma unroll
          for (int u = 0; u < NBATCH; ++u) {
            if (jb[u] < 0) continue;
            maxrel = fmax(maxrel, visc_pw_term<SqrtLib>(acc[u & (SPHX_SUM_PARTS - 1)], q0b[u], qvb[u], rhob[u], mcb[u], r0, rv,
                                                         rho_i, cs_i, hi2, ci, clip != 0));
          }
        }
        const double ax = parts_total(acc, &ViscAcc::x), ay = parts_total(acc, &ViscAcc::y), az = parts_total(acc, &ViscAcc::z);
        const double heat = parts_total(acc, &ViscAcc::h);
        va[3 * (size_t)o + 0] = -ax; va[3 * (size_t)o + 1] = -ay; va[3 * (size_t)o + 2] = -az;
        vh[o] = heat * m[o] / 2.0;
        if (sf.mg > 0.0) my_ct = ct_vote_bits(h_i, maxrel);
    }
    block_min_vote<256>(my_ct, ct_bits);
}

int sphx_pass_visc_pw(sphx_ctx* ctx, int64_t n, int k, const double* m) {
    SPHX_TRY(sphx_ensure(ctx, ctx->va, (size_t)n * 3 * sizeof(double)));
    SPHX_TRY(sphx_ensure(ctx, ctx->vh, (size_t)n * sizeof(double)));
    u64* ct = ctx->scal.as<u64>() + SC_CT_BITS;
    if (!ctx->ct_primed) SPHX_TRY(sphx_prime_ct(ctx, ct));
    ctx->ct_primed = false;
    if (ctx->qorder && ctx->blob_lists) return sphx_blob_visc_pw(ctx, n, k, m, ct);
    hipLaunchKernelGGL(pass_visc_pw_kernel, dim3((unsigned)((n + 255) / 256)), dim3(256), 0, ctx->stream,
                       (int)n, (int)sphx_pad64(n), k, ctx->clip_grad, ctx->nbr.as<int>(), ctx->recv.as<RecB>(),
                       ctx->rho_s.as<double>(), ctx->bc_s.as<RecBC>(), ctx->self_s.as<RecSelf>(), ctx->qorder,
                       OutMap{ctx->map_perm, ctx->map_perm ? ctx->map_nactive : (int)n}, m,
                       ctx->va.as<double>(), ctx->vh.as<double>(), ct);
    HIPCHK(hipGetLastError());
    return SPHX_OK;
}

__global__ __launch_bounds__(256) void drag_count_kernel(int n, int npad, int k, const int* __restrict__ nbr,
                                                         const double* __restrict__ ptype, const int* __restrict__ qorder,
                                                         int* cnt) {
    const int p = blockIdx.x * blockDim.x + threadIdx.x;
    if (p >= n) return;
    const int i = qorder ? qorder[p] : p;
    for (int kk = 0; kk < k; ++kk) {
        const int j = nbr[(size_t)kk * npad + p];
        if (j >= 0 && j != i && ptype[j] == 2.0) atomicAdd(&cnt[j], 1);
    }
}
#define DRAG_RED_BLOCKS 2048
#define DRAG_RED_U 4
template <int U>
__device__ __forceinline__ void drag_slice_sum(int s, int L, const DragEntry* __restrict__ ent,
                                               double* pk, int lane, double& acc) {
    u64 key[U];
    double vx[U], vy[U], vz[U];
    int rank[U];
#pragma unroll
    for (int u = 0; u < U; ++u) {
        const int q = lane + 64 * u;
        key[u] = ~0ull; vx[u] = vy[u] = vz[u] = 0.0;
        if (q < L) {
            const double2* e = reinterpret_cast<const double2*>(ent + s + q);
            const double2 e0 = e[0], e1 = e[1];
            key[u] = (u64)__double_as_longlong(e0.x); vx[u] = e0.y; vy[u] = e1.x; vz[u] = e1.y;
        }
        rank[u] = 0;
    }
#pragma unroll
    for (int c = 0; c < U; ++c) {
        const int lc = L - 64 * c < 64 ? L - 64 * c : 64;
        for (int t = 0; t < lc; ++t) {
            const u64 kt = ((u64)(unsigned)__builtin_amdgcn_readlane((int)(key[c] >> 32), t) << 32) |
                           (u64)(unsigned)__builtin_amdgcn_readlane((int)key[c], t);
#pragma unroll
            for (int u = 0; u < U; ++u) rank[u] += kt < key[u] ? 1 : 0;
        }
    }
#pragma unroll
    for (int u = 0; u < U; ++u) {
        const int q = lane + 64 * u;
        if (q < L) { pk[3 * rank[u]] = vx[u]; pk[3 * rank[u] + 1] = vy[u]; pk[3 * rank[u] + 2] = vz[u]; }
    }
    wave_sync();
    if (lane < 3) {
        int t = 0;
        for (; t + 8 <= L; t += 8) {
            double v[8];
#pragma unroll
            for (int q = 0; q < 8; ++q) v[q] = pk[3 * (t + q) + lane];
#pragma unroll
            for (int q = 0; q < 8; ++q) acc += v[q];
        }
        for (; t < L; ++t) acc += pk[3 * t + lane];
    }
    wave_sync();
}
__global__ __launch_bounds__(256) void drag_reduce_kernel(int n, const int* __restrict__ start,
                                                          const DragEntry* __restrict__ ent, double* react) {
    __shared__ double parked[4][64 * DRAG_RED_U * 3];
    const int lane = threadIdx.x & 63, wave = threadIdx.x >> 6;
    double* pk = parked[wave];
    for (int j0 = (blockIdx.x * 4 + wave) * 64; j0 < n; j0 += gridDim.x * 4 * 64) {
        const int jl = j0 + lane;
        int sl = 0, Ll = 0;
        if (jl < n) { sl = start[jl]; Ll = start[jl + 1] - sl; }
        if (jl < n && Ll == 0) { react[3 * (size_t)jl] = 0.0; react[3 * (size_t)jl + 1] = 0.0; react[3 * (size_t)jl + 2] = 0.0; }
        u64 todo = __builtin_amdgcn_ballot_w64(Ll > 0);
        while (todo) {
            const int t = __builtin_ctzll(todo);
            todo &= todo - 1;
// ... 232 lines not shown
```

Before: 826.4 million.

## Defer leapfrog integrate into next step's fused grid-count kernel

```diff
diff --git a/sph-code_amd/csrc/sphx_api.hip b/sph-code_amd/csrc/sphx_api.hip
--- a/sph-code_amd/csrc/sphx_api.hip
+++ b/sph-code_amd/csrc/sphx_api.hip
@@ -381,7 +381,8 @@
     }
     HIPCHK(hipMemsetAsync(ctx->scal.p, 0, SC_NSLOTS * 8, ctx->stream));
     HIPCHK(hipMemsetAsync(ctx->badc.p, 0, (size_t)BADC_BUCKETS * BADC_STRIDE * sizeof(u64), ctx->stream));
-    ctx->ct_primed = false;
+    sphx_ct_unprimed_all(ctx);
+    ctx->upd_pending.on = false;
     ctx->nbr_api_valid = false;
     HIPCHK(hipStreamSynchronize(ctx->stream));
     ctx->n = n;
@@ -499,6 +500,16 @@
 
 static int step_search(sphx_ctx* ctx, int k, double dist, hipEvent_t* ev) {
     const int64_t n = ctx->n;
+    IntegArgs upd;
+    const bool upd_pending = ctx->upd_pending.on;
+    if (upd_pending) {
+        ctx->upd_pending.on = false;
+        SPHX_TRY(sphx_integrate_args(ctx, n, 1, ctx->upd_pending.first, ctx->upd_pending.fixed_dt, ctx->upd_pending.ct_slot, &upd));
+        if (ctx->use_verlet) {
+            SPHX_TRY(sphx_integrate_launch(ctx, upd));
+            sphx_integrate_done(ctx);
+        }
+    }
     if (ctx->use_verlet) SPHX_TRY(sphx_clamp(ctx, n, ctx->st));
     SPHX_TRY(sphx_ensure(ctx, ctx->nbr, (size_t)k * ctx->npad * sizeof(int)));
     if (ctx->use_verlet && ctx->list_valid && ctx->list_n == n && ctx->list_k == k) {
@@ -523,6 +534,7 @@
         g.alias_ev = ev[1];
         g.sort_cells_later = blob;
         if (!ctx->use_verlet) { g.clamp_vel[0] = r.vx.as<double>(); g.clamp_vel[1] = r.vy.as<double>(); g.clamp_vel[2] = r.vz.as<double>(); }
+        if (upd_pending && !ctx->use_verlet) g.update = &upd;
         SPHX_TRY(sphx_build_grid(ctx, n, k, r.x.as<double>(), r.y.as<double>(), r.z.as<double>(), cell_hint, g));
         if (blob) SPHX_TRY(sphx_build_blob_order(ctx, n, true));
     }
@@ -634,7 +646,8 @@
     return SPHX_OK;
 }
 
-static int one_step(sphx_ctx* ctx, int k, double dist, int first, double fixed_dt, bool call_first, bool call_last) {
+static int one_step(sphx_ctx* ctx, int k, double dist, int first, double fixed_dt, bool call_first, bool call_last,
+                    bool may_defer) {
     const int64_t n = ctx->n;
     const int ring = (int)(ctx->step_count % 3);
     hipEvent_t* ev = ctx->evring[ring];
@@ -667,7 +680,14 @@
                                               ctx->grav.as<double>()));
     }
     if (detail) HIPCHK(hipEventRecord(ev[8], ctx->stream));
-    SPHX_TRY(sphx_integrate(ctx, n, 1, first, fixed_dt));
+    if (may_defer && !ctx->use_verlet && !detail) {
+        ctx->upd_pending.on = true;
+        ctx->upd_pending.first = first;
+        ctx->upd_pending.fixed_dt = fixed_dt;
+        ctx->upd_pending.ct_slot = sphx_ct_slot(ctx);
+    } else {
+        SPHX_TRY(sphx_integrate(ctx, n, 1, first, fixed_dt));
+    }
     if (rec7) HIPCHK(hipEventRecord(ev[7], ctx->stream));
     ctx->step_count++;
     return SPHX_OK;
@@ -722,12 +742,13 @@
     HIPCHK(hipSetDevice(ctx->device));
     if (!(dist > 0.0) || !isfinite(dist)) dist = 0.0;
     ctx->k = k;
+    ctx->upd_pending.on = false;
     const bool per_call = !ctx->timing_detail;
     if (per_call) HIPCHK(hipEventRecord(ctx->ev[8], ctx->stream));
     for (int it = 0; it < nsteps; ++it) {
         const int ring = (int)(ctx->step_count % 3);
         SPHX_TRY(collect_stats(ctx, ring));
-        SPHX_TRY(one_step(ctx, k, dist, first && it == 0, fixed_dt, false, false));
+        SPHX_TRY(one_step(ctx, k, dist, first && it == 0, fixed_dt, false, false, it + 1 < nsteps));
         ctx->ev_pending |= 1u << ring;
         SPHX_TRY(collect_stats(ctx, (ring + 1) % 3));
     }
diff --git a/sph-code_amd/csrc/sphx_dev.hip b/sph-code_amd/csrc/sphx_dev.hip
--- a/sph-code_amd/csrc/sphx_dev.hip
+++ b/sph-code_amd/csrc/sphx_dev.hip
@@ -187,13 +187,13 @@
         hipLaunchKernelGGL(inject_field_kernel, dim3((unsigned)((n + 255) / 256)), dim3(256), 0, ctx->stream, (int)n,
                            ctx->map_perm, rho_complete, ctx->rho_s.as<double>(), 1);
     HIPCHK(hipGetLastError());
-    if (ctx->pass_part == 2) ctx->ct_primed = true;
+    if (ctx->pass_part == 2) sphx_ct_set_primed(ctx, sphx_ct_slot(ctx));
     {
         Borrow b1(ctx->Pi, Pi, (size_t)n * sizeof(double)), b2(ctx->Bw, Bw, (size_t)n * sizeof(double));
         SPHX_TRY(sphx_pass_pi(ctx, n, ctx->k, nullptr, nullptr));
     }
     if (ct_out)
-        HIPCHK(hipMemcpyAsync(ct_out, ctx->scal.as<u64>() + SC_CT_BITS, 8, hipMemcpyDeviceToDevice, ctx->stream));
+        HIPCHK(hipMemcpyAsync(ct_out, sphx_ct_bits(ctx, sphx_ct_slot(ctx)), 8, hipMemcpyDeviceToDevice, ctx->stream));
     return SPHX_OK;
 }
 
@@ -228,13 +228,13 @@
         hipLaunchKernelGGL(inject_field_kernel, dim3((unsigned)((n + 255) / 256)), dim3(256), 0, ctx->stream, (int)n,
                            ctx->map_perm, rho_complete, ctx->rho_s.as<double>(), 1);
     HIPCHK(hipGetLastError());
-    if (ctx->pass_part == 2) ctx->ct_primed = true;
+    if (ctx->pass_part == 2) sphx_ct_set_primed(ctx, sphx_ct_slot(ctx));
     {
         Borrow b1(ctx->va, visc_accel, 3 * (size_t)n * sizeof(double)), b2(ctx->vh, visc_heat, (size_t)n * sizeof(double));
         SPHX_TRY(sphx_pass_visc_pw(ctx, n, ctx->k, mass));
     }
     if (ct_out)
-        HIPCHK(hipMemcpyAsync(ct_out, ctx->scal.as<u64>() + SC_CT_BITS, 8, hipMemcpyDeviceToDevice, ctx->stream));
+        HIPCHK(hipMemcpyAsync(ct_out, sphx_ct_bits(ctx, sphx_ct_slot(ctx)), 8, hipMemcpyDeviceToDevice, ctx->stream));
     return SPHX_OK;
 }
 
diff --git a/sph-code_amd/csrc/sphx_grid.hip b/sph-code_amd/csrc/sphx_grid.hip
--- a/sph-code_amd/csrc/sphx_grid.hip
+++ b/sph-code_amd/csrc/sphx_grid.hip
@@ -1,6 +1,9 @@
 #include "sphx_internal.h"
 #include <rocprim/rocprim.hpp>
 #include <float.h>
+#pragma clang fp contract(off)
+#include "sphx_update.h"
+#pragma clang fp contract(fast)
 
 #define RED_BLOCK 256
 #define RED_MAXBLOCKS 1024
@@ -186,7 +189,9 @@
     u64* ct_reset;
     int* zero_int;
     int* rank;
+    IntegArgs upd;
 };
+template <bool UPD>
 __global__ __launch_bounds__(RED_BLOCK) void grid_count_fused(FusedCountArgs a) {
     __shared__ double sm[RED_BLOCK / 64][BB_W];
     double mn[3] = {INFINITY, INFINITY, INFINITY}, mx[3] = {-INFINITY, -INFINITY, -INFINITY};
@@ -195,8 +200,18 @@
     const double piv[3] = {a.clip.pivot[0], a.clip.pivot[1], a.clip.pivot[2]};
     if (a.ct_reset && blockIdx.x == 0 && threadIdx.x == 0) *a.ct_reset = SPHX_CT_NONE;
     if (a.zero_int && blockIdx.x == 0 && threadIdx.x == 0) { a.zero_int[0] = 0; a.zero_int[1] = 0; }
+    double dt = 0.0;
+    if (UPD) {
+        dt = sphx_update_dt(a.upd);
+        if (a.upd.ct_bits && blockIdx.x == 0 && threadIdx.x == 0) *a.upd.dt_out = dt;
+    }
     for (int i = blockIdx.x * blockDim.x + threadIdx.x; i < a.n; i += gridDim.x * blockDim.x) {
-        double v[3] = {a.x[i], a.y[i], a.z[i]};
+        double v[3], w[3];
+        if (UPD) {
+            sphx_update_particle(a.upd, i, dt, v, w);
+        } else {
+            v[0] = a.x[i]; v[1] = a.y[i]; v[2] = a.z[i];
+        }
         if (a.vx) {
             const double o0 = v[0], o1 = v[1], o2 = v[2];
 #pragma unroll
@@ -209,7 +224,8 @@
             if (__double_as_longlong(v[0]) != __double_as_longlong(o0)) a.x[i] = v[0];
             if (__double_as_longlong(v[1]) != __double_as_longlong(o1)) a.y[i] = v[1];
             if (__double_as_longlong(v[2]) != __double_as_longlong(o2)) a.z[i] = v[2];
-            const double w0 = a.vx[i], w1 = a.vy[i], w2 = a.vz[i];
+            if (!UPD) { w[0] = a.vx[i]; w[1] = a.vy[i]; w[2] = a.vz[i]; }
+            const double w0 = w[0], w1 = w[1], w2 = w[2];
             const double u0 = sphx_nan_to_num(w0), u1 = sphx_nan_to_num(w1), u2 = sphx_nan_to_num(w2);
             if (__double_as_longlong(u0) != __double_as_longlong(w0)) a.vx[i] = u0;
             if (__double_as_longlong(u1) != __double_as_longlong(w1)) a.vy[i] = u1;
@@ -553,7 +569,13 @@
                     const GridBuildOpts& opts) {
     double bb[13], rel[9];
     bool clamp_pending = opts.clamp_vel[0] != nullptr;
+    bool update_pending = opts.update != nullptr;
     auto clamp_now = [&]() -> int {
+        if (update_pending) {
+            update_pending = false;
+            SPHX_TRY(sphx_integrate_launch(ctx, *opts.update));
+            sphx_integrate_done(ctx);
+        }
         if (!clamp_pending) return SPHX_OK;
         clamp_pending = false;
         return sphx_clamp(ctx, n, ctx->st);
@@ -689,7 +711,8 @@
         fa.cell_of = ctx->cell_of.as<int>();
         fa.hist = fill;
         fa.partial = part; fa.ticket = ticket; fa.fin = fin;
-        fa.ct_reset = ctx->scal.as<u64>() + SC_CT_BITS;
+        const int ct_slot = sphx_ct_slot(ctx);
+        fa.ct_reset = sphx_ct_bits(ctx, ct_slot);
         fa.zero_int = nullptr;
         SPHX_TRY(sphx_ensure(ctx, ctx->cell_rank, (size_t)n * sizeof(int)));
         fa.rank = ctx->cell_rank.as<int>();
@@ -699,9 +722,21 @@
             ctx->fcount_zeroed = ctx->fail_list.p;
             ctx->fcount_zeroed_n = n;
         }
-        ctx->ct_primed = true;
+        sphx_ct_set_primed(ctx, ct_slot);
         int fb = pb < FUSED_MAXBLOCKS ? pb : FUSED_MAXBLOCKS;
-        hipLaunchKernelGGL(grid_count_fused, dim3(fb), dim3(RED_BLOCK), 0, ctx->stream, fa);
+        const bool upd_here = update_pending && fa.vx && opts.update->n == fa.n && opts.update->x == fa.x && opts.update->y == fa.y &&
+                              opts.update->z == fa.z && opts.update->vx == fa.vx && opts.update->vy == fa.vy &&
+                              opts.update->vz == fa.vz && opts.update->ct_bits != fa.ct_reset;
+        if (update_pending && !upd_here) SPHX_TRY(clamp_now());
+        if (upd_here) {
+            update_pending = false;
+            fa.upd = *opts.update;
+            hipLaunchKernelGGL(grid_count_fused<true>, dim3(fb), dim3(RED_BLOCK), 0, ctx->stream, fa);
+            sphx_integrate_done(ctx);
+        } else {
+            memset(&fa.upd, 0, sizeof(fa.upd));
+            hipLaunchKernelGGL(grid_count_fused<false>, dim3(fb), dim3(RED_BLOCK), 0, ctx->stream, fa);
+        }
         HIPCHK(hipGetLastError());
         if (pb >= BB_W) {
             bb_fold_blocks = fb; bb_fold_part = part; bb_fold_out = fin;
diff --git a/sph-code_amd/csrc/sphx_integrate.hip b/sph-code_amd/csrc/sphx_integrate.hip
--- a/sph-code_amd/csrc/sphx_integrate.hip
+++ b/sph-code_amd/csrc/sphx_integrate.hip
@@ -2,7 +2,7 @@
 #pragma clang fp contract(off)
 #include <float.h>
 
-#include "sphx_leapfrog.h"
+#include "sphx_update.h"
 #define nan_to_num sphx_nan_to_num
 
 __global__ __launch_bounds__(256) void clamp_kernel(int n, double lim, double* x, double* y, double* z,
@@ -203,101 +203,27 @@
 }
 
 int sphx_compute_dt(sphx_ctx* ctx, int first, double fixed_dt) {
-    hipLaunchKernelGGL(dt_kernel, dim3(1), dim3(64), 0, ctx->stream, ctx->scal.as<u64>() + SC_CT_BITS,
+    const int slot = sphx_ct_slot(ctx);
+    hipLaunchKernelGGL(dt_kernel, dim3(1), dim3(64), 0, ctx->stream, sphx_ct_bits(ctx, slot),
                        ctx->scal.as<double>() + SC_DT, first, fixed_dt, ctx->cst.dt_0, ctx->cst.max_age);
     HIPCHK(hipGetLastError());
-    ctx->ct_primed = true;
-    return SPHX_OK;
-}
-
-struct IntegArgs {
-    int n;
-    double *x, *y, *z, *vx, *vy, *vz, *ax, *ay, *az;
-    double *E, *T;
-    const double *m, *mu, *gam, *ptype;
-    const double *ha, *va, *vh;
-    const double *rho, *rhod, *drag_on, *drag_re;
-    const double* grav;
-    const double* G;
-    const double* dt;
-    double m_h, kB;
-    int no_old;
-    const u64* ct_bits;
-    double* dt_out;
-    int first;
-    double fixed_dt, dt_0, max_age;
-    u64* counters;
-};
+    sphx_ct_set_primed(ctx, slot);
+    return SPHX_OK;
+}
+
 __global__ __launch_bounds__(256) void integrate_kernel(IntegArgs a) {
     int i = blockIdx.x * blockDim.x + threadIdx.x;
     if (i >= a.n) return;
-    double dt;
-    if (a.ct_bits) {
-        if (a.fixed_dt > 0.0) {
-            dt = a.fixed_dt;
-        } else {
-            const u64 b = *a.ct_bits;
-            const double ct = sphx_ct_value(b == SPHX_CT_NONE, __longlong_as_double((long long)b), a.dt_0);
-            dt = sphx_dt_rule(ct, a.first, a.dt_0, a.max_age);
-        }
-        if (i == 0) *a.dt_out = dt;
-    } else {
-        dt = *a.dt;
-    }
-    const double g = (a.ptype[i] == 0.0) ? 1.0 : 0.0;
-    const double v[3] = {a.vx[i], a.vy[i], a.vz[i]};
-    double pa[3], vis[3];
-    bool bad_acc = false;
-#pragma unroll
-    for (int c = 0; c < 3; ++c) {
-        if (a.G) {
-            const double praw = a.G[3 * (size_t)i + c] / a.rho[i] * g;
-            pa[c] = nan_to_num(praw);
-            vis[c] = a.va[3 * (size_t)i + c];
-            bad_acc = bad_acc || !sphx_finite(praw) || !sphx_finite(vis[c]);
-        } else {
-            const double praw = -a.ha[3 * (size_t)i + c] * g, vraw = -a.va[3 * (size_t)i + c] * g;
-            pa[c] = nan_to_num(praw);
-            vis[c] = nan_to_num(vraw);
-            bad_acc = bad_acc || !sphx_finite(praw) || !sphx_finite(vraw);
-        }
-        if (a.drag_on) {
-            const double draw = a.drag_on[3 * (size_t)i + c] * a.rhod[i] / a.rho[i] * g, rraw = a.drag_re[3 * (size_t)i + c];
-            const double dg = nan_to_num(draw);
-            vis[c] = dg + nan_to_num(rraw) + vis[c];
-            bad_acc = bad_acc || !sphx_finite(draw) || !sphx_finite(rraw);
-        }
-    }
-    double x[3] = {a.x[i], a.y[i], a.z[i]};
-    double vv[3] = {v[0], v[1], v[2]};
-    double gr[3], old[3], tot[3];
-#pragma unroll
-    for (int c = 0; c < 3; ++c) gr[c] = a.grav ? a.grav[3 * (size_t)i + c] : 0.0;
-    old[0] = a.ax[i]; old[1] = a.ay[i]; old[2] = a.az[i];
-    sphx_leapfrog_update(dt, x, vv, vis, pa, a.grav ? gr : nullptr, a.no_old ? nullptr : old, tot);
-    a.x[i] = x[0]; a.y[i] = x[1]; a.z[i] = x[2];
-    a.vx[i] = vv[0]; a.vy[i] = vv[1]; a.vz[i] = vv[2];
-    a.ax[i] = tot[0]; a.ay[i] = tot[1]; a.az[i] = tot[2];
-    double E = a.E[i], T;
-    const double heat = a.vh[i];
-    const bool bad_en = !sphx_finite(E) || !sphx_finite(heat * dt);
-    sphx_energy_update(dt, heat, a.mu[i], a.gam[i], a.m[i], a.m_h, a.kB, E, T);
-    a.E[i] = E;
-    a.T[i] = T;
-    if (a.counters) {
-        bool bad_st = false;
-#pragma unroll
-        for (int c = 0; c < 3; ++c) bad_st = bad_st || !sphx_finite(x[c]) || !sphx_finite(vv[c]);
-        sphx_count_bad(a.counters, BAD_ACCEL, bad_acc);
-        sphx_count_bad(a.counters, BAD_ENERGY, bad_en);
-        sphx_count_bad(a.counters, BAD_STATE, bad_st);
-    }
-}
-
-int sphx_integrate(sphx_ctx* ctx, int64_t n, int fold_dt, int first, double fixed_dt) {
+    const double dt = sphx_update_dt(a);
+    if (a.ct_bits && i == 0) *a.dt_out = dt;
+    double x[3], v[3];
+    sphx_update_particle(a, i, dt, x, v);
+}
+
+int sphx_integrate_args(sphx_ctx* ctx, int64_t n, int fold_dt, int first, double fixed_dt, int ct_slot, IntegArgs* out) {
     StateArrays& s = ctx->st;
-    IntegArgs a;
-    a.ct_bits = fold_dt ? ctx->scal.as<u64>() + SC_CT_BITS : nullptr;
+    IntegArgs& a = *out;
+    a.ct_bits = fold_dt ? sphx_ct_bits(ctx, ct_slot) : nullptr;
     a.dt_out = ctx->scal.as<double>() + SC_DT;
     a.first = first; a.fixed_dt = fixed_dt; a.dt_0 = ctx->cst.dt_0; a.max_age = ctx->cst.max_age;
     a.n = (int)n;
@@ -318,10 +244,23 @@
     a.m_h = ctx->cst.m_h; a.kB = ctx->cst.k_B;
     a.no_old = 0;
     a.counters = ctx->badc.as<u64>();
-    hipLaunchKernelGGL(integrate_kernel, dim3((unsigned)((n + 255) / 256)), dim3(256), 0, ctx->stream, a);
-    HIPCHK(hipGetLastError());
-    { DevBuf t = s.T; s.T = ctx->alt.T; ctx->alt.T = t; }
+    return SPHX_OK;
+}
+int sphx_integrate_launch(sphx_ctx* ctx, const IntegArgs& a) {
+    hipLaunchKernelGGL(integrate_kernel, dim3((unsigned)((a.n + 255) / 256)), dim3(256), 0, ctx->stream, a);
+    HIPCHK(hipGetLastError());
+    return SPHX_OK;
+}
+void sphx_integrate_done(sphx_ctx* ctx) {
+    { DevBuf t = ctx->st.T; ctx->st.T = ctx->alt.T; ctx->alt.T = t; }
     ctx->tprev_valid = true;
+}
+
+int sphx_integrate(sphx_ctx* ctx, int64_t n, int fold_dt, int first, double fixed_dt) {
+    IntegArgs a;
+    SPHX_TRY(sphx_integrate_args(ctx, n, fold_dt, first, fixed_dt, sphx_ct_slot(ctx), &a));
+    SPHX_TRY(sphx_integrate_launch(ctx, a));
+    sphx_integrate_done(ctx);
     return SPHX_OK;
 }
 
diff --git a/sph-code_amd/csrc/sphx_internal.h b/sph-code_amd/csrc/sphx_internal.h
--- a/sph-code_amd/csrc/sphx_internal.h
+++ b/sph-code_amd/csrc/sphx_internal.h
@@ -168,7 +168,8 @@
     int64_t step_count = 0;
     double dt_last = 0.0;
     bool tprev_valid = false;
-    bool ct_primed = false;
+    bool ct_primed[2] = {false, false};
+    struct { bool on = false; int first = 0; double fixed_dt = 0.0; int ct_slot = 0; } upd_pending;
     bool recs_pw = false;
     bool nbr_api_valid = false;
     int64_t nbr_api_n = 0;
@@ -340,8 +341,21 @@
     SC_CROWDED = 13,
     SC_DENSEP = 14,
     SC_KGDBG = 16,
-    SC_NSLOTS = 24
-};
+    SC_CT_BITS1 = 24,
+    SC_NSLOTS = 25
+};
+
+static inline int sphx_ct_slot(const sphx_ctx* ctx) { return (int)(ctx->step_count & 1); }
+static inline u64* sphx_ct_bits(sphx_ctx* ctx, int slot) { return ctx->scal.as<u64>() + (slot ? SC_CT_BITS1 : SC_CT_BITS); }
+static inline void sphx_ct_set_primed(sphx_ctx* ctx, int slot) { ctx->ct_primed[slot] = true; }
+static inline void sphx_ct_unprimed_all(sphx_ctx* ctx) { ctx->ct_primed[0] = ctx->ct_primed[1] = false; }
+static inline int sphx_ct_open(sphx_ctx* ctx, u64** ct, bool always = false) {
+    const int slot = sphx_ct_slot(ctx);
+    *ct = sphx_ct_bits(ctx, slot);
+    const bool primed = ctx->ct_primed[slot] && !always;
+    ctx->ct_primed[slot] = false;
+    return primed ? SPHX_OK : sphx_prime_ct(ctx, *ct);
+}
 
 enum {
     BAD_ACCEL = 0,
@@ -381,11 +395,13 @@
 int sphx_blob_visc_pw(sphx_ctx* ctx, int64_t n, int k, const double* m, u64* ct_bits);
 int sphx_blob_species(sphx_ctx* ctx, int64_t n, int k, int S, const double* fun, const int* row_of, const double* m_sorted, double* F,
                       double* Z, double* agb, int agb_on);
+struct IntegArgs;
 struct GridBuildOpts {
     bool lagged = false;
     hipEvent_t alias_ev = nullptr;
     bool sort_cells_later = false;
     double* clamp_vel[3] = {nullptr, nullptr, nullptr};
+    const IntegArgs* update = nullptr;
 };
 int sphx_build_grid(sphx_ctx* ctx, int64_t n, int k, const double* x, const double* y, const double* z, double cell_hint,
                     const GridBuildOpts& opts = GridBuildOpts());
@@ -449,6 +465,27 @@
 int sphx_hsum(sphx_ctx* ctx, int64_t n, const double* h, hipStream_t stream);
 int sphx_compute_dt(sphx_ctx* ctx, int first, double fixed_dt);
 int sphx_integrate(sphx_ctx* ctx, int64_t n, int fold_dt = 0, int first = 0, double fixed_dt = 0.0);
+struct IntegArgs {
+    int n;
+    double *x, *y, *z, *vx, *vy, *vz, *ax, *ay, *az;
+    double *E, *T;
+    const double *m, *mu, *gam, *ptype;
+    const double *ha, *va, *vh;
+    const double *rho, *rhod, *drag_on, *drag_re;
+    const double* grav;
+    const double* G;
+    const double* dt;
+    double m_h, kB;
+    int no_old;
+    const u64* ct_bits;
+    double* dt_out;
+    int first;
+    double fixed_dt, dt_0, max_age;
+    u64* counters;
+};
+int sphx_integrate_args(sphx_ctx* ctx, int64_t n, int fold_dt, int first, double fixed_dt, int ct_slot, IntegArgs* out);
+int sphx_integrate_launch(sphx_ctx* ctx, const IntegArgs& a);
+void sphx_integrate_done(sphx_ctx* ctx);
 int sphx_pass_drag(sphx_ctx* ctx, int64_t n, int k, const double* m, const double* ptype, const double* mgm,
                    const double* mcs);
 int sphx_aos_to_soa3(sphx_ctx* ctx, int64_t n, const double* aos, double* x, double* y, double* z);
diff --git a/sph-code_amd/csrc/sphx_loopforms.hip b/sph-code_amd/csrc/sphx_loopforms.hip
--- a/sph-code_amd/csrc/sphx_loopforms.hip
+++ b/sph-code_amd/csrc/sphx_loopforms.hip
@@ -295,9 +295,7 @@
     LoopArgs a;
     SPHX_TRY(loop_begin(ctx, n, k, neighbor, &a));
     UPF(in_b, velocities, 3 * n, vel); UPF(in_d, sizes, n, h); UPF(in_h, particle_type, n, pt);
-    a.ct_bits = ctx->scal.as<u64>() + SC_CT_BITS;
-    SPHX_TRY(sphx_prime_ct(ctx, a.ct_bits));
-    ctx->ct_primed = false;
+    SPHX_TRY(sphx_ct_open(ctx, &a.ct_bits, true));
     LAUNCH1(loop_ct_kernel);
     u64 bits = 0;
     SPHX_TRY(down(ctx, &bits, a.ct_bits, sizeof(u64)));
@@ -732,9 +730,8 @@
 int sphx_loop_step_sums(sphx_ctx* ctx, int64_t n, int k, double d) {
     StateArrays& st = ctx->st;
     SPHX_TRY(loop_prep_launch(ctx, n, d, st));
-    u64* ct = ctx->scal.as<u64>() + SC_CT_BITS;
-    if (!ctx->ct_primed) SPHX_TRY(sphx_prime_ct(ctx, ct));
-    ctx->ct_primed = false;
+    u64* ct;
+    SPHX_TRY(sphx_ct_open(ctx, &ct));
     SPHX_TRY(loop_pass1_launch(ctx, n, k, d, st, st.hprev.as<double>()));
     SPHX_TRY(loop_pass2_launch(ctx, n, k, st, st.hprev.as<double>(), ct));
     return SPHX_OK;
@@ -831,9 +828,8 @@
     ctx->loop2_interior_done = false;
     if (!(ctx->qorder && ctx->blob_lists && ctx->blob_split_valid)) return 0;
     HIPCHK(hipSetDevice(ctx->device));
-    u64* ct = ctx->scal.as<u64>() + SC_CT_BITS;
-    SPHX_TRY(sphx_prime_ct(ctx, ct));
-    ctx->ct_primed = false;
+    u64* ct;
+    SPHX_TRY(sphx_ct_open(ctx, &ct, true));
     SPHX_TRY(loop_pass2_launch(ctx, ctx->n, ctx->k, ctx->alt, ctx->alt.ax.as<double>(), ct, 1));
     ctx->loop2_interior_done = true;
     return 1;
@@ -850,11 +846,11 @@
     StateArrays& st = ctx->alt;
     hipLaunchKernelGGL(dev_rho_to_records_kernel, dim3(grid), dim3(256), 0, ctx->stream, (int)n, ctx->map_perm, rho_complete,
                        ctx->lrec_v.as<RecP2>());
-    u64* ct = ctx->scal.as<u64>() + SC_CT_BITS;
     const bool rest_only = ctx->loop2_interior_done;
     ctx->loop2_interior_done = false;
-    if (!rest_only) SPHX_TRY(sphx_prime_ct(ctx, ct));
-    ctx->ct_primed = false;
+    u64* ct;
+    if (rest_only) sphx_ct_set_primed(ctx, sphx_ct_slot(ctx));
+    SPHX_TRY(sphx_ct_open(ctx, &ct, !rest_only));
     SPHX_TRY(loop_pass2_launch(ctx, n, ctx->k, st, st.ax.as<double>(), ct, rest_only ? 2 : 0));
     if (visc_accel)
         hipLaunchKernelGGL(dev_to_caller_kernel, dim3(grid), dim3(256), 0, ctx->stream, (int)n, ctx->map_perm, ctx->map_nactive,
diff --git a/sph-code_amd/csrc/sphx_sums.hip b/sph-code_amd/csrc/sphx_sums.hip
--- a/sph-code_amd/csrc/sphx_sums.hip
+++ b/sph-code_amd/csrc/sphx_sums.hip
@@ -212,9 +212,8 @@
     (void)ptype; (void)h;
     SPHX_TRY(sphx_ensure(ctx, ctx->Pi, (size_t)n * sizeof(double)));
     SPHX_TRY(sphx_ensure(ctx, ctx->Bw, (size_t)n * sizeof(double)));
-    u64* ct = ctx->scal.as<u64>() + SC_CT_BITS;
-    if (!ctx->ct_primed) SPHX_TRY(sphx_prime_ct(ctx, ct));
-    ctx->ct_primed = false;
+    u64* ct;
+    SPHX_TRY(sphx_ct_open(ctx, &ct));
     if (ctx->qorder && ctx->blob_lists) return sphx_blob_pi(ctx, n, k, ct);
     hipLaunchKernelGGL(pass_pi_kernel, dim3((unsigned)((n + 255) / 256)), dim3(256), 0, ctx->stream,
                        (int)n, (int)sphx_pad64(n), k, ctx->nbr.as<int>(), ctx->recv.as<RecB>(),
@@ -338,9 +337,8 @@
 int sphx_pass_visc_pw(sphx_ctx* ctx, int64_t n, int k, const double* m) {
     SPHX_TRY(sphx_ensure(ctx, ctx->va, (size_t)n * 3 * sizeof(double)));
     SPHX_TRY(sphx_ensure(ctx, ctx->vh, (size_t)n * sizeof(double)));
-    u64* ct = ctx->scal.as<u64>() + SC_CT_BITS;
-    if (!ctx->ct_primed) SPHX_TRY(sphx_prime_ct(ctx, ct));
-    ctx->ct_primed = false;
+    u64* ct;
+    SPHX_TRY(sphx_ct_open(ctx, &ct));
     if (ctx->qorder && ctx->blob_lists) return sphx_blob_visc_pw(ctx, n, k, m, ct);
     hipLaunchKernelGGL(pass_visc_pw_kernel, dim3((unsigned)((n + 255) / 256)), dim3(256), 0, ctx->stream,
                        (int)n, (int)sphx_pad64(n), k, ctx->clip_grad, ctx->nbr.as<int>(), ctx->recv.as<RecB>(),
diff --git a/sph-code_amd/csrc/sphx_update.h b/sph-code_amd/csrc/sphx_update.h
--- /dev/null
+++ b/sph-code_amd/csrc/sphx_update.h
@@ -0,0 +1,67 @@
+#pragma once
+#include "sphx_leapfrog.h"
+
+__device__ __forceinline__ double sphx_update_dt(const IntegArgs& a) {
+    if (!a.ct_bits) return *a.dt;
+    if (a.fixed_dt > 0.0) return a.fixed_dt;
+    const u64 b = *a.ct_bits;
+    const double ct = sphx_ct_value(b == SPHX_CT_NONE, __longlong_as_double((long long)b), a.dt_0);
+    return sphx_dt_rule(ct, a.first, a.dt_0, a.max_age);
+}
+
+__device__ __forceinline__ void sphx_update_particle(const IntegArgs& a, int i, double dt, double x[3], double vv[3]) {
+    const double g = (a.ptype[i] == 0.0) ? 1.0 : 0.0;
+    const double v[3] = {a.vx[i], a.vy[i], a.vz[i]};
+    double pa[3], vis[3];
+    bool bad_acc = false;
+#pragma unroll
+    for (int c = 0; c < 3; ++c) {
+        if (a.G) {
+            const double praw = a.G[3 * (size_t)i + c] / a.rho[i] * g;
+            pa[c] = sphx_nan_to_num(praw);
+            vis[c] = a.va[3 * (size_t)i + c];
+            bad_acc = bad_acc || !sphx_finite(praw) || !sphx_finite(vis[c]);
+        } else {
+            const double praw = -a.ha[3 * (size_t)i + c] * g, vraw = -a.va[3 * (size_t)i + c] * g;
+            pa[c] = sphx_nan_to_num(praw);
+            vis[c] = sphx_nan_to_num(vraw);
+            bad_acc = bad_acc || !sphx_finite(praw) || !sphx_finite(vraw);
+        }
+        if (a.drag_on) {
+            const double draw = a.drag_on[3 * (size_t)i + c] * a.rhod[i] / a.rho[i] * g, rraw = a.drag_re[3 * (size_t)i + c];
+            const double dg = sphx_nan_to_num(draw);
+            vis[c] = dg + sphx_nan_to_num(rraw) + vis[c];
+            bad_acc = bad_acc || !sphx_finite(draw) || !sphx_finite(rraw);
+        }
+    }
+    x[0] = a.x[i]; x[1] = a.y[i]; x[2] = a.z[i];
+    vv[0] = v[0]; vv[1] = v[1]; vv[2] = v[2];
+    double gr[3], old[3], tot[3];
+#pragma unroll
+    for (int c = 0; c < 3; ++c) gr[c] = a.grav ? a.grav[3 * (size_t)i + c] : 0.0;
+    old[0] = a.ax[i]; old[1] = a.ay[i]; old[2] = a.az[i];
+    if (a.grav) {
+        if (a.no_old) sphx_leapfrog_update(dt, x, vv, vis, pa, gr, nullptr, tot);
+        else sphx_leapfrog_update(dt, x, vv, vis, pa, gr, old, tot);
+    } else {
+        if (a.no_old) sphx_leapfrog_update(dt, x, vv, vis, pa, nullptr, nullptr, tot);
+        else sphx_leapfrog_update(dt, x, vv, vis, pa, nullptr, old, tot);
+    }
+    a.x[i] = x[0]; a.y[i] = x[1]; a.z[i] = x[2];
+    a.vx[i] = vv[0]; a.vy[i] = vv[1]; a.vz[i] = vv[2];
+    a.ax[i] = tot[0]; a.ay[i] = tot[1]; a.az[i] = tot[2];
+    double E = a.E[i], T;
+    const double heat = a.vh[i];
+    const bool bad_en = !sphx_finite(E) || !sphx_finite(heat * dt);
+    sphx_energy_update(dt, heat, a.mu[i], a.gam[i], a.m[i], a.m_h, a.kB, E, T);
+    a.E[i] = E;
+    a.T[i] = T;
+    if (a.counters) {
+        bool bad_st = false;
+#pragma unroll
+        for (int c = 0; c < 3; ++c) bad_st = bad_st || !sphx_finite(x[c]) || !sphx_finite(vv[c]);
+        sphx_count_bad(a.counters, BAD_ACCEL, bad_acc);
+        sphx_count_bad(a.counters, BAD_ENERGY, bad_en);
+        sphx_count_bad(a.counters, BAD_STATE, bad_st);
+    }
+}
```

Result: no change. 826.9 million (median of 3 runs) (+0.1%).
